# nkkrnkl/category-agnostic-pose-estimation

Measured on AMD Instinct MI355X. Metric: episodes/sec (1-shot, 256x256, 17kpt) training step, higher is better.
Workload: dtype f32 storage/accumulate, GEMMs as bf16x3 split (3 bf16 MFMAs per product); 1 GPU; configs[1]: 1-shot training step (fwd+loss+bwd+clip+AdamW at learning rate 0, dropout on), 256x256, 17 kpt, ResNet-50 + deformable transformer, 16 episodes x 2 queries per GPU; episodes_per_gpu=16, queries_per_episode=2, image_size=256, global_batch_episodes=16, parallelism=dp1, weights=random init (no checkpoint offline)

## Files before the change

### category-agnostic-pose-estimation_amd/csrc/error.hip

```cpp
#include <stdarg.h>
#include "common.h"

static thread_local char g_err[512] = "";

int cape_set_error(const char* fmt, ...) {
  va_list ap;
  va_start(ap, fmt);
  vsnprintf(g_err, sizeof(g_err), fmt, ap);
  va_end(ap);
  return 1;
}

extern "C" const char* cape_last_error(void) { return g_err; }
extern "C" int cape_abi_version(void) { return 11; }

__global__ void rng_advance_kernel(uint64_t* st) { st[1] += 1; }
extern "C" int cape_rng_advance(uint64_t* rng_state, cape_stream_t stream) {
  CAPE_REQUIRE(rng_state != nullptr, "cape_rng_advance: null state");
  hipLaunchKernelGGL(rng_advance_kernel, dim3(1), dim3(1), 0, as_stream(stream), rng_state);
  CAPE_LAUNCH_CHECK("cape_rng_advance");
  return 0;
}

static hipEvent_t g_ev[64];
static int g_ev_next = 0, g_ev_init = 0;
static int order_after(hipStream_t first, hipStream_t then, const char* what) {
  if (!g_ev_init) {
    for (int i = 0; i < 64; ++i) {
      hipError_t e = hipEventCreateWithFlags(&g_ev[i], hipEventDisableTiming);
      if (e != hipSuccess) return cape_set_error("%s: hipEventCreate: %s", what, hipGetErrorString(e));
    }
    g_ev_init = 1;
  }
  hipEvent_t ev = g_ev[g_ev_next];
  g_ev_next = (g_ev_next + 1) & 63;
  hipError_t e = hipEventRecord(ev, first);
  if (e == hipSuccess) e = hipStreamWaitEvent(then, ev, 0);
  if (e != hipSuccess) return cape_set_error("%s: %s", what, hipGetErrorString(e));
  return 0;
}
extern "C" int cape_stream_fork(cape_stream_t main_stream, cape_stream_t side_stream) {
  return order_after(as_stream(main_stream), as_stream(side_stream), "cape_stream_fork");
}
extern "C" int cape_stream_join(cape_stream_t main_stream, cape_stream_t side_stream) {
  return order_after(as_stream(side_stream), as_stream(main_stream), "cape_stream_join");
}
```

### category-agnostic-pose-estimation_amd/csrc/gemm.hip

```cpp
#include "gemm_tile.h"

namespace {

template <int BM, int BN, int AMODE, int BMODE, bool VEC, int PREC, bool KFULL>
__global__ void __launch_bounds__(256) gemm_kernel(const GemmP pin) {
  GemmP p = pin;
  if (gridDim.y > 1) {
    const int b0 = blockIdx.y / p.bdiv, b1 = blockIdx.y - b0 * p.bdiv;
    p.A += b0 * p.sA0 + b1 * p.sA1;
    p.B += b0 * p.sB0 + b1 * p.sB1;
    p.C += b0 * p.sC0 + b1 * p.sC1;
    if (p.bias) p.bias += b0 * p.sBias0 + b1 * p.sBias1;
  }
  gemm_tile_body<BM, BN, AMODE, BMODE, VEC, PREC, KFULL>(p, (int)blockIdx.x);
}

constexpr int SK_COLS = 8, SK_KC = 256;

__global__ void __launch_bounds__(512) gemm_skinny_kernel(const GemmP p) {
  __shared__ __attribute__((aligned(16))) float xs[64 * (SK_KC + 4)];
  __shared__ __attribute__((aligned(16))) float ws[SK_COLS * (SK_KC + 4)];
  const int t = threadIdx.x;
  const int n0 = blockIdx.x * SK_COLS;
  const int col = t & (SK_COLS - 1), row = t >> 3;
// ... 46 lines not shown
      return 0;                                                                            \
    }                                                                                      \
    if (vec && kfull) hipLaunchKernelGGL((gemm_kernel<BM, BN, AM, BM_, true, 0, true>), grid, dim3(256), 0, s, p);   \
    else if (vec) hipLaunchKernelGGL((gemm_kernel<BM, BN, AM, BM_, true, 0, false>), grid, dim3(256), 0, s, p);      \
    else hipLaunchKernelGGL((gemm_kernel<BM, BN, AM, BM_, false, 0, false>), grid, dim3(256), 0, s, p);              \
    return 0;                                                                              \
  }
  CASE(0, 0) CASE(2, 0) CASE(0, 1) CASE(3, 2) CASE(1, 1) CASE(1, 3)
#undef CASE
  return cape_set_error("cape_gemm_f32: unsupported (a_mode=%d, b_mode=%d)", a_mode, b_mode);
}

}

extern "C" int cape_gemm_f32(const cape_gemm_desc* d, cape_stream_t stream) {
  CAPE_REQUIRE(d != nullptr, "cape_gemm_f32: null descriptor");
  CAPE_REQUIRE(d->M >= 0 && d->N >= 0 && d->K >= 0, "cape_gemm_f32: negative size");
  if (d->M == 0 || d->N == 0) return 0;
  CAPE_REQUIRE(d->A && d->B && d->C, "cape_gemm_f32: null operand");
  CAPE_REQUIRE(d->split_k >= 1, "cape_gemm_f32: split_k must be >= 1");
  if (d->split_k > 1)
    CAPE_REQUIRE(!d->scale && !d->residual && !d->relu && d->dropout_p == 0.f,
                 "cape_gemm_f32: split_k > 1 allows no epilogue op besides the bias and accumulation");
  if (d->a_mode == 2 || d->a_mode == 3 || d->b_mode == 2 || d->b_mode == 3) {
    CAPE_REQUIRE(d->cC % 4 == 0 && d->cO % 4 == 0, "cape_gemm_f32: conv channels must be multiples of 4 (C=%d, O=%d)", d->cC, d->cO);
    CAPE_REQUIRE(d->cStride >= 1 && d->cKH >= 1 && d->cKW >= 1, "cape_gemm_f32: bad conv geometry");
    const long long taps = (long long)d->cKH * d->cKW;
    if (d->a_mode == 2) CAPE_REQUIRE(d->K == taps * d->cC && d->M == (long long)d->cN * d->cOH * d->cOW, "cape_gemm_f32: conv-fwd shape mismatch");
    if (d->a_mode == 3) CAPE_REQUIRE(d->K == taps * d->cO && d->M == (long long)d->cN * d->cH * d->cW && d->N == d->cC, "cape_gemm_f32: conv-dgrad shape mismatch");
    if (d->b_mode == 3) CAPE_REQUIRE(d->N == taps * d->cC && d->K == (long long)d->cN * d->cOH * d->cOW && d->M == d->cO, "cape_gemm_f32: conv-wgrad shape mismatch");
    CAPE_REQUIRE((reinterpret_cast<uintptr_t>(d->A) & 15) == 0 && (reinterpret_cast<uintptr_t>(d->B) & 15) == 0,
                 "cape_gemm_f32: conv operands must be 16-byte aligned");
  }
  if (d->dropout_p > 0.f) CAPE_REQUIRE(d->rng_state != nullptr && d->dropout_p < 1.f, "cape_gemm_f32: dropout needs rng_state and p < 1");

  GemmP p;
  p.M = d->M; p.N = d->N; p.K = d->K;
  p.A = d->A; p.lda = d->lda; p.B = d->B; p.ldb = d->ldb; p.C = d->C; p.ldc = d->ldc;
  p.cN = d->cN; p.cH = d->cH; p.cW = d->cW; p.cC = d->cC; p.cKH = d->cKH; p.cKW = d->cKW;
  p.cStride = d->cStride; p.cPad = d->cPad; p.cOH = d->cOH; p.cOW = d->cOW; p.cO = d->cO;
  p.scale = d->scale; p.bias = d->bias; p.residual = d->residual; p.ldr = d->ldr;
  p.relu = d->relu; p.accumulate = d->accumulate; p.split_k = d->split_k;
  p.colsum_out = d->colsum_out;
  if (d->colsum_out) CAPE_REQUIRE(d->a_mode == 1, "cape_gemm_f32: colsum_out needs a_mode 1 (the wgrad product)");
  p.drop_thresh = d->dropout_p > 0.f ? cape_drop_threshold(d->dropout_p) : 0u;
  p.inv_keep = d->dropout_p > 0.f ? 1.f / (1.f - d->dropout_p) : 1.f;
  p.rng_state = d->rng_state; p.rng_stream = d->rng_stream;

  p.Bpack = d->B_packed;
  p.mask_src = d->mask_src; p.ldm = d->ldm; p.mask_scale = d->mask_scale;
  p.bdiv = d->batch_div > 0 ? d->batch_div : 1;
  p.sA0 = d->sA0; p.sA1 = d->sA1; p.sB0 = d->sB0; p.sB1 = d->sB1; p.sC0 = d->sC0; p.sC1 = d->sC1;
  p.res_cols = d->res_cols; p.sBias0 = d->sBias0; p.sBias1 = d->sBias1;
  if (d->cKHp > 0) {
    CAPE_REQUIRE(d->a_mode == 3 && d->b_mode == 2 && d->cStride == 1 && d->cO % 32 == 0 && d->K % 32 == 0 && d->cKWp > 0 &&
                     d->cTapHS >= 1 && d->cTapWS >= 1 && d->cTapH0 >= 0 && d->cTapW0 >= 0 &&
                     d->cTapH0 + (d->cKH - 1) * d->cTapHS < d->cKHp && d->cTapW0 + (d->cKW - 1) * d->cTapWS < d->cKWp,
                 "cape_gemm_f32: tap sub-lattice needs conv-dgrad modes, stride 1, O %% 32 == 0 and taps inside the physical filter");
    p.cPadX = d->cPadX; p.cKHp = d->cKHp; p.cKWp = d->cKWp;
    p.cTapH0 = d->cTapH0; p.cTapHS = d->cTapHS; p.cTapW0 = d->cTapW0; p.cTapWS = d->cTapWS;
  } else {
    p.cPadX = d->cPad; p.cKHp = d->cKH; p.cKWp = d->cKW; p.cTapH0 = 0; p.cTapHS = 1; p.cTapW0 = 0; p.cTapWS = 1;
  }
  CAPE_REQUIRE(d->res_cols >= 0 && d->res_cols % 32 == 0, "cape_gemm_f32: res_cols must be a non-negative multiple of 32");
  if (d->batch > 1)
    CAPE_REQUIRE(d->batch <= 65535 && d->split_k == 1 && !d->scale && !d->residual && !d->mask_src && !d->colsum_out &&
                     d->dropout_p == 0.f && (d->a_mode == 0 || d->a_mode == 1) && (d->b_mode == 0 || d->b_mode == 1),
                 "cape_gemm_f32: batched launches take dense modes, no epilogue vector besides the bias, split_k 1, batch <= 65535");
  if (d->mask_src) CAPE_REQUIRE(d->split_k == 1, "cape_gemm_f32: mask_src needs split_k == 1");
  CAPE_REQUIRE(d->precision >= 0 && d->precision <= 2, "cape_gemm_f32: precision must be 0 (fp32), 1 (bf16x3) or 2 (single bf16)");
  p.single = d->precision == 2;
  const int prec = d->precision == 0 ? 0 : 1;
  if (prec == 1 && d->batch <= 1 && cape_gemm_rs_eligible(p, d->a_mode, d->b_mode)) return cape_gemm_rs_launch(p, d->b_mode, as_stream(stream));

  auto al16 = [](const void* q) { return (reinterpret_cast<uintptr_t>(q) & 15) == 0; };
  bool vec = al16(d->A) && al16(d->B);
  if (d->a_mode == 0) vec = vec && (d->lda % 4 == 0) && (d->K % 4 == 0);
  if (d->a_mode == 1) vec = vec && (d->lda % 4 == 0) && (d->M % 4 == 0) && d->M >= 4;
  if (d->b_mode == 0) vec = vec && (d->ldb % 4 == 0) && (d->K % 4 == 0);
  if (d->b_mode == 1) vec = vec && (d->ldb % 4 == 0) && (d->N % 4 == 0) && d->N >= 4;
  if (d->b_mode == 2 || d->b_mode == 3) vec = vec && (d->N % 4 == 0) && d->N >= 4;
  if (d->batch > 1) vec = vec && ((d->sA0 | d->sA1 | d->sB0 | d->sB1) % 4 == 0);
  if ((d->a_mode >= 2 || d->b_mode >= 2) && !vec) return cape_set_error("cape_gemm_f32: conv modes need the aligned vector path");
  if (d->a_mode == 0 && d->b_mode == 0 && d->M <= 64 && d->batch <= 1 && vec && d->split_k == 1 && d->dropout_p == 0.f && !d->colsum_out &&
      !d->mask_src && (d->N + SK_COLS - 1) / SK_COLS < (1 << 30)) {
    static const bool off = getenv("CAPE_GEMM_NO_SKINNY") != nullptr;
    if (!off) {
      hipLaunchKernelGGL(gemm_skinny_kernel, dim3((d->N + SK_COLS - 1) / SK_COLS), dim3(512), 0, as_stream(stream), p);
      CAPE_LAUNCH_CHECK("cape_gemm_f32(skinny)");
      return 0;
    }
  }

  const long long t128 = (long long)((d->M + 127) / 128) * ((d->N + 127) / 128) * d->split_k;
  bool big = d->K / d->split_k >= 1024 && t128 >= 256 && (long long)d->M * d->N >= 256 * 1024 && prec == 1 && vec;
  {
    static const char* force = getenv("CAPE_GEMM_TILE");
    if (force && force[0] == '1') big = true;
    if (force && force[0] == '6') big = false;
  }
  const int BMv = big ? 128 : 64;
  p.tilesM = (d->M + BMv - 1) / BMv;
  p.tilesN = (d->N + BMv - 1) / BMv;
  const long long ntiles = (long long)p.tilesM * p.tilesN;
  CAPE_REQUIRE(ntiles < (1ll << 31), "cape_gemm_f32: too many tiles");
  CAPE_REQUIRE(ntiles * d->split_k < (1ll << 31), "cape_gemm_f32: grid too large");
// ... 93 lines not shown
```

### category-agnostic-pose-estimation_amd/csrc/gemm_common.h

```cpp
#pragma once
#include "common.h"

typedef float f32x16 __attribute__((ext_vector_type(16)));
typedef __bf16 bf16x8 __attribute__((ext_vector_type(8)));

typedef __bf16 bf16x2 __attribute__((ext_vector_type(2)));
__device__ __forceinline__ unsigned pk_bf16(float lo, float hi) {
  bf16x2 v;
  v[0] = (__bf16)lo;
  v[1] = (__bf16)hi;
  return __builtin_bit_cast(unsigned, v);
}
__device__ __forceinline__ void split2(float& x, float& y, unsigned& hi, unsigned& lo) {
  hi = pk_bf16(x, y);
  const bf16x2 hv = __builtin_bit_cast(bf16x2, hi);
  x = __builtin_amdgcn_fdot2_f32_bf16(hv, __builtin_bit_cast(bf16x2, 0x8000BF80u), x, false);
  y = __builtin_amdgcn_fdot2_f32_bf16(hv, __builtin_bit_cast(bf16x2, 0xBF808000u), y, false);
  lo = pk_bf16(x, y);
}

struct GemmP {
  int M, N, K;
  const float* A; long long lda;
  const float* B; long long ldb;
  float* C; long long ldc;
  int cN, cH, cW, cC, cKH, cKW, cStride, cPad, cOH, cOW, cO;
  const float* scale; const float* bias; const float* residual; long long ldr;
  int relu, accumulate, split_k;
  float* colsum_out;
  uint32_t drop_thresh; float inv_keep;
  const uint64_t* rng_state; uint32_t rng_stream;
  int tilesM, tilesN;
  const unsigned short* Bpack;
  const float* mask_src; long long ldm; float mask_scale;
  int bdiv; long long sA0, sA1, sB0, sB1, sC0, sC1;
  int single;
  int res_cols;
  long long sBias0, sBias1;
  int cPadX, cKHp, cKWp, cTapH0, cTapHS, cTapW0, cTapWS;
};

__device__ __forceinline__ float4 zero4() { return make_float4(0.f, 0.f, 0.f, 0.f); }

template <int W>
__device__ __forceinline__ int tr_off(int k, int chunk) {
  static_assert(W == 64 || W == 128, "tile widths of the family");
  const int mask = (W == 128) ? ((k & 3) << 2) : (((k >> 1) & 1) << 2);
  return k * (W * 2) + ((chunk ^ mask) << 4);
}
typedef short tr_s4 __attribute__((ext_vector_type(4)));
__device__ __forceinline__ bf16x8 tr_read8(const char* p, int rows4) {
#if defined(__HIP_DEVICE_COMPILE__)
  const tr_s4 a = __builtin_amdgcn_ds_read_tr16_b64_v4i16((tr_s4 __attribute__((address_space(3)))*)(p));
  const tr_s4 b = __builtin_amdgcn_ds_read_tr16_b64_v4i16((tr_s4 __attribute__((address_space(3)))*)(p + rows4));
  typedef short s8 __attribute__((ext_vector_type(8)));
  const s8 v = __builtin_shufflevector(a, b, 0, 1, 2, 3, 4, 5, 6, 7);
  return __builtin_bit_cast(bf16x8, v);
#else
  (void)p; (void)rows4;
  return bf16x8{};
#endif
}

constexpr int BK = 32;

bool cape_gemm_rs_eligible(const GemmP& p, int a_mode, int b_mode);
int cape_gemm_rs_launch(const GemmP& p, int b_mode, hipStream_t stream);
```

### category-agnostic-pose-estimation_amd/csrc/gemm_group.hip

```cpp
#include "gemm_tile.h"

namespace {

constexpr int GROUP_MAX = CAPE_GEMM_GROUP_MAX;

struct GroupItem {
  const float* A; const float* B; float* C; float* colsum_out;
  int M, N, K, split_k;
  int lda, ldb, ldc, tilesM;
  int tilesN, cN, cH, cW;
  int cC, cKH, cKW, cStride;
  int cPad, cOH, cOW, cO;
};

struct GroupArgs {
  int n, single;
  int bstart[GROUP_MAX + 1];
  GroupItem it[GROUP_MAX];
};
static_assert(sizeof(GroupArgs) <= 4096, "the item table travels as kernel arguments");

template <int BM, int BN, int BMODE, int PREC, bool KFULL>
__global__ void __launch_bounds__(256) gemm_group_kernel(const GroupArgs g) {
  const int b = blockIdx.x;
  int i = 0;
  while (i + 1 < g.n && b >= g.bstart[i + 1]) ++i;
  const GroupItem& q = g.it[i];
  GemmP p;
  p.M = q.M; p.N = q.N; p.K = q.K;
  p.A = q.A; p.lda = q.lda; p.B = q.B; p.ldb = q.ldb; p.C = q.C; p.ldc = q.ldc;
  p.cN = q.cN; p.cH = q.cH; p.cW = q.cW; p.cC = q.cC; p.cKH = q.cKH; p.cKW = q.cKW;
  p.cStride = q.cStride; p.cPad = q.cPad; p.cOH = q.cOH; p.cOW = q.cOW; p.cO = q.cO;
  p.cPadX = q.cPad; p.cKHp = q.cKH; p.cKWp = q.cKW; p.cTapH0 = 0; p.cTapHS = 1; p.cTapW0 = 0; p.cTapWS = 1;
  p.scale = nullptr; p.bias = nullptr; p.residual = nullptr; p.ldr = 0;
  p.relu = 0; p.accumulate = 1; p.split_k = q.split_k;
  p.colsum_out = q.colsum_out;
  p.drop_thresh = 0; p.inv_keep = 1.f; p.rng_state = nullptr; p.rng_stream = 0;
  p.tilesM = q.tilesM; p.tilesN = q.tilesN;
  p.Bpack = nullptr; p.mask_src = nullptr; p.ldm = 0; p.mask_scale = 1.f;
  p.bdiv = 1; p.sA0 = p.sA1 = p.sB0 = p.sB1 = p.sC0 = p.sC1 = 0;
  p.res_cols = 0; p.sBias0 = p.sBias1 = 0; p.single = g.single;
  gemm_tile_body<BM, BN, 1, BMODE, true, PREC, KFULL>(p, b - g.bstart[i]);
}

template <int BM, int BMODE>
void launch_group(const GroupArgs& g, int prec, bool kfull, hipStream_t s) {
  const dim3 grid((unsigned)g.bstart[g.n]), block(256);
  if (prec == 1) {
    if (kfull) hipLaunchKernelGGL((gemm_group_kernel<BM, BM, BMODE, 1, true>), grid, block, 0, s, g);
    else hipLaunchKernelGGL((gemm_group_kernel<BM, BM, BMODE, 1, false>), grid, block, 0, s, g);
  } else {
    if (kfull) hipLaunchKernelGGL((gemm_group_kernel<BM, BM, BMODE, 0, true>), grid, block, 0, s, g);
    else hipLaunchKernelGGL((gemm_group_kernel<BM, BM, BMODE, 0, false>), grid, block, 0, s, g);
  }
}

}

extern "C" int cape_gemm_group_f32(const cape_gemm_desc* descs, int n, int tile, cape_stream_t stream) {
  CAPE_REQUIRE(descs != nullptr && n >= 1 && n <= GROUP_MAX, "cape_gemm_group_f32: n=%d must be in 1..%d", n, GROUP_MAX);
  CAPE_REQUIRE(tile == 64 || tile == 128, "cape_gemm_group_f32: tile must be 64 or 128");
  const int b_mode = descs[0].b_mode, prec_in = descs[0].precision, prec = prec_in == 0 ? 0 : 1;
  CAPE_REQUIRE(b_mode == 1 || b_mode == 3, "cape_gemm_group_f32: only the weight-gradient modes (a_mode 1, b_mode 1 or 3) are grouped");
  CAPE_REQUIRE(prec_in >= 0 && prec_in <= 2, "cape_gemm_group_f32: precision must be 0 (fp32), 1 (bf16x3) or 2 (single bf16)");
  auto al16 = [](const void* q) { return (reinterpret_cast<uintptr_t>(q) & 15) == 0; };
  GroupArgs g;
  g.n = n;
  g.single = prec_in == 2;
  bool kfull = true;
  long long blocks = 0;
  for (int i = 0; i < n; ++i) {
    const cape_gemm_desc& d = descs[i];
    CAPE_REQUIRE(d.a_mode == 1 && d.b_mode == b_mode && d.precision == prec_in, "cape_gemm_group_f32: item %d: mixed modes / precisions", i);
    CAPE_REQUIRE(d.M > 0 && d.N > 0 && d.K > 0 && d.A && d.B && d.C, "cape_gemm_group_f32: item %d: empty product or null operand", i);
    CAPE_REQUIRE(d.accumulate && !d.scale && !d.bias && !d.residual && !d.relu && d.dropout_p == 0.f && !d.mask_src && d.batch <= 1,
                 "cape_gemm_group_f32: item %d: grouped products accumulate onto C and take no other epilogue operand", i);
    CAPE_REQUIRE(d.split_k >= 1, "cape_gemm_group_f32: item %d: split_k must be >= 1", i);
    CAPE_REQUIRE(al16(d.A) && al16(d.B) && d.lda % 4 == 0 && d.M % 4 == 0 && d.M >= 4 && d.N % 4 == 0 && d.N >= 4 &&
                     (b_mode == 3 || d.ldb % 4 == 0),
                 "cape_gemm_group_f32: item %d: operands must be 16-byte aligned with M, N, lda, ldb multiples of 4", i);
    CAPE_REQUIRE(d.lda < (1ll << 31) && d.ldb < (1ll << 31) && d.ldc < (1ll << 31), "cape_gemm_group_f32: item %d: leading dimension too large", i);
    if (b_mode == 3) {
      const long long taps = (long long)d.cKH * d.cKW;
      CAPE_REQUIRE(d.cC % 4 == 0 && d.cO % 4 == 0 && d.cStride >= 1 && d.cKH >= 1 && d.cKW >= 1, "cape_gemm_group_f32: item %d: bad conv geometry", i);
      CAPE_REQUIRE(d.N == taps * d.cC && d.K == (long long)d.cN * d.cOH * d.cOW && d.M == d.cO, "cape_gemm_group_f32: item %d: conv-wgrad shape mismatch", i);
    }
    GroupItem& q = g.it[i];
    q.A = d.A; q.B = d.B; q.C = d.C; q.colsum_out = d.colsum_out;
    q.M = d.M; q.N = d.N; q.K = d.K; q.split_k = d.split_k;
    q.lda = (int)d.lda; q.ldb = (int)d.ldb; q.ldc = (int)d.ldc;
    q.tilesM = (d.M + tile - 1) / tile; q.tilesN = (d.N + tile - 1) / tile;
    q.cN = d.cN; q.cH = d.cH; q.cW = d.cW; q.cC = d.cC; q.cKH = d.cKH; q.cKW = d.cKW;
    q.cStride = d.cStride; q.cPad = d.cPad; q.cOH = d.cOH; q.cOW = d.cOW; q.cO = d.cO;
    kfull = kfull && (d.K % BK == 0);
// ... 14 lines not shown
```

### category-agnostic-pose-estimation_amd/csrc/gemm_rs.hip

```cpp
#include <stdlib.h>
#include "gemm_common.h"

namespace {

constexpr int RS_UNIT = 64;

#ifdef RS_STAMPS
__device__ long long* g_rs_stamps;
#define RS_STAMP(i) do { if (threadIdx.x == 0 && (i) < 16) g_rs_stamps[blockIdx.x * 16 + (i)] = clock64(); } while (0)
#define RS_FINE(cond, i) do { if ((cond) && threadIdx.x == 0) g_rs_stamps[blockIdx.x * 16 + 8 + (i)] = clock64(); } while (0)
#else
#define RS_STAMP(i) do {} while (0)
#define RS_FINE(cond, i) do {} while (0)
#endif

template <int KS>
struct RsGeom {
  static constexpr int K = 16 * KS;
  static constexpr int LD = K + 8;
  static constexpr int PLANE = RS_UNIT * LD;
  static constexpr int NV = KS / 2;
  static constexpr size_t LDS_BYTES = (size_t)2  * 2  * PLANE * 2;
};

template <int NW, int BMODE, int KS, int EPI>
__global__ void __launch_bounds__(512) gemm_rs_kernel(const GemmP p, int nchunks, int gpc) {
  using G = RsGeom<KS>;
  constexpr int K = G::K, LD = G::LD, NV = G::NV;
  constexpr int CPR = K / 4;
  extern __shared__ __attribute__((aligned(16))) unsigned short lds[];

  const int t = threadIdx.x, lane = t & 63, wave = t >> 6;
  const int r = lane & 31, h = lane >> 5;
  const int wn = wave % NW, wm = wave / NW;

  const int bid = blockIdx.x;
  const int xcd = bid & 7, loc = bid >> 3;
  const int chunk = loc % nchunks;
  const int slot = (loc / nchunks) * 8 + xcd;
  const int n0 = chunk * (32 * NW) + 32 * wn;
  const int nunits = (p.M + RS_UNIT - 1) / RS_UNIT;
  if (slot >= nunits) return;

  const int st_row = t / CPR, st_kc = t % CPR;
  constexpr int RSTEP = 512 / CPR;
  auto load_rows = [&](float4 (&dst)[NV], const float* base, long long ld, int row0, int nrows) {
#pragma unroll
    for (int i = 0; i < NV; ++i) {
      const int row = min(row0 + st_row + RSTEP * i, nrows - 1);
      dst[i] = *reinterpret_cast<const float4*>(base + (long long)row * ld + 4 * st_kc);
    }
  };
  auto store_rows = [&](float4 (&src)[NV], int buf) {
    unsigned short* Ph = lds + buf * 2 * G::PLANE;
    unsigned short* Pl = Ph + G::PLANE;
#pragma unroll
    for (int i = 0; i < NV; ++i) {
      const int o = (st_row + RSTEP * i) * LD + 4 * st_kc;
      unsigned h0, l0, h1, l1;
      split2(src[i].x, src[i].y, h0, l0);
      split2(src[i].z, src[i].w, h1, l1);
      *reinterpret_cast<uint2*>(Ph + o) = make_uint2(h0, h1);
      *reinterpret_cast<uint2*>(Pl + o) = make_uint2(l0, l1);
    }
  };

  const int col = n0 + r;
  const bool col_ok = col < p.N;
  const float sc = p.scale ? p.scale[min(col, p.N - 1)] : 1.f;
  const float bi = p.bias ? p.bias[min(col, p.N - 1)] : 0.f;
  const float floor_v = p.relu ? 0.f : -__builtin_inff();
  uint64_t seed = 0, step = 0;
  if constexpr (EPI == 4) { seed = p.rng_state[0]; step = p.rng_state[1]; }
  const int ldc = (int)p.ldc;
  const unsigned lo_c = (unsigned)(4 * h * ldc + col);
  const int ldx = EPI == 1 ? (int)p.ldr : ldc;
  const unsigned lo_x = (unsigned)(4 * h * ldx + col);
  const bool res_on = EPI != 1 || !p.res_cols || n0 < p.res_cols;

  auto store_piece = [&](float4& v, int i, int buf) {
    unsigned short* Ph = lds + buf * 2 * G::PLANE + (st_row + RSTEP * i) * LD + 4 * st_kc;
    unsigned h0, l0, h1, l1;
    split2(v.x, v.y, h0, l0);
    split2(v.z, v.w, h1, l1);
    *reinterpret_cast<uint2*>(Ph) = make_uint2(h0, h1);
    *reinterpret_cast<uint2*>(Ph + G::PLANE) = make_uint2(l0, l1);
  };

  RS_STAMP(0);
  bf16x8 bhi[KS], blo[KS];
  float4 ra[NV];
  if (p.Bpack) {
    load_rows(ra, p.A, p.lda, slot * RS_UNIT, p.M);
    const int grp = min(n0 >> 5, (p.N + 31) / 32 - 1);
    const uint4* bp = reinterpret_cast<const uint4*>(p.Bpack) + ((long long)grp * KS * 2) * 64 + lane;
#pragma unroll
    for (int s = 0; s < KS; ++s) {
      bhi[s] = __builtin_bit_cast(bf16x8, bp[(2 * s + 0) * 64]);
      blo[s] = __builtin_bit_cast(bf16x8, bp[(2 * s + 1) * 64]);
    }
  } else if constexpr (BMODE == 0) {
    constexpr int NPASS = NW / 2;
    const int nb = chunk * (32 * NW);
    float4 rw[2][NV];
    load_rows(rw[0], p.B, p.ldb, nb, p.N);
    if (NPASS > 1) load_rows(rw[1], p.B, p.ldb, nb + 64, p.N);
    load_rows(ra, p.A, p.lda, slot * RS_UNIT, p.M);
#pragma unroll
    for (int q = 0; q < NPASS; ++q) {
      store_rows(rw[q & 1], q & 1);
      if (q + 2 < NPASS) load_rows(rw[q & 1], p.B, p.ldb, nb + 64 * (q + 2), p.N);
      __syncthreads();
      if ((wn >> 1) == q) {
        const unsigned short* Ph = lds + (q & 1) * 2 * G::PLANE + (32 * (wn & 1) + r) * LD + 8 * h;
#pragma unroll
        for (int s = 0; s < KS; ++s) {
          bhi[s] = *reinterpret_cast<const bf16x8*>(Ph + 16 * s);
          blo[s] = *reinterpret_cast<const bf16x8*>(Ph + G::PLANE + 16 * s);
        }
      }
    }
    __syncthreads();
  } else {
    load_rows(ra, p.A, p.lda, slot * RS_UNIT, p.M);
    const int n = min(n0 + r, p.N - 1);
#pragma unroll
    for (int s = 0; s < KS; ++s) {
      float f[8];
      const int k = 16 * s + 8 * h;
#pragma unroll
      for (int j = 0; j < 8; ++j) f[j] = p.B[(long long)(k + j) * p.ldb + n];
      unsigned hw[4], lw[4];
#pragma unroll
      for (int j = 0; j < 4; ++j) split2(f[2 * j], f[2 * j + 1], hw[j], lw[j]);
      bhi[s] = __builtin_bit_cast(bf16x8, make_uint4(hw[0], hw[1], hw[2], hw[3]));
      blo[s] = __builtin_bit_cast(bf16x8, make_uint4(lw[0], lw[1], lw[2], lw[3]));
    }
  }

  RS_STAMP(1);
  store_rows(ra, 0);
  if (slot + gpc < nunits) load_rows(ra, p.A, p.lda, (slot + gpc) * RS_UNIT, p.M);
  __syncthreads();
  RS_STAMP(2);
  int stamp_i = 3;

  int buf = 0;
  for (int u = slot; u < nunits; u += gpc) {
    const bool has_next = u + gpc < nunits;
    const unsigned short* Ah = lds + buf * 2 * G::PLANE;
    const unsigned short* Al = Ah + G::PLANE;
    const bool full = (u + 1) * RS_UNIT <= p.M;
    constexpr int H1 = (NW == 8) ? 2 : 1;
#pragma unroll
    for (int hh = 0; hh < H1; ++hh) {
      const int half = (NW == 8) ? hh : wm;
      float xv[16];
      if constexpr (EPI >= 1 && EPI <= 3) {
        if (col_ok && res_on) {
          const int rb = u * RS_UNIT + 32 * half;
          const float* xb = EPI == 1 ? p.residual : EPI == 2 ? p.mask_src : p.C;
          const float* x0 = xb + (long long)rb * ldx;
#pragma unroll
          for (int i = 0; i < 16; ++i) {
            const int roff = (i & 3) + 8 * (i >> 2);
            if (full) xv[i] = x0[lo_x + (unsigned)(roff * ldx)];
            else xv[i] = xb[(long long)min(rb + roff + 4 * h, p.M - 1) * ldx + col];
          }
        } else {
#pragma unroll
          for (int i = 0; i < 16; ++i) xv[i] = 0.f;
        }
      }
      f32x16 acc;
#pragma unroll
      for (int i = 0; i < 16; ++i) acc[i] = 0.f;
      RS_FINE(u == slot + gpc, 3 * hh);
      const int ao = (32 * half + r) * LD + 8 * h;
#pragma unroll
      for (int s = 0; s < KS; ++s) {
        const bf16x8 ahi = *reinterpret_cast<const bf16x8*>(Ah + ao + 16 * s);
        const bf16x8 alo = *reinterpret_cast<const bf16x8*>(Al + ao + 16 * s);
        if (!p.single) {
          acc = __builtin_amdgcn_mfma_f32_32x32x16_bf16(alo, bhi[s], acc, 0, 0, 0);
          acc = __builtin_amdgcn_mfma_f32_32x32x16_bf16(ahi, blo[s], acc, 0, 0, 0);
        }
        acc = __builtin_amdgcn_mfma_f32_32x32x16_bf16(ahi, bhi[s], acc, 0, 0, 0);
        if (hh == H1 - 1 && s >= KS - NV && has_next) store_piece(ra[s - (KS - NV)], s - (KS - NV), buf ^ 1);
      }
      RS_FINE(u == slot + gpc, 3 * hh + 1);
      if (!col_ok) continue;
      const int rb = u * RS_UNIT + 32 * half;
      const int rlim = full ? 64 : p.M - rb - 4 * h;
      float* c0 = p.C + (long long)rb * ldc;
      if constexpr (EPI == 0) {
        if (full) {
#pragma unroll
          for (int i = 0; i < 16; ++i) c0[lo_c + (unsigned)(((i & 3) + 8 * (i >> 2)) * ldc)] = fmaxf(fmaf(acc[i], sc, bi), floor_v);
        } else {
#pragma unroll
          for (int i = 0; i < 16; ++i) {
            const int roff = (i & 3) + 8 * (i >> 2);
            if (roff < rlim) c0[lo_c + (unsigned)(roff * ldc)] = fmaxf(fmaf(acc[i], sc, bi), floor_v);
          }
        }
      } else if constexpr (EPI == 4) {
#pragma unroll
        for (int i = 0; i < 16; ++i) {
          const int roff = (i & 3) + 8 * (i >> 2);
          const int row = rb + roff + 4 * h;
          float v = fmaxf(fmaf(acc[i], sc, bi), floor_v);
          v = cape_keep(seed, step, p.rng_stream, (uint64_t)row * (uint64_t)p.N + col, p.drop_thresh) ? v * p.inv_keep : 0.f;
          if (roff < rlim) c0[lo_c + (unsigned)(roff * ldc)] = v;
        }
      } else {
#pragma unroll
        for (int i = 0; i < 16; ++i) {
          const int roff = (i & 3) + 8 * (i >> 2);
          const float x = xv[i];
          float v = fmaf(acc[i], sc, bi);
          if constexpr (EPI == 1) v = fmaxf(v + x, floor_v);
          if constexpr (EPI == 2) v = x != 0.f ? fmaxf(v, floor_v) * p.mask_scale : 0.f;
          if constexpr (EPI == 3) v = fmaxf(v, floor_v) + x;
          if (roff < rlim) c0[lo_c + (unsigned)(roff * ldc)] = v;
        }
      }
    }
    RS_FINE(u == slot + gpc, 6);
    if (u + 2 * gpc < nunits) load_rows(ra, p.A, p.lda, (u + 2 * gpc) * RS_UNIT, p.M);
    __syncthreads();
    RS_FINE(u == slot + gpc, 7);
    RS_STAMP(stamp_i); ++stamp_i;
    buf ^= 1;
  }
}

static int rs_epi(const GemmP& p) {
  const int n = (p.residual != nullptr) + (p.mask_src != nullptr) + (p.accumulate != 0) + (p.drop_thresh != 0);
  if (n == 0) return 0;
  if (n > 1) return -1;
  return p.residual ? 1 : p.mask_src ? 2 : p.accumulate ? 3 : 4;
}

template <int NW, int BMODE, int KS, int EPI>
int rs_launch_epi(const GemmP& p, int nchunks, int gpc, hipStream_t s) {
  static bool attr_set = false;
  auto kfn = gemm_rs_kernel<NW, BMODE, KS, EPI>;
  if (!attr_set) {
    hipError_t e = hipFuncSetAttribute(reinterpret_cast<const void*>(kfn), hipFuncAttributeMaxDynamicSharedMemorySize,
                                       (int)RsGeom<KS>::LDS_BYTES);
    if (e != hipSuccess) return cape_set_error("cape_gemm_f32(rs): hipFuncSetAttribute: %s", hipGetErrorString(e));
    attr_set = true;
  }
  hipLaunchKernelGGL(kfn, dim3((unsigned)(gpc * nchunks)), dim3(512), RsGeom<KS>::LDS_BYTES, s, p, nchunks, gpc);
  return 0;
}

template <int NW, int BMODE, int KS>
int rs_launch(const GemmP& p, int nchunks, int gpc, hipStream_t s) {
  switch (rs_epi(p)) {
    case 0: return rs_launch_epi<NW, BMODE, KS, 0>(p, nchunks, gpc, s);
    case 1: return rs_launch_epi<NW, BMODE, KS, 1>(p, nchunks, gpc, s);
    case 2: return rs_launch_epi<NW, BMODE, KS, 2>(p, nchunks, gpc, s);
    case 3: return rs_launch_epi<NW, BMODE, KS, 3>(p, nchunks, gpc, s);
    case 4: return rs_launch_epi<NW, BMODE, KS, 4>(p, nchunks, gpc, s);
  }
  return cape_set_error("cape_gemm_f32(rs): unsupported epilogue combination");
}

struct PackItem { const float* B; unsigned short* out; long long ldb; int N, K, b_mode, pad; };
static_assert(sizeof(PackItem) == sizeof(cape_pack_item), "cape_pack_item layout");

__global__ void __launch_bounds__(256) pack_weights_kernel(const PackItem* items, int n_items) {
  const int lane = threadIdx.x & 63, wave = threadIdx.x >> 6;
  const int r = lane & 31, h = lane >> 5;
  for (int it = blockIdx.y; it < n_items; it += gridDim.y) {
    const PackItem q = items[it];
    const int KS = q.K >> 4, groups = (q.N + 31) >> 5;
    for (int w = blockIdx.x * 4 + wave; w < groups * KS; w += gridDim.x * 4) {
      const int g = w / KS, s = w - g * KS;
      const int n = 32 * g + r, k = 16 * s + 8 * h;
      float f[8];
#pragma unroll
      for (int j = 0; j < 8; ++j) f[j] = 0.f;
      if (n < q.N) {
        if (q.b_mode == 0) {
#pragma unroll
          for (int j = 0; j < 8; ++j) f[j] = q.B[(long long)n * q.ldb + k + j];
        } else {
#pragma unroll
          for (int j = 0; j < 8; ++j) f[j] = q.B[(long long)(k + j) * q.ldb + n];
        }
      }
      unsigned hw[4], lw[4];
#pragma unroll
      for (int j = 0; j < 4; ++j) split2(f[2 * j], f[2 * j + 1], hw[j], lw[j]);
      uint4* o = reinterpret_cast<uint4*>(q.out) + ((long long)w * 2) * 64 + lane;
      o[0] = make_uint4(hw[0], hw[1], hw[2], hw[3]);
      o[64] = make_uint4(lw[0], lw[1], lw[2], lw[3]);
    }
  }
}

}

extern "C" size_t cape_packed_weight_bytes(int N, int K) {
  if (N <= 0 || K <= 0) return 0;
  return (size_t)((N + 31) / 32) * 32 * (size_t)K * 4;
}

extern "C" int cape_pack_weights(const cape_pack_item* items_dev, int n_items, int max_blocks_per_item, cape_stream_t stream) {
  CAPE_REQUIRE(items_dev != nullptr && n_items >= 0 && max_blocks_per_item >= 1, "cape_pack_weights: bad arguments");
  if (n_items == 0) return 0;
  const unsigned gy = (unsigned)(n_items < 65535 ? n_items : 65535);
  hipLaunchKernelGGL(pack_weights_kernel, dim3((unsigned)max_blocks_per_item, gy), dim3(256), 0, as_stream(stream),
                     reinterpret_cast<const PackItem*>(items_dev), n_items);
  CAPE_LAUNCH_CHECK("cape_pack_weights");
  return 0;
// ... 42 lines not shown
```

### category-agnostic-pose-estimation_amd/csrc/gemm_tile.h

```cpp
#pragma once
#include <stdlib.h>
#include <type_traits>
#include "gemm_common.h"

namespace {

__device__ __forceinline__ float4 ldg4(const float* p, int valid) {
  if (valid >= 4 && ((reinterpret_cast<uintptr_t>(p) & 15) == 0)) return *reinterpret_cast<const float4*>(p);
  float4 r = zero4();
  if (valid > 0) r.x = p[0];
  if (valid > 1) r.y = p[1];
  if (valid > 2) r.z = p[2];
  if (valid > 3) r.w = p[3];
  return r;
}

template <int BM, int BN, int AMODE, int BMODE, bool VEC, int PREC, bool KFULL>
__device__ __forceinline__ void gemm_tile_body(const GemmP& p, const int bid) {
  constexpr bool A_KC = (AMODE == 0 || AMODE == 2 || AMODE == 3);
  constexpr bool B_KC = (BMODE == 0);
  constexpr int A_LD = A_KC ? 36 : (BM + 4);
  constexpr int B_LD = B_KC ? 36 : (BN + 4);
  constexpr int A_SZ = A_KC ? BM * 36 : BK * (BM + 4);
  constexpr int B_SZ = B_KC ? BN * 36 : BK * (BN + 4);
// ... 482 lines not shown
    if (t + 1 + DEPTH < kt_end) load_tiles(t + 1 + DEPTH, NEXT);
  };
  using S0 = std::integral_constant<int, 0>;
  using S1 = std::integral_constant<int, 1 % DEPTH>;
  using S2 = std::integral_constant<int, 2 % DEPTH>;
  load_tiles(kt_begin, S0{});
  if constexpr (DEPTH >= 2)
    if (kt_begin + 1 < kt_end) load_tiles(kt_begin + 1, S1{});
  if constexpr (DEPTH == 3)
    if (kt_begin + 2 < kt_end) load_tiles(kt_begin + 2, S2{});
  if (do_colsum) colsum_tile(S0{});
  store_tiles(0, S0{});
  if (kt_begin + DEPTH < kt_end) load_tiles(kt_begin + DEPTH, S0{});
  __syncthreads();
  int cur = 0;
  for (int kt = kt_begin; kt < kt_end; kt += DEPTH) {
    pipeline_step(kt, cur, S1{});
    cur ^= 1;
    if constexpr (DEPTH >= 2) {
      if (kt + 1 >= kt_end) break;
      pipeline_step(kt + 1, cur, S2{});
      cur ^= 1;
    }
    if constexpr (DEPTH == 3) {
      if (kt + 2 >= kt_end) break;
      pipeline_step(kt + 2, cur, S0{});
      cur ^= 1;
    }
  }

  if constexpr (AMODE == 1) {
    if (do_colsum) {
      float4* red = reinterpret_cast<float4*>(&As[0][0]);
      red[t] = csum;
      __syncthreads();
      if (t < A_CH) {
        float4 r = red[t];
#pragma unroll
        for (int i = 1; i < 256 / A_CH; ++i) { const float4 u = red[t + A_CH * i]; r.x += u.x; r.y += u.y; r.z += u.z; r.w += u.w; }
        const int m = m0 + 4 * t;
        if (m < p.M) atomicAdd(p.colsum_out + m, r.x);
        if (m + 1 < p.M) atomicAdd(p.colsum_out + m + 1, r.y);
        if (m + 2 < p.M) atomicAdd(p.colsum_out + m + 2, r.z);
        if (m + 3 < p.M) atomicAdd(p.colsum_out + m + 3, r.w);
      }
    }
  }

  uint64_t seed = 0, step = 0;
  const bool drop = p.drop_thresh != 0;
  if (drop) { seed = p.rng_state[0]; step = p.rng_state[1]; }
  const bool atomic = p.split_k > 1;
  const bool interior = (m0 + BM <= p.M) && (n0 + BN <= p.N);
  const int n_extra = (p.residual != nullptr) + (p.mask_src != nullptr) + (p.accumulate != 0) + (drop ? 1 : 0);
  const bool same_ld = (!p.residual || p.ldr == p.ldc) && (!p.mask_src || p.ldm == p.ldc);
  if (interior && !drop && n_extra <= 1 && same_ld && (long long)BM * p.ldc < (1ll << 30)) {
    const int wave_s = __builtin_amdgcn_readfirstlane(wave);
    const int wm_s = wave_s >> 1, wn_s = wave_s & 1;
    const int ldc = (int)p.ldc;
    const float floor_v = p.relu ? 0.f : -INFINITY;
    const float* xb = p.residual ? p.residual : p.mask_src ? p.mask_src : (p.accumulate && !atomic) ? p.C : nullptr;
    const int kind = atomic ? 1 : p.residual ? 2 : p.mask_src ? 3 : p.accumulate ? 4 : 0;
#pragma unroll
    for (int i = 0; i < TI; ++i) {
#pragma unroll
      for (int j = 0; j < TJ; ++j) {
        const int colb = n0 + wn_s * WTN + j * 32;
        const long long base = (long long)(m0 + wm_s * WTM + i * 32) * ldc + colb;
        float* c0 = p.C + base;
        const unsigned lo = (unsigned)(4 * lh * ldc + l31);
        const float sc = p.scale ? p.scale[colb + l31] : 1.f;
        const float bi = p.bias ? p.bias[colb + l31] : 0.f;
        const int kind_t = (kind == 2 && p.res_cols && colb >= p.res_cols) ? 0 : kind;
        if (kind == 1) {
          const float b0 = split == 0 ? bi : 0.f;
#pragma unroll
          for (int r = 0; r < 16; ++r) atomicAdd(c0 + (lo + (unsigned)(((r & 3) + 8 * (r >> 2)) * ldc)), acc[i][j][r] + b0);
        } else if (kind_t == 0) {
#pragma unroll
          for (int r = 0; r < 16; ++r) c0[lo + (unsigned)(((r & 3) + 8 * (r >> 2)) * ldc)] = fmaxf(fmaf(acc[i][j][r], sc, bi), floor_v);
        } else {
          const float* x0 = xb + base;
          float xv[16];
#pragma unroll
          for (int r = 0; r < 16; ++r) xv[r] = x0[lo + (unsigned)(((r & 3) + 8 * (r >> 2)) * ldc)];
#pragma unroll
          for (int r = 0; r < 16; ++r) {
            float v = fmaf(acc[i][j][r], sc, bi);
            if (kind == 2) v = fmaxf(v + xv[r], floor_v);
            else if (kind == 3) v = xv[r] != 0.f ? fmaxf(v, floor_v) * p.mask_scale : 0.f;
            else v = fmaxf(v, floor_v) + xv[r];
            c0[lo + (unsigned)(((r & 3) + 8 * (r >> 2)) * ldc)] = v;
          }
        }
      }
    }
    return;
  }
#pragma unroll
  for (int i = 0; i < TI; ++i) {
#pragma unroll
    for (int j = 0; j < TJ; ++j) {
      const int col = n0 + wn * WTN + j * 32 + l31;
      if (!interior && col >= p.N) continue;
      const float sc = p.scale ? p.scale[col] : 1.f;
      const float bi = p.bias ? p.bias[col] : 0.f;
#pragma unroll
      for (int r = 0; r < 16; ++r) {
        const int row = m0 + wm * WTM + i * 32 + (r & 3) + 8 * (r >> 2) + 4 * lh;
        if (!interior && row >= p.M) continue;
        float v = acc[i][j][r];
        float* cp = p.C + (long long)row * p.ldc + col;
        if (atomic) { atomicAdd(cp, split == 0 ? v + bi : v); continue; }
        v = v * sc + bi;
        if (p.residual && (!p.res_cols || col < p.res_cols)) v += p.residual[(long long)row * p.ldr + col];
        if (p.relu) v = fmaxf(v, 0.f);
        if (drop) v = cape_keep(seed, step, p.rng_stream, (uint64_t)row * (uint64_t)p.N + col, p.drop_thresh) ? v * p.inv_keep : 0.f;
        if (p.mask_src) v = p.mask_src[(long long)row * p.ldm + col] != 0.f ? v * p.mask_scale : 0.f;
        if (p.accumulate) v += *cp;
        *cp = v;
      }
    }
  }
}

}
```

### category-agnostic-pose-estimation_amd/csrc/norm.hip

```cpp
#include "common.h"

namespace {

constexpr int LN_MAXV = 4;

__global__ void __launch_bounds__(256) add_ln_fwd_kernel(const float* __restrict__ x, const float* __restrict__ y,
                                                          const float* __restrict__ gamma, const float* __restrict__ beta,
                                                          float* __restrict__ out, float* __restrict__ mean_o,
                                                          float* __restrict__ rstd_o, const float* __restrict__ pos,
                                                          float* __restrict__ out_pos, int rows, int C, uint32_t thresh,
                                                          float inv_keep, const uint64_t* rng_state, uint32_t rng_stream) {
  const int lane = threadIdx.x & 63;
  const int row = blockIdx.x * 4 + (threadIdx.x >> 6);
  if (row >= rows) return;
  const int nv = C >> 8;
  const int rem = (C & 255) >> 2;
  uint64_t seed = 0, step = 0;
  if (thresh) { seed = rng_state[0]; step = rng_state[1]; }
  float4 s[LN_MAXV];
  float sum = 0.f;
  const long long base = (long long)row * C;
#pragma unroll
  for (int i = 0; i < LN_MAXV; ++i) {
    const bool act = (i < nv) || (i == nv && lane < rem);
// ... 55 lines not shown
#endif
constexpr int LN_BWD_ROWS = LN_BWD_ROWS_DEF;

__global__ void __launch_bounds__(256) add_ln_bwd_kernel(const float* __restrict__ d_out, const float* __restrict__ d_out_pos,
                                                          const float* __restrict__ x, const float* __restrict__ y,
                                                          const float* __restrict__ gamma, const float* __restrict__ mean_i,
                                                          const float* __restrict__ rstd_i, float* __restrict__ d_x,
                                                          float* __restrict__ d_y, float* __restrict__ dgamma,
                                                          float* __restrict__ dbeta, int rows, int C, uint32_t thresh,
                                                          float inv_keep, const uint64_t* rng_state, uint32_t rng_stream) {
  __shared__ float red[2][4][1024];
  const int lane = threadIdx.x & 63, w = threadIdx.x >> 6;
  const int nv = C >> 8, rem = (C & 255) >> 2;
  uint64_t seed = 0, step = 0;
  if (thresh) { seed = rng_state[0]; step = rng_state[1]; }
  float4 ag[LN_MAXV], ab[LN_MAXV], gam[LN_MAXV];
#pragma unroll
  for (int i = 0; i < LN_MAXV; ++i) {
    ag[i] = make_float4(0.f, 0.f, 0.f, 0.f);
    ab[i] = make_float4(0.f, 0.f, 0.f, 0.f);
    const bool act = (i < nv) || (i == nv && lane < rem);
    gam[i] = act ? *reinterpret_cast<const float4*>(gamma + (i * 64 + lane) * 4) : make_float4(0.f, 0.f, 0.f, 0.f);
  }
  const int r_begin = blockIdx.x * LN_BWD_ROWS;
  for (int rr = w; rr < LN_BWD_ROWS; rr += 4) {
    const int row = r_begin + rr;
    if (row >= rows) break;
    const long long base = (long long)row * C;
    const float mean = mean_i[row], rstd = rstd_i[row];
    float4 xh[LN_MAXV], g[LN_MAXV];
    uint32_t keepbits = 0;
    float s1 = 0.f, s2 = 0.f;
#pragma unroll
    for (int i = 0; i < LN_MAXV; ++i) {
      const bool act = (i < nv) || (i == nv && lane < rem);
      xh[i] = make_float4(0.f, 0.f, 0.f, 0.f);
      g[i] = make_float4(0.f, 0.f, 0.f, 0.f);
      if (act) {
        const int c = (i * 64 + lane) * 4;
        float4 v = *reinterpret_cast<const float4*>(x + base + c);
        if (y) {
          float4 q = *reinterpret_cast<const float4*>(y + base + c);
          if (thresh) {
            const uint64_t idx = (uint64_t)base + c;
            const bool k0 = cape_keep(seed, step, rng_stream, idx + 0, thresh);
            const bool k1 = cape_keep(seed, step, rng_stream, idx + 1, thresh);
            const bool k2 = cape_keep(seed, step, rng_stream, idx + 2, thresh);
            const bool k3 = cape_keep(seed, step, rng_stream, idx + 3, thresh);
            keepbits |= ((uint32_t)k0 | ((uint32_t)k1 << 1) | ((uint32_t)k2 << 2) | ((uint32_t)k3 << 3)) << (4 * i);
            q.x = k0 ? q.x * inv_keep : 0.f; q.y = k1 ? q.y * inv_keep : 0.f;
            q.z = k2 ? q.z * inv_keep : 0.f; q.w = k3 ? q.w * inv_keep : 0.f;
          }
          v.x += q.x; v.y += q.y; v.z += q.z; v.w += q.w;
        }
        float4 d = *reinterpret_cast<const float4*>(d_out + base + c);
        if (d_out_pos) {
          const float4 e = *reinterpret_cast<const float4*>(d_out_pos + base + c);
          d.x += e.x; d.y += e.y; d.z += e.z; d.w += e.w;
        }
        xh[i].x = (v.x - mean) * rstd; xh[i].y = (v.y - mean) * rstd;
        xh[i].z = (v.z - mean) * rstd; xh[i].w = (v.w - mean) * rstd;
        ag[i].x += d.x * xh[i].x; ag[i].y += d.y * xh[i].y; ag[i].z += d.z * xh[i].z; ag[i].w += d.w * xh[i].w;
        ab[i].x += d.x; ab[i].y += d.y; ab[i].z += d.z; ab[i].w += d.w;
        g[i].x = d.x * gam[i].x; g[i].y = d.y * gam[i].y; g[i].z = d.z * gam[i].z; g[i].w = d.w * gam[i].w;
        s1 += g[i].x + g[i].y + g[i].z + g[i].w;
        s2 += g[i].x * xh[i].x + g[i].y * xh[i].y + g[i].z * xh[i].z + g[i].w * xh[i].w;
      }
    }
    const float m1 = wave_sum(s1) / (float)C, m2 = wave_sum(s2) / (float)C;
#pragma unroll
    for (int i = 0; i < LN_MAXV; ++i) {
      const bool act = (i < nv) || (i == nv && lane < rem);
      if (act) {
        const int c = (i * 64 + lane) * 4;
        float4 ds;
        ds.x = rstd * (g[i].x - m1 - xh[i].x * m2);
        ds.y = rstd * (g[i].y - m1 - xh[i].y * m2);
        ds.z = rstd * (g[i].z - m1 - xh[i].z * m2);
        ds.w = rstd * (g[i].w - m1 - xh[i].w * m2);
        *reinterpret_cast<float4*>(d_x + base + c) = ds;
        if (d_y && d_y != d_x) {
          if (thresh) {
            const uint32_t kb = keepbits >> (4 * i);
            ds.x = (kb & 1) ? ds.x * inv_keep : 0.f; ds.y = (kb & 2) ? ds.y * inv_keep : 0.f;
            ds.z = (kb & 4) ? ds.z * inv_keep : 0.f; ds.w = (kb & 8) ? ds.w * inv_keep : 0.f;
          }
          *reinterpret_cast<float4*>(d_y + base + c) = ds;
        }
      }
    }
  }
#pragma unroll
  for (int i = 0; i < LN_MAXV; ++i) {
    const bool act = (i < nv) || (i == nv && lane < rem);
    if (act) {
      const int c = (i * 64 + lane) * 4;
      *reinterpret_cast<float4*>(&red[0][w][c]) = ag[i];
      *reinterpret_cast<float4*>(&red[1][w][c]) = ab[i];
    }
  }
  __syncthreads();
#ifndef LAB_LN_NO_ATOMIC
  for (int c = threadIdx.x; c < C; c += 256) {
    atomicAdd(&dgamma[c], red[0][0][c] + red[0][1][c] + red[0][2][c] + red[0][3][c]);
    atomicAdd(&dbeta[c], red[1][0][c] + red[1][1][c] + red[1][2][c] + red[1][3][c]);
  }
#endif
}

constexpr int LN256_R = 4;

constexpr int LN256_W = 16;

__global__ void __launch_bounds__(64 * LN256_W) add_ln_bwd256_kernel(const float* __restrict__ d_out, const float* __restrict__ d_out_pos,
                                                             const float* __restrict__ x, const float* __restrict__ y,
                                                             const float* __restrict__ gamma, const float* __restrict__ mean_i,
                                                             const float* __restrict__ rstd_i, float* __restrict__ d_x,
                                                             float* __restrict__ d_y, float* __restrict__ dgamma,
                                                             float* __restrict__ dbeta, int rows, uint32_t thresh, float inv_keep,
                                                             const uint64_t* rng_state, uint32_t rng_stream) {
  __shared__ float red[2][LN256_W][256];
  const int lane = threadIdx.x & 63, w = threadIdx.x >> 6;
  uint64_t seed = 0, step = 0;
  if (thresh) { seed = rng_state[0]; step = rng_state[1]; }
  const float4 gam = *reinterpret_cast<const float4*>(gamma + 4 * lane);
  float4 ag = make_float4(0.f, 0.f, 0.f, 0.f), ab = make_float4(0.f, 0.f, 0.f, 0.f);
  const bool split = d_y && d_y != d_x;
  const int wave_g = blockIdx.x * LN256_W + w, nwaves = gridDim.x * LN256_W;
  for (int r0 = wave_g * LN256_R; r0 < rows; r0 += nwaves * LN256_R) {
    float4 v[LN256_R], d[LN256_R];
    float mean[LN256_R], rstd[LN256_R];
    uint32_t kb[LN256_R];
#pragma unroll
    for (int k = 0; k < LN256_R; ++k) {
      const int row = min(r0 + k, rows - 1);
      const long long base = (long long)row * 256 + 4 * lane;
      v[k] = *reinterpret_cast<const float4*>(x + base);
      d[k] = *reinterpret_cast<const float4*>(d_out + base);
      mean[k] = mean_i[row]; rstd[k] = rstd_i[row];
    }
    if (y) {
#pragma unroll
      for (int k = 0; k < LN256_R; ++k) {
        const int row = min(r0 + k, rows - 1);
        const long long base = (long long)row * 256 + 4 * lane;
        float4 q = *reinterpret_cast<const float4*>(y + base);
        kb[k] = 0xF;
        if (thresh) {
          const uint64_t idx = (uint64_t)base;
          const bool k0 = cape_keep(seed, step, rng_stream, idx + 0, thresh), k1 = cape_keep(seed, step, rng_stream, idx + 1, thresh);
          const bool k2 = cape_keep(seed, step, rng_stream, idx + 2, thresh), k3 = cape_keep(seed, step, rng_stream, idx + 3, thresh);
          kb[k] = (uint32_t)k0 | ((uint32_t)k1 << 1) | ((uint32_t)k2 << 2) | ((uint32_t)k3 << 3);
          q.x = k0 ? q.x * inv_keep : 0.f; q.y = k1 ? q.y * inv_keep : 0.f;
          q.z = k2 ? q.z * inv_keep : 0.f; q.w = k3 ? q.w * inv_keep : 0.f;
        }
        v[k].x += q.x; v[k].y += q.y; v[k].z += q.z; v[k].w += q.w;
      }
    }
    if (d_out_pos) {
#pragma unroll
      for (int k = 0; k < LN256_R; ++k) {
        const int row = min(r0 + k, rows - 1);
        const float4 e = *reinterpret_cast<const float4*>(d_out_pos + (long long)row * 256 + 4 * lane);
        d[k].x += e.x; d[k].y += e.y; d[k].z += e.z; d[k].w += e.w;
      }
    }
#pragma unroll
    for (int k = 0; k < LN256_R; ++k) {
      const bool live = r0 + k < rows;
      float4 xh, g;
      xh.x = (v[k].x - mean[k]) * rstd[k]; xh.y = (v[k].y - mean[k]) * rstd[k];
      xh.z = (v[k].z - mean[k]) * rstd[k]; xh.w = (v[k].w - mean[k]) * rstd[k];
      if (live) {
        ag.x += d[k].x * xh.x; ag.y += d[k].y * xh.y; ag.z += d[k].z * xh.z; ag.w += d[k].w * xh.w;
        ab.x += d[k].x; ab.y += d[k].y; ab.z += d[k].z; ab.w += d[k].w;
      }
      g.x = d[k].x * gam.x; g.y = d[k].y * gam.y; g.z = d[k].z * gam.z; g.w = d[k].w * gam.w;
      const float m1 = wave_sum(g.x + g.y + g.z + g.w) * (1.f / 256.f);
      const float m2 = wave_sum(g.x * xh.x + g.y * xh.y + g.z * xh.z + g.w * xh.w) * (1.f / 256.f);
      float4 ds;
      ds.x = rstd[k] * (g.x - m1 - xh.x * m2); ds.y = rstd[k] * (g.y - m1 - xh.y * m2);
      ds.z = rstd[k] * (g.z - m1 - xh.z * m2); ds.w = rstd[k] * (g.w - m1 - xh.w * m2);
      if (live) {
        const long long base = (long long)(r0 + k) * 256 + 4 * lane;
        *reinterpret_cast<float4*>(d_x + base) = ds;
        if (split) {
          if (thresh) {
            ds.x = (kb[k] & 1) ? ds.x * inv_keep : 0.f; ds.y = (kb[k] & 2) ? ds.y * inv_keep : 0.f;
            ds.z = (kb[k] & 4) ? ds.z * inv_keep : 0.f; ds.w = (kb[k] & 8) ? ds.w * inv_keep : 0.f;
          }
          *reinterpret_cast<float4*>(d_y + base) = ds;
        }
      }
    }
  }
  *reinterpret_cast<float4*>(&red[0][w][4 * lane]) = ag;
  *reinterpret_cast<float4*>(&red[1][w][4 * lane]) = ab;
  __syncthreads();
  if (threadIdx.x < 512) {
    const int which = threadIdx.x >> 8, c = threadIdx.x & 255;
    float a = 0.f;
#pragma unroll
    for (int k = 0; k < LN256_W; ++k) a += red[which][k][c];
    atomicAdd((which ? dbeta : dgamma) + c, a);
  }
}

constexpr int GN_ROWS = 16;

// ... 54 lines not shown
  atomicAdd(w, sd);
  atomicAdd(w + 1, sdx);
}

__global__ void groupnorm_bwd_apply_kernel(const float* __restrict__ d_out, long long d_out_image_stride,
                                           const float* __restrict__ x, const float* __restrict__ gamma,
                                           const float* __restrict__ mean_i, const float* __restrict__ rstd_i,
                                           const float* __restrict__ ws, float* __restrict__ d_x,
                                           float* __restrict__ dgamma, float* __restrict__ dbeta, int HW, int C, int G) {
  const int n = blockIdx.y, c = threadIdx.x;
  const int cpg = C / G;
  const float mean = mean_i[n * G + c / cpg], rstd = rstd_i[n * G + c / cpg];
  const float sd = ws[((long long)n * C + c) * 2], sdx = ws[((long long)n * C + c) * 2 + 1];
  if (blockIdx.x == 0) { atomicAdd(&dgamma[c], sdx); atomicAdd(&dbeta[c], sd); }
  const float g = gamma[c];
  const float cnt = (float)HW * (float)cpg;
  const float A = group_sum(g * sd, cpg) / cnt;
  const float B = group_sum(g * sdx, cpg) / cnt;
  const int r0 = blockIdx.x * GN_ROWS, r1 = min(HW, r0 + GN_ROWS);
  const float* xp = x + (long long)n * HW * C + c;
  const float* dp = d_out + (long long)n * d_out_image_stride + c;
  float* op = d_x + (long long)n * HW * C + c;
  for (int r = r0; r < r1; ++r) {
    const float xh = (xp[(long long)r * C] - mean) * rstd;
    op[(long long)r * C] = rstd * (g * dp[(long long)r * C] - A - xh * B);
  }
}

}

extern "C" int cape_add_layernorm_fwd(const float* x, const float* y, const float* gamma, const float* beta,
                                      float* out, float* mean, float* rstd, const float* pos, float* out_pos,
                                      int rows, int C, float dropout_p, const uint64_t* rng_state,
                                      uint32_t rng_stream, cape_stream_t stream) {
  CAPE_REQUIRE(x && gamma && beta && out && mean && rstd, "cape_add_layernorm_fwd: null pointer");
  CAPE_REQUIRE(C > 0 && C <= 1024 && (C % 4) == 0, "cape_add_layernorm_fwd: C=%d must be a multiple of 4, <= 1024", C);
  CAPE_REQUIRE((pos == nullptr) == (out_pos == nullptr), "cape_add_layernorm_fwd: pos and out_pos go together");
  CAPE_REQUIRE(dropout_p == 0.f || (y && rng_state && dropout_p < 1.f), "cape_add_layernorm_fwd: dropout needs y and rng_state");
  if (rows <= 0) return 0;
  const uint32_t th = dropout_p > 0.f ? cape_drop_threshold(dropout_p) : 0u;
  const float ik = dropout_p > 0.f ? 1.f / (1.f - dropout_p) : 1.f;
  hipLaunchKernelGGL(add_ln_fwd_kernel, dim3((rows + 3) / 4), dim3(256), 0, as_stream(stream), x, y, gamma, beta, out,
                     mean, rstd, pos, out_pos, rows, C, th, ik, rng_state, rng_stream);
  CAPE_LAUNCH_CHECK("cape_add_layernorm_fwd");
  return 0;
}

extern "C" int cape_add_layernorm_bwd(const float* d_out, const float* d_out_pos, const float* x, const float* y,
                                      const float* gamma, const float* mean, const float* rstd, float* d_x,
                                      float* d_y, float* dgamma, float* dbeta, int rows, int C, float dropout_p,
                                      const uint64_t* rng_state, uint32_t rng_stream, cape_stream_t stream) {
  CAPE_REQUIRE(d_out && x && gamma && mean && rstd && d_x && dgamma && dbeta, "cape_add_layernorm_bwd: null pointer");
  CAPE_REQUIRE(C > 0 && C <= 1024 && (C % 4) == 0, "cape_add_layernorm_bwd: C=%d must be a multiple of 4, <= 1024", C);
  CAPE_REQUIRE(dropout_p == 0.f || (y && d_y && d_y != d_x && rng_state && dropout_p < 1.f),
               "cape_add_layernorm_bwd: dropout needs y, a separate d_y and rng_state");
  if (rows <= 0) return 0;
  const uint32_t th = dropout_p > 0.f ? cape_drop_threshold(dropout_p) : 0u;
  const float ik = dropout_p > 0.f ? 1.f / (1.f - dropout_p) : 1.f;
  static const bool general_only = getenv("CAPE_LN_BWD_GENERAL") != nullptr;
  if (C == 256 && !general_only) {
    const int trips = (rows + LN256_W * LN256_R - 1) / (LN256_W * LN256_R);
    const int blocks = trips < 256 ? trips : 256;
    hipLaunchKernelGGL(add_ln_bwd256_kernel, dim3(blocks), dim3(64 * LN256_W), 0, as_stream(stream), d_out, d_out_pos, x, y, gamma, mean, rstd,
                       d_x, d_y, dgamma, dbeta, rows, th, ik, rng_state, rng_stream);
    CAPE_LAUNCH_CHECK("cape_add_layernorm_bwd");
    return 0;
  }
  hipLaunchKernelGGL(add_ln_bwd_kernel, dim3((rows + LN_BWD_ROWS - 1) / LN_BWD_ROWS), dim3(256), 0, as_stream(stream),
                     d_out, d_out_pos, x, y, gamma, mean, rstd, d_x, d_y, dgamma, dbeta, rows, C, th, ik, rng_state,
                     rng_stream);
  CAPE_LAUNCH_CHECK("cape_add_layernorm_bwd");
  return 0;
}

static int gn_check(int N, int HW, int C, int G) {
  if (N <= 0 || HW <= 0) return 0;
  CAPE_REQUIRE(C >= 64 && C <= 1024 && (C % 64) == 0, "cape_groupnorm: C=%d must be a multiple of 64, <= 1024", C);
  CAPE_REQUIRE(G > 0 && (C % G) == 0, "cape_groupnorm: G=%d must divide C=%d", G, C);
  const int cpg = C / G;
  CAPE_REQUIRE(cpg <= 64 && (cpg & (cpg - 1)) == 0, "cape_groupnorm: channels per group (%d) must be a power of two <= 64", cpg);
  return 0;
}

extern "C" size_t cape_groupnorm_workspace_bytes(int N, int C, int G) {
  if (N <= 0 || C <= 0 || G <= 0) return 0;
  const size_t f = (size_t)N * G * 2 * sizeof(double), b = (size_t)N * C * 2 * sizeof(float);
  return f > b ? f : b;
}

extern "C" int cape_groupnorm_fwd(const float* x, const float* gamma, const float* beta, float* out,
                                  long long out_image_stride, float* mean, float* rstd, int N, int HW, int C, int G,
                                  void* workspace, size_t workspace_bytes, cape_stream_t stream) {
  CAPE_REQUIRE(x && gamma && beta && out && mean && rstd, "cape_groupnorm_fwd: null pointer");
  if (gn_check(N, HW, C, G)) return 1;
  if (N <= 0 || HW <= 0) return 0;
  const size_t need = (size_t)N * G * 2 * sizeof(double);
  CAPE_REQUIRE(workspace && workspace_bytes >= need && (reinterpret_cast<uintptr_t>(workspace) & 7) == 0,
               "cape_groupnorm_fwd: workspace of %zu bytes (8-byte aligned) needed, %zu given", need, workspace_bytes);
  CAPE_REQUIRE(N <= 65535, "cape_groupnorm_fwd: N too large");
  hipError_t e = hipMemsetAsync(workspace, 0, need, as_stream(stream));
  if (e != hipSuccess) return cape_set_error("cape_groupnorm_fwd: memset: %s", hipGetErrorString(e));
  const dim3 grid((HW + GN_ROWS - 1) / GN_ROWS, N);
  hipLaunchKernelGGL(groupnorm_stats_kernel, grid, dim3(C), 0, as_stream(stream), x, static_cast<double*>(workspace), HW, C, G);
  hipLaunchKernelGGL(groupnorm_apply_kernel, grid, dim3(C), 0, as_stream(stream), x, gamma, beta, out, out_image_stride,
                     static_cast<const double*>(workspace), mean, rstd, HW, C, G);
  CAPE_LAUNCH_CHECK("cape_groupnorm_fwd");
  return 0;
}
// ... 23 lines not shown
```

### category-agnostic-pose-estimation_amd/hip/functional.py

```python
import contextlib
import ctypes
import os

import torch

from . import lib, ops


class Runtime:
    rng = None
    direct_grad = False
    use_side_stream = os.environ.get("CAPE_SIDE_STREAM", "1") == "1"
    side = None
    on_param_grad = []
    capture_keep = None

    pending = []
    side_dirty = False

    defer_wgrad = os.environ.get("CAPE_DEFER_WGRAD", "1") == "1"
    wgrad_group = int(os.environ.get("CAPE_WGRAD_GROUP", "12"))
    wq = {}
    wq_total = 0
    wq_notify = []
# ... 152 lines not shown
        base = p._base
        if isinstance(base, torch.nn.Parameter) and base.grad is not None and base.requires_grad:
            off = p.storage_offset() - base.storage_offset() + base.grad.storage_offset()
            return torch.as_strided(base.grad, p.shape, p.stride(), off)
        return None

    def side(self, *tensors):
        return _Side(tensors) if self.direct else _NO_SIDE

    def gemm(self, *args, **kw):
        d, keep = ops.gemm_desc(*args, **kw)
        if self.direct and Runtime.defer_wgrad and _groupable(d):
            Runtime.enqueue_wgrad(d, keep)
        else:
            ops.launch_gemm(d)

    def result(self):
        if not self.direct:
            return tuple(self.bufs)
        Runtime.notify(*[r if isinstance(r, torch.nn.Parameter) else r._base for r, n in zip(self.refs, self.needs) if n])
        return (None,) * len(self.refs)


class _Slot:
    __slots__ = ("buf",)

    def __init__(self):
        self.buf = None


_SLOTS = os.environ.get("CAPE_GRAD_SLOTS", "1") == "1"


def _slot_of(x):
    return getattr(x, "_cape_slot", None) if _SLOTS else None


def _grad_target(slot, shape, device):
    if slot is not None and slot.buf is not None:
        b = slot.buf
        if b.is_contiguous() and b.numel() == int(torch.Size(shape).numel()) and b.device == device:
            return b.view(shape), True
    buf = torch.empty(shape, dtype=torch.float32, device=device)
    if slot is not None and slot.buf is None:
        slot.buf = buf
    return buf, False


def _slot_offer(slot, buf):
    if slot is not None and slot.buf is None and buf is not None and buf.is_contiguous():
        slot.buf = buf


class LinearFn(torch.autograd.Function):
    @staticmethod
    def forward(ctx, x, weight, bias, residual, relu, dropout_p, rng_stream):
        K = x.shape[-1]
        N = weight.shape[0]
        assert weight.shape[1] == K and weight.stride(1) == 1
        x2 = _c(x).view(-1, K)
        M = x2.shape[0]
        res2 = _c(residual).view(-1, N) if residual is not None else None
        y = torch.empty(M, N, dtype=torch.float32, device=x.device)
        rng = Runtime.get_rng(x.device) if dropout_p > 0 else None
        ops.gemm(x2, weight, y, M, N, K, ldb=weight.stride(0), bias=bias, residual=res2, relu=relu, dropout_p=dropout_p,
                 rng=rng, rng_stream=rng_stream)
        ctx.save_for_backward(x2, weight, y if (relu or dropout_p > 0) else None)
        ctx.w_ref, ctx.b_ref = weight, bias
        ctx.slot = _slot_of(x)
        ctx.meta = (relu, dropout_p, bias is not None, residual is not None, x.shape, M, N, K)
        return y.view(*x.shape[:-1], N)

    @staticmethod
    def backward(ctx, dy):
        x2, weight, y = ctx.saved_tensors
        relu, p, has_bias, has_res, xshape, M, N, K = ctx.meta
        dy2 = _c(dy).view(M, N)
        dpre = dy2
        if relu or p > 0:
            assert relu, "dropout epilogue is only used together with relu"
            dpre = ops.relu_drop_bwd(dy2, y, 1.0 / (1.0 - p) if p > 0 else 1.0)
        dx = None
        if ctx.needs_input_grad[0]:
            dx, acc = _grad_target(ctx.slot, (M, K), dy.device)
            ops.gemm(dpre, weight, dx, M, K, N, a_mode=0, b_mode=1, ldb=weight.stride(0), accumulate=acc)
            dx = dx.view(xshape)
        pg = _ParamGrads((ctx.w_ref, ctx.b_ref), ctx.needs_input_grad[1:3])
        dw, db = pg.bufs
        with pg.side(dpre, x2):
            if dw is not None:
                pg.gemm(dpre, x2, dw, N, K, M, a_mode=1, b_mode=1, lda=N, ldb=K, ldc=dw.stride(0), accumulate=True,
                        split_k=ops.pick_split_k(N, K, M), colsum_out=db)
            elif db is not None:
                ops.colsum(dpre, M, N, db)
        dres = dy if (has_res and ctx.needs_input_grad[3]) else None
        return (dx,) + pg.result() + (dres, None, None, None)


def linear(x, weight, bias=None, residual=None, relu=False, dropout_p=0.0, rng_stream=0):
    return LinearFn.apply(x, weight, bias, residual, relu, float(dropout_p), int(rng_stream))


class FFNFn(torch.autograd.Function):

    @staticmethod
    def forward(ctx, x, w1, b1, w2, b2, dropout_p, rng_stream):
        K, Hd, N = x.shape[-1], w1.shape[0], w2.shape[0]
        x2 = _c(x).view(-1, K)
        M = x2.shape[0]
        rng = Runtime.get_rng(x.device) if dropout_p > 0 else None
        h = torch.empty(M, Hd, dtype=torch.float32, device=x.device)
        ops.gemm(x2, w1, h, M, Hd, K, ldb=w1.stride(0), bias=b1, relu=True, dropout_p=dropout_p, rng=rng, rng_stream=rng_stream)
        y = torch.empty(M, N, dtype=torch.float32, device=x.device)
        ops.gemm(h, w2, y, M, N, Hd, ldb=w2.stride(0), bias=b2)
        ctx.save_for_backward(x2, w1, w2, h)
        ctx.refs = (w1, b1, w2, b2)
        ctx.slot = _slot_of(x)
        ctx.meta = (dropout_p, x.shape, M, K, Hd, N)
        return y.view(*x.shape[:-1], N)

    @staticmethod
    def backward(ctx, dy):
        x2, w1, w2, h = ctx.saved_tensors
        p, xshape, M, K, Hd, N = ctx.meta
        dy2 = _c(dy).view(M, N)
        dpre = torch.empty(M, Hd, dtype=torch.float32, device=dy.device)
        ops.gemm(dy2, w2, dpre, M, Hd, N, a_mode=0, b_mode=1, ldb=w2.stride(0), mask_src=h, mask_scale=1.0 / (1.0 - p) if p > 0 else 1.0)
        dx = None
        if ctx.needs_input_grad[0]:
            dx, acc = _grad_target(ctx.slot, (M, K), dy.device)
            ops.gemm(dpre, w1, dx, M, K, Hd, a_mode=0, b_mode=1, ldb=w1.stride(0), accumulate=acc)
            dx = dx.view(xshape)
        pg = _ParamGrads(ctx.refs)
        dw1, db1, dw2, db2 = pg.bufs
        with pg.side(dy2, dpre, h, x2):
            pg.gemm(dy2, h, dw2, N, Hd, M, a_mode=1, b_mode=1, lda=N, ldb=Hd, ldc=dw2.stride(0), accumulate=True,
                    split_k=ops.pick_split_k(N, Hd, M), colsum_out=db2)
            pg.gemm(dpre, x2, dw1, Hd, K, M, a_mode=1, b_mode=1, lda=Hd, ldb=K, ldc=dw1.stride(0), accumulate=True,
                    split_k=ops.pick_split_k(Hd, K, M), colsum_out=db1)
        return (dx,) + pg.result() + (None, None)


_NO_FFN_FUSE = os.environ.get("CAPE_NO_FFN_FUSE") is not None
_DETERMINISTIC = os.environ.get("CAPE_DETERMINISTIC", "0") == "1"


def ffn(x, w1, b1, w2, b2, dropout_p=0.0, rng_stream=0):
    if _NO_FFN_FUSE:
        return linear(linear(x, w1, b1, relu=True, dropout_p=dropout_p, rng_stream=rng_stream), w2, b2)
    return FFNFn.apply(x, w1, b1, w2, b2, float(dropout_p), int(rng_stream))


def _adjacent(a, b):
    return (a.is_contiguous() and b.is_contiguous() and a.untyped_storage().data_ptr() == b.untyped_storage().data_ptr()
            and b.data_ptr() == a.data_ptr() + a.numel() * a.element_size())


class LinearCat2Fn(torch.autograd.Function):

    @staticmethod
    def forward(ctx, x, w1, b1, w2, b2):
        K = x.shape[-1]
        N1, N2 = w1.shape[0], w2.shape[0]
        x2 = _c(x).view(-1, K)
        M = x2.shape[0]
        y = torch.empty(M, N1 + N2, dtype=torch.float32, device=x.device)
        adjacent = _adjacent(w1, w2) and _adjacent(b1, b2)
        if adjacent:
            ops.gemm(x2, torch.as_strided(w1, (N1 + N2, K), (K, 1)), y, M, N1 + N2, K, bias=torch.as_strided(b1, (N1 + N2,), (1,)))
        else:
            ops.gemm(x2, w1, y, M, N1, K, bias=b1, ldc=N1 + N2)
            ops.gemm(x2, w2, y[:, N1:], M, N2, K, bias=b2, ldc=N1 + N2)
        ctx.save_for_backward(x2, w1, w2)
        ctx.refs = (w1, b1, w2, b2)
        ctx.meta = (x.shape, M, N1, N2, K, adjacent)
        return y.view(*x.shape[:-1], N1 + N2)

    @staticmethod
    def backward(ctx, dy):
        x2, w1, w2 = ctx.saved_tensors
        xshape, M, N1, N2, K, adjacent = ctx.meta
        NT = N1 + N2
        dy2 = _c(dy).view(M, NT)
        dev = dy.device
        dx = None
        if ctx.needs_input_grad[0]:
            dx = torch.empty(M, K, dtype=torch.float32, device=dev)
            ops.gemm(dy2, w1, dx, M, K, N1, a_mode=0, b_mode=1, lda=NT)
            ops.gemm(dy2[:, N1:], w2, dx, M, K, N2, a_mode=0, b_mode=1, lda=NT, accumulate=True)
            dx = dx.view(xshape)
        pg = _ParamGrads(ctx.refs)
        dw1, db1, dw2, db2 = pg.bufs
        with pg.side(dy2, x2):
            if adjacent and _adjacent(dw1, dw2) and _adjacent(db1, db2):
                pg.gemm(dy2, x2, torch.as_strided(dw1, (NT, K), (K, 1)), NT, K, M, a_mode=1, b_mode=1, lda=NT, accumulate=True,
                        split_k=ops.pick_split_k(NT, K, M), colsum_out=torch.as_strided(db1, (NT,), (1,)))
            else:
                for dw, db, lo, n in ((dw1, db1, 0, N1), (dw2, db2, N1, N2)):
                    pg.gemm(dy2[:, lo:], x2, dw, n, K, M, a_mode=1, b_mode=1, lda=NT, accumulate=True, split_k=ops.pick_split_k(n, K, M),
                            colsum_out=db)
        return (dx,) + pg.result()


# ... 137 lines not shown
    if not relu:
        return dy, (dy if want_res else None)
    d = ops.relu_drop_bwd(dy, y, 1.0)
    return d, (d if want_res else None)


def _mask_only(dy, y, relu):
    return ops.relu_drop_bwd(dy, y, 1.0) if relu else dy


class BottleneckFn(torch.autograd.Function):

    @staticmethod
    def forward(ctx, x, w1, w2, w3, wd, s1, b1, s2, b2, s3, b3, sd, bd, stride, allow_split):
        o1, m1, t1 = _conv_stage_fwd(x, w1, s1, b1, None, 1, 0, True, allow_split)
        o2, m2, t2 = _conv_stage_fwd(o1, w2, s2, b2, None, stride, 1, True, allow_split)
        idt, md, td = x, None, ()
        if wd is not None:
            idt, md, td = _conv_stage_fwd(x, wd, sd, bd, None, stride, 0, False, allow_split)
        y, m3, t3 = _conv_stage_fwd(o2, w3, s3, b3, idt, 1, 0, True, allow_split)
        ctx.save_for_backward(*t1, *t2, *t3, *td)
        ctx.cuts = (len(t1), len(t1) + len(t2), len(t1) + len(t2) + len(t3))
        ctx.metas = (m1, m2, m3, md)
        ctx.w_refs = (w1, w2, w3, wd)
        return y

    @staticmethod
    def backward(ctx, dy):
        t, (a, b, c) = ctx.saved_tensors, ctx.cuts
        t1, t2, t3, td = t[:a], t[a:b], t[b:c], t[c:]
        m1, m2, m3, md = ctx.metas
        w1, w2, w3, wd = ctx.w_refs
        need_x, need_w1, need_w2, need_w3, need_wd = ctx.needs_input_grad[:5]
        d2, dw3, _, dres = _conv_stage_bwd(m3, t3, dy, w3, need_x=True, need_w=need_w3, need_res=need_x or wd is not None)
        d1, dw2, _, _ = _conv_stage_bwd(m2, t2, d2, w2, need_x=True, need_w=need_w2)
        dwd, dshort = None, (dres if need_x else None)
        if wd is not None:
            dshort, dwd, _, _ = _conv_stage_bwd(md, td, dres, wd, need_x=need_x, need_w=need_wd)
        dx, dw1, _, _ = _conv_stage_bwd(m1, t1, d1, w1, need_x=need_x, need_w=need_w1, acc_dx=dshort)
        return (dx, dw1, dw2, dw3, dwd) + (None,) * 10


def bottleneck(x, w1, w2, w3, wd, bn1, bn2, bn3, bnd, stride):
    sd, bd = bnd if bnd is not None else (None, None)
    return BottleneckFn.apply(x, w1, w2, w3, wd, bn1[0], bn1[1], bn2[0], bn2[1], bn3[0], bn3[1], sd, bd, int(stride), torch.is_grad_enabled())


def conv_bn_act(x, weight, scale, shift, stride=1, pad=0, relu=False, residual=None):
    return ConvFn.apply(x, weight, scale, shift, residual, int(stride), int(pad), bool(relu), torch.is_grad_enabled())


class AddLayerNormFn(torch.autograd.Function):
    @staticmethod
    def forward(ctx, x, y, gamma, beta, pos, dropout_p, rng_stream):
        x, y, pos = _c(x), _c(y), _c(pos)
        rng = Runtime.get_rng(x.device) if dropout_p > 0 else None
        out, mean, rstd, out_pos = ops.add_layernorm_fwd(x, y, gamma, beta, pos=pos, dropout_p=dropout_p, rng=rng,
                                                         rng_stream=rng_stream)
        ctx.save_for_backward(x, y, gamma, mean, rstd)
        ctx.refs = (gamma, beta)
        ctx.slot = _slot_of(x)
        ctx.meta = (dropout_p, rng_stream, pos is not None)
        ctx.set_materialize_grads(False)
        if pos is None:
            return out
        return out, out_pos

    @staticmethod
    def backward(ctx, d_out, d_out_pos=None):
        x, y, gamma, mean, rstd = ctx.saved_tensors
        p, stream, has_pos = ctx.meta
        g_pos = d_out_pos
        if d_out is None and d_out_pos is None:
            return None, None, None, None, None, None, None
        if d_out is None:
            d_out, d_out_pos = d_out_pos, None
        d_out, d_out_pos = _c(d_out), _c(d_out_pos)
        pg = _ParamGrads(ctx.refs)
        rng = Runtime.get_rng(x.device) if p > 0 else None
        dx, dy = ops.add_layernorm_bwd(d_out, d_out_pos, x, y, gamma, mean, rstd, *pg.bufs, dropout_p=p, rng=rng,
                                       rng_stream=stream)
        if y is None or dy is not dx:
            _slot_offer(ctx.slot, dx)
        dpos = g_pos if (has_pos and ctx.needs_input_grad[4]) else None
        return (dx, (dy if y is not None else None)) + pg.result() + (dpos, None, None)


def add_layernorm(x, y, gamma, beta, pos=None, dropout_p=0.0, rng_stream=0):
    return AddLayerNormFn.apply(x, y, gamma, beta, pos, float(dropout_p), int(rng_stream))


class AddFn(torch.autograd.Function):
    @staticmethod
    def forward(ctx, a, b):
        return ops.add(_c(a), _c(b))

    @staticmethod
    def backward(ctx, g):
        return g, g


def add(a, b):
    return AddFn.apply(a, b)


class FanOutFn(torch.autograd.Function):

    @staticmethod
    def forward(ctx, x, k, slot):
        ctx.k, ctx.slot = k, slot
        ctx.set_materialize_grads(False)
        return tuple(x.view_as(x) for _ in range(k))

    @staticmethod
    def backward(ctx, *grads):
        ctx.slot.buf = None
        gs, seen = [], set()
        for g in grads:
            if g is not None and (g.data_ptr(), g.numel()) not in seen:
                seen.add((g.data_ptr(), g.numel()))
                gs.append(g)
        if not gs:
            return None, None, None
        if len(gs) > 1 and len(gs) <= 8 and not all(g.is_contiguous() for g in gs) and all(_row_strided(g) for g in gs):
            return ops.add_n_rows(gs), None, None
        gs = [_c(g) for g in gs]
        out = gs[0]
        for i in range(0, len(gs) - 1, 7):
            out = ops.add_n([out] + gs[1 + i:8 + i]) if len(gs) > 1 else out
        return out, None, None


def _row_strided(g):
    if g.dim() < 2 or g.stride(-1) != 1 or g.shape[-1] % 4 or g.data_ptr() % 16 or g.stride(-2) % 4:
        return False
    st, sh = g.stride(), g.shape
    return all(st[i] == st[i + 1] * sh[i + 1] for i in range(len(sh) - 2))


def fanout(x, k):
    if k == 1 or not (torch.is_grad_enabled() and x.requires_grad):
        return (x,) * k
# ... 184 lines not shown
        ctx.N = N
        ctx.le_ref = level_embed
        return out

    @staticmethod
    def backward(ctx, d_pos):
        geo, N = ctx.geo, ctx.N
        d_pos = _c(d_pos)
        C = d_pos.shape[-1]
        pg = _ParamGrads((ctx.le_ref,))
        for l in range(geo.L):
            h, w = geo.shapes[l]
            ops.colsum(d_pos[0, geo.starts[l]:], h * w, C, pg.bufs[0][l], nbatch=N, batch_stride=geo.S * C)
        return (None,) + pg.result() + (None,) * geo.L


def level_pos(geo, level_embed, masks_u8):
    return LevelPosFn.apply(geo, level_embed, *masks_u8)


class MSDAFn(torch.autograd.Function):
    @staticmethod
    def forward(ctx, value, offw, ref, geo, P):
        value, offw, ref = _c(value), _c(offw), _c(ref)
        N, Lq = offw.shape[0], offw.shape[1]
        out = ops.msda_fwd(value, offw, ref, geo, N, Lq, P)
        ctx.save_for_backward(value, offw, ref)
        ctx.meta = (geo, N, Lq, P)
        return out

    @staticmethod
    def backward(ctx, d_out):
        value, offw, ref = ctx.saved_tensors
        geo, N, Lq, P = ctx.meta
        dv, do, dr = ops.msda_bwd(_c(d_out), value, offw, ref, geo, N, Lq, P, need_ref_grad=ctx.needs_input_grad[2])
        return dv, do, dr, None, None


def msda(value, offw, ref, geo, P=4):
    return MSDAFn.apply(value, offw, ref, geo, P)


def _from_row(t, r):
    return t if (t is None or r == 0) else t[r:]


def _col_blocks(groups, bufs, C):
    return [buf[..., j * C:(j + 1) * C] for (_, w, *_), buf in zip(groups, bufs) for j in range(w)]


class MHAFn(torch.autograd.Function):

    @staticmethod
    def forward(ctx, q_in, k_in, v_in, in_w, in_b, out_w, out_b, nheads, mask_mode, kpm_u8, dropout_p, rng_stream):
        ins = q_in, k_in, v_in = _c(q_in), _c(k_in), _c(v_in)
        N, Lq, C = q_in.shape
        Lk = k_in.shape[1]
        dev = q_in.device
        scale = (C // nheads) ** -0.5
        rng = Runtime.get_rng(dev) if dropout_p > 0 else None
        ctx.route = ops.attn_route(N, nheads, Lq, Lk, flash=False)
        if ctx.route != "mm" and k_in is v_in:
            layout = ((0, 3),) if q_in is k_in else ((0, 1), (1, 2))
        else:
            layout = ((0, 1), (1, 1), (2, 1))
        ctx.groups = tuple((r, w, r != 1 and ins[r] is k_in) for r, w in layout)
        bufs = [torch.empty(N, ins[r].shape[1], w * C, dtype=torch.float32, device=dev) for r, w in layout]
        for (r, w), buf in zip(layout, bufs):
            ops.gemm(ins[r].view(-1, C), _from_row(in_w, r * C), buf, N * ins[r].shape[1], w * C, C, bias=_from_row(in_b, r * C))
        q, k, v = _col_blocks(layout, bufs, C)
        O, saved = ops.attn_core_fwd(ctx.route, q, k, v, N, nheads, Lq, Lk, scale, mask_mode=mask_mode, kpm=kpm_u8, dropout_p=dropout_p,
                                     rng=rng, rng_stream=rng_stream)
        out = torch.empty(N, Lq, C, dtype=torch.float32, device=dev)
        ops.gemm(O.view(-1, C), out_w, out, N * Lq, C, C, bias=out_b)
        ctx.save_for_backward(q_in, k_in, v_in, in_w, out_w, q, k, v, O, kpm_u8, *saved)
        ctx.refs = (in_w, in_b, out_w, out_b)
        ctx.slot_q = _slot_of(q_in)
        ctx.meta = (nheads, mask_mode, dropout_p, rng_stream, scale)
        return out

    @staticmethod
    def backward(ctx, d_out):
        q_in, k_in, v_in, in_w, out_w, q, k, v, O, kpm, *saved = ctx.saved_tensors
        nheads, mask_mode, p, stream, scale = ctx.meta
        ins = q_in, k_in, v_in
        N, Lq, C = q_in.shape
        Lk = k_in.shape[1]
        dev = d_out.device
        d_out2 = _c(d_out).view(-1, C)
        Mq = N * Lq
        dO = torch.empty(Mq, C, dtype=torch.float32, device=dev)
        ops.gemm(d_out2, out_w, dO, Mq, C, C, a_mode=0, b_mode=1)
        pg = _ParamGrads(ctx.refs)
        d_in_w, d_in_b, d_out_w, d_out_b = pg.bufs
        with pg.side(d_out2, O):
            pg.gemm(d_out2, O.view(-1, C), d_out_w, C, C, Mq, a_mode=1, b_mode=1, accumulate=True,
                    split_k=ops.pick_split_k(C, C, Mq), colsum_out=d_out_b)
        dbufs = [torch.empty(N, ins[r].shape[1], w * C, dtype=torch.float32, device=dev) for r, w, _ in ctx.groups]
        dq, dk, dv = _col_blocks(ctx.groups, dbufs, C)
        rng = Runtime.get_rng(dev) if p > 0 else None
        ops.attn_core_bwd(ctx.route, saved, dO.view(N, Lq, C), q, k, v, O, dq, dk, dv, N, nheads, Lq, Lk, scale, mask_mode=mask_mode,
                          kpm=kpm, dropout_p=p, rng=rng, rng_stream=stream)
        pairs = list(zip(ctx.groups, dbufs))
        with pg.side(*dbufs, q_in, k_in, v_in):
            for (r, w, _), g in pairs:
                M = N * ins[r].shape[1]
                pg.gemm(g.view(-1, w * C), ins[r].view(-1, C), _from_row(d_in_w, r * C), w * C, C, M, a_mode=1, b_mode=1, lda=w * C,
                        accumulate=True, split_k=ops.pick_split_k(w * C, C, M), colsum_out=_from_row(d_in_b, r * C))
        d_in_w, d_in_b, d_out_w, d_out_b = pg.result()
        d_ins, dk_in = [None, None, None], None
        for (r, w, dup), g in pairs[1:] + pairs[:1]:
            live = [j for j in range(r, r + w) if ctx.needs_input_grad[j]]
            if not live:
                continue
            if dup and dk_in is not None:
                dst, acc = dk_in, True
            else:
                if r == 0 and len(pairs) == 2:
                    dst, acc = _grad_target(ctx.slot_q, ins[r].shape, dev)
                else:
                    dst, acc = torch.empty(ins[r].shape, dtype=torch.float32, device=dev), False
                d_ins[live[0]] = dst
            ops.gemm(g.view(-1, w * C), _from_row(in_w, r * C), dst, N * ins[r].shape[1], C, w * C, a_mode=0, b_mode=1, accumulate=acc)
            if live[0] == 1:
                dk_in = dst
        return (*d_ins, d_in_w, d_in_b, d_out_w, d_out_b, None, None, None, None, None)


class DecSelfAttnFn(torch.autograd.Function):

    @staticmethod
    def forward(ctx, tgt, pos, wq, wk, wv, in_w, in_b, out_w, out_b, nheads, dropout_p, rng_stream):
        N, L, C = tgt.shape
        M = N * L
        dev = tgt.device
        x, pos2 = _c(tgt).view(M, C), _c(pos).view(M, C)
        stacked = _adjacent(wq, wk) and _adjacent(wk, wv)
        qkv1 = torch.empty(M, 3 * C, dtype=torch.float32, device=dev)
        if stacked:
            ops.gemm(x, torch.as_strided(wq, (3 * C, C), (C, 1)), qkv1, M, 3 * C, C, residual=pos2, ldr=C, res_cols=C)
        else:
            ops.gemm(x, wq, qkv1, M, C, C, ldc=3 * C, residual=pos2, ldr=C)
            ops.gemm(x, wk, qkv1[:, C:], M, C, C, ldc=3 * C)
            ops.gemm(x, wv, qkv1[:, 2 * C:], M, C, C, ldc=3 * C)
        qkv2 = torch.empty(N, L, 3 * C, dtype=torch.float32, device=dev)
        ops.gemm(qkv1, in_w, qkv2, M, C, C, lda=3 * C, ldb=C, ldc=3 * C, bias=in_b,
                 batch=(3, 3, 0, C, 0, C * C, 0, C), bias_strides=(0, C))
        q, k, v = qkv2[..., :C], qkv2[..., C:2 * C], qkv2[..., 2 * C:]
        scale = (C // nheads) ** -0.5
        rng = Runtime.get_rng(dev) if dropout_p > 0 else None
        ctx.route = ops.attn_route(N, nheads, L, L, flash=True)
        O, saved = ops.attn_core_fwd(ctx.route, q, k, v, N, nheads, L, L, scale, mask_mode=1, dropout_p=dropout_p, rng=rng,
                                     rng_stream=rng_stream)
        out = torch.empty(N, L, C, dtype=torch.float32, device=dev)
        ops.gemm(O.view(M, C), out_w, out, M, C, C, bias=out_b)
        ctx.save_for_backward(x, wq, wk, wv, in_w, out_w, qkv1, qkv2, O, *saved)
        ctx.refs = (wq, wk, wv, in_w, in_b, out_w, out_b)
        ctx.meta = (nheads, dropout_p, rng_stream, scale, stacked, N, L, C)
        ctx.slot = _slot_of(tgt)
        return out

    @staticmethod
    def backward(ctx, d_out):
        x, wq, wk, wv, in_w, out_w, qkv1, qkv2, O, *saved = ctx.saved_tensors
        nheads, p, stream, scale, stacked, N, L, C = ctx.meta
        M = N * L
        dev = d_out.device
        d_out2 = _c(d_out).view(M, C)
        dO = torch.empty(M, C, dtype=torch.float32, device=dev)
        ops.gemm(d_out2, out_w, dO, M, C, C, a_mode=0, b_mode=1)
        dqkv2 = torch.empty(N, L, 3 * C, dtype=torch.float32, device=dev)
        dq, dk, dv = dqkv2[..., :C], dqkv2[..., C:2 * C], dqkv2[..., 2 * C:]
        q, k, v = qkv2[..., :C], qkv2[..., C:2 * C], qkv2[..., 2 * C:]
        rng = Runtime.get_rng(dev) if p > 0 else None
        ops.attn_core_bwd(ctx.route, saved, dO.view(N, L, C), q, k, v, O, dq, dk, dv, N, nheads, L, L, scale, mask_mode=1, dropout_p=p,
                          rng=rng, rng_stream=stream)
        dqkv1 = torch.empty(M, 3 * C, dtype=torch.float32, device=dev)
        ops.gemm(dqkv2.view(M, 3 * C), in_w, dqkv1, M, C, C, a_mode=0, b_mode=1, lda=3 * C, ldb=C, ldc=3 * C,
                 batch=(3, 3, 0, C, 0, C * C, 0, C))
        need_x, need_pos = ctx.needs_input_grad[0], ctx.needs_input_grad[1]
        dx = None
        if need_x:
            dx, acc = _grad_target(ctx.slot, (N, L, C), dev)
            if stacked:
                ops.gemm(dqkv1, torch.as_strided(wq, (3 * C, C), (C, 1)), dx, M, C, 3 * C, a_mode=0, b_mode=1, accumulate=acc)
            else:
                for i, w in enumerate((wq, wk, wv)):
                    ops.gemm(dqkv1[:, i * C:], w, dx, M, C, C, a_mode=0, b_mode=1, lda=3 * C, accumulate=acc or i > 0)

        pg = _ParamGrads(ctx.refs)
        d_wq, d_wk, d_wv, d_in_w, d_in_b, d_out_w, d_out_b = pg.bufs
        with pg.side(d_out2, O, dqkv2, qkv1, dqkv1, x):
            Mv = dqkv2.view(M, 3 * C)
            pg.gemm(d_out2, O.view(M, C), d_out_w, C, C, M, a_mode=1, b_mode=1, accumulate=True, split_k=ops.pick_split_k(C, C, M),
                    colsum_out=d_out_b)
            for i, dw in enumerate((d_wq, d_wk, d_wv)):
                pg.gemm(Mv[:, i * C:], qkv1[:, i * C:], d_in_w[i * C:], C, C, M, a_mode=1, b_mode=1, lda=3 * C, ldb=3 * C, accumulate=True,
                        split_k=ops.pick_split_k(C, C, M), colsum_out=d_in_b[i * C:])
                pg.gemm(dqkv1[:, i * C:], x, dw, C, C, M, a_mode=1, b_mode=1, lda=3 * C, ldb=C, accumulate=True,
                        split_k=ops.pick_split_k(C, C, M))
        dpos = dqkv1[:, :C].view(N, L, C) if need_pos else None
        return (dx, dpos) + pg.result() + (None, None, None)


def dec_self_attn(tgt, pos, wq, wk, wv, in_w, in_b, out_w, out_b, nheads=8, dropout_p=0.0, rng_stream=0):
    return DecSelfAttnFn.apply(tgt, pos, wq, wk, wv, in_w, in_b, out_w, out_b, nheads, float(dropout_p), int(rng_stream))


def mha(q_in, k_in, v_in, in_w, in_b, out_w, out_b, nheads=8, mask_mode=0, kpm_u8=None, dropout_p=0.0, rng_stream=0):
    return MHAFn.apply(q_in, k_in, v_in, in_w, in_b, out_w, out_b, nheads, mask_mode, kpm_u8, float(dropout_p), int(rng_stream))


class TokenEmbedFn(torch.autograd.Function):
    @staticmethod
    def forward(ctx, table, pad_idx, s11, s21, s12, s22, dx1, dx2, dy1, dy2):
        shape = s11.shape
        seqs = [_c(s).view(-1) for s in (s11, s21, s12, s22)]
        deltas = [_c(d).view(-1) for d in (dx1, dx2, dy1, dy2)]
        out = ops.token_embed_fwd(table, seqs, deltas)
        ctx.save_for_backward(*seqs, *deltas)
        ctx.t_ref = table
        ctx.meta = (table.shape, pad_idx)
        return out.view(*shape, table.shape[1])

    @staticmethod
    def backward(ctx, d_out):
        sv = ctx.saved_tensors
        tshape, pad_idx = ctx.meta
        pg = _ParamGrads((ctx.t_ref,))
        ops.token_embed_bwd(_c(d_out).view(-1, tshape[1]), sv[:4], sv[4:], pg.bufs[0], pad_idx if pad_idx is not None else -1)
        return pg.result() + (None,) * 9


def token_embed(table, pad_idx, s11, s21, s12, s22, dx1, dx2, dy1, dy2):
    return TokenEmbedFn.apply(table, pad_idx, s11, s21, s12, s22, dx1, dx2, dy1, dy2)


class QuerySineFn(torch.autograd.Function):
    @staticmethod
    def forward(ctx, ref):
        ref = _c(ref)
        ctx.save_for_backward(ref)
        return ops.query_sine_fwd(ref).view(*ref.shape[:-1], 256)

    @staticmethod
    def backward(ctx, d_out):
        (ref,) = ctx.saved_tensors
        return ops.query_sine_bwd(_c(d_out).view(-1, 256), ref).view_as(ref)


def query_sine(ref):
    return QuerySineFn.apply(ref)


class RefineFn(torch.autograd.Function):
    @staticmethod
    def forward(ctx, delta, ref):
        delta, ref = _c(delta), _c(ref)
        out = ops.refine_fwd(delta, ref)
        ctx.save_for_backward(out, ref)
        return out

    @staticmethod
# ... 236 lines not shown
```

### category-agnostic-pose-estimation_amd/hip/lib.py

```python
import ctypes
import os

import torch

from ctypes import POINTER, c_char_p, c_float, c_int, c_int32, c_int64, c_longlong, c_size_t, c_uint32, c_uint64, c_uint8, c_void_p

_HERE = os.path.dirname(os.path.abspath(__file__))
LIB_PATH = os.environ.get("CAPE_HIP_LIB", os.path.join(_HERE, "..", "csrc", "libcape_hip.so"))
LIB_PATH = os.path.abspath(LIB_PATH)

if not os.path.exists(LIB_PATH):
    raise ImportError(
        f"libcape_hip.so not found at {LIB_PATH}; build it with `python -c 'import __graft_entry__ as g; g.build()'` "
        "(or `make -C category-agnostic-pose-estimation_amd/csrc`).  There is no CPU fallback.")
try:
    _lib = ctypes.CDLL(LIB_PATH)
except OSError as e:
    raise ImportError(f"cannot load {LIB_PATH}: {e}") from e

_lib.cape_last_error.restype = c_char_p
_lib.cape_abi_version.restype = c_int


class GemmDesc(ctypes.Structure):
    _fields_ = [
        ("M", c_int), ("N", c_int), ("K", c_int), ("a_mode", c_int), ("b_mode", c_int),
        ("A", c_void_p), ("lda", c_longlong), ("B", c_void_p), ("ldb", c_longlong), ("C", c_void_p), ("ldc", c_longlong),
        ("cN", c_int), ("cH", c_int), ("cW", c_int), ("cC", c_int), ("cKH", c_int), ("cKW", c_int),
        ("cStride", c_int), ("cPad", c_int), ("cOH", c_int), ("cOW", c_int), ("cO", c_int),
        ("scale", c_void_p), ("bias", c_void_p), ("residual", c_void_p), ("ldr", c_longlong),
        ("relu", c_int), ("accumulate", c_int), ("split_k", c_int), ("dropout_p", c_float),
        ("rng_state", c_void_p), ("rng_stream", c_uint32), ("colsum_out", c_void_p), ("precision", c_int),
        ("B_packed", c_void_p),
        ("mask_src", c_void_p), ("ldm", c_longlong), ("mask_scale", c_float),
        ("batch", c_int), ("batch_div", c_int), ("sA0", c_longlong), ("sA1", c_longlong), ("sB0", c_longlong), ("sB1", c_longlong),
        ("sC0", c_longlong), ("sC1", c_longlong),
        ("res_cols", c_int), ("sBias0", c_longlong), ("sBias1", c_longlong),
        ("cPadX", c_int), ("cKHp", c_int), ("cKWp", c_int), ("cTapH0", c_int), ("cTapHS", c_int), ("cTapW0", c_int), ("cTapWS", c_int),
    ]


class PackItem(ctypes.Structure):
    _fields_ = [("B", c_void_p), ("out", c_void_p), ("ldb", c_longlong), ("N", c_int), ("K", c_int), ("b_mode", c_int), ("pad", c_int)]


class DecodeLinearDesc(ctypes.Structure):
    _fields_ = [
        ("N", c_int), ("K", c_int), ("Nout", c_int),
        ("X", c_void_p), ("ldx", c_longlong), ("in_gamma", c_void_p), ("in_beta", c_void_p), ("in_add", c_void_p), ("ld_add", c_longlong),
        ("W", c_void_p), ("ldw", c_longlong), ("bias", c_void_p),
        ("X2", c_void_p), ("ldx2", c_longlong), ("K2", c_int), ("W2", c_void_p), ("ldw2", c_longlong), ("n2", c_int),
        ("R", c_void_p), ("ldr", c_longlong), ("res_gamma", c_void_p), ("res_beta", c_void_p),
        ("relu", c_int), ("nseg", c_int), ("seg", c_int), ("out", c_void_p * 3), ("ldo", c_longlong * 3),
    ]


class DecodeTailDesc(ctypes.Structure):
    _fields_ = [
        ("N", c_int), ("L", c_int),
        ("P4", c_void_p), ("ldp", c_longlong), ("g3", c_void_p), ("b3", c_void_p),
        ("W1", c_void_p), ("B1", c_void_p), ("W2", c_void_p), ("B2", c_void_p), ("W3", c_void_p), ("B3", c_void_p),
        ("ref", c_void_p),
        ("Wc", c_void_p), ("Bc", c_void_p), ("ncls", c_int),
        ("Wp", c_void_p), ("Bp", c_void_p), ("gp", c_void_p), ("bp", c_void_p),
        ("dim_t", c_void_p), ("vr", c_void_p),
        ("ref_out", c_void_p), ("ld_ref", c_longlong),
        ("qpos_out", c_void_p), ("refin_out", c_void_p),
        ("cls_out", c_void_p), ("ld_cls", c_longlong),
        ("hs_out", c_void_p), ("ld_hs", c_longlong),
    ]


class AugItem(ctypes.Structure):
    _fields_ = [("src", c_void_p), ("aug", c_void_p), ("out", c_void_p), ("stat", c_void_p), ("h", c_int), ("w", c_int),
                ("M", c_float * 6), ("color_on", c_int), ("order", c_int * 4),
                ("bright", c_float), ("contrast", c_float), ("sat", c_float), ("hue", c_float),
                ("mode", c_int), ("noise_std", c_float), ("seed", c_uint32), ("blur_k", c_int), ("blur_w", c_float * 49)]


DECODE_MAX_LAYERS = 8
GEMM_GROUP_MAX = 32
SUMSQ_PARTS = 256


class DecodeLayerDesc(ctypes.Structure):
    _fields_ = [(n, c_void_p) for n in (
        "w_qkv", "b_qkv", "w_qin", "k_cache", "v_cache", "w_o", "b_o", "ln2_g", "ln2_b",
        "w_sq", "b_sq", "sup_k", "sup_v", "sup_mask", "w_so", "b_so", "lns_g", "lns_b",
        "w_off", "b_off", "value", "w_mo", "b_mo", "ln1_g", "ln1_b",
        "w1", "b1", "w2", "b2", "ln3_g", "ln3_b", "m1w", "m1b", "m2w", "m2b", "m3w", "m3b")]

# ... 36 lines not shown
    "cape_flash_attn_bwd": [P, P, P, P, P, P, P, P, P, P, LL, LL, LL, LL, LL, LL, LL, LL, I, I, I, I, F, I, I, P, F, P, U32, P],
    "cape_attn_softmax_fwd": [P, P, P, I, I, I, I, F, I, I, P, F, P, U32, P],
    "cape_attn_softmax_bwd": [P, P, I, I, I, I, F, F, P, U32, P],
    "cape_add_f32": [P, P, P, LL, P],
    "cape_level_embed_add": [P, P, P, P, I, I, I, I, P],
    "cape_add_n_f32": [POINTER(c_void_p), I, P, LL, P],
    "cape_add_n_rows_f32": [POINTER(c_void_p), POINTER(c_longlong), I, P, LL, LL, I, P],
    "cape_augment_batch": [P, I, I, I, P, P, P],
    "cape_gelu_f32": [P, P, LL, P],
    "cape_support_masks": [P, P, P, I, I, I, P],
    "cape_interleave2x2_f32": [POINTER(c_void_p), P, P, I, I, I, I, P],
    "cape_gelu_bwd_f32": [P, P, P, LL, P],
    "cape_scale_residual_bwd_f32": [P, P, P, P, P, LL, I, P],
    "cape_scale_residual_f32": [P, P, P, P, LL, I, P],
    "cape_nchw_to_nhwc": [P, P, I, I, I, I, I, P],
    "cape_bn_fold": [P, P, P, P, F, P, P, I, P],
    "cape_maxpool3x3s2_nhwc": [P, P, I, I, I, I, P],
    "cape_bn_relu_bwd": [P, P, P, P, P, LL, I, I, P],
    "cape_affine_act_f32": [P, P, P, P, LL, I, I, P],
    "cape_relu_drop_bwd": [P, P, P, LL, F, P],
    "cape_pos_sine_level": [P, P, P, P, LL, I, I, I, I, P],
    "cape_token_embed_fwd": [P, P, P, P, P, P, P, P, P, P, LL, I, I, P],
    "cape_token_embed_bwd": [P, P, P, P, P, P, P, P, P, P, LL, I, I, I, P],
    "cape_query_sine_fwd": [P, P, P, LL, P],
    "cape_query_sine_bwd": [P, P, P, P, I, LL, P],
    "cape_refine_fwd": [P, P, P, LL, P],
    "cape_refine_bwd": [P, P, P, P, P, I, LL, P],
    "cape_sigmoid_fwd": [P, P, LL, P],
    "cape_sigmoid_bwd": [P, P, P, I, LL, P],
    "cape_ref_scale_fwd": [P, P, P, LL, I, I, P],
    "cape_ref_scale_bwd": [P, P, P, I, LL, I, I, P],
    "cape_support_embed_fwd": [P, P, P, P, P, P, P, I, I, I, P],
    "cape_support_embed_bwd": [P, P, P, P, P, I, I, I, P],
    "cape_adjacency": [P, P, P, P, I, I, P],
    "cape_gcn_aggregate_fwd": [P, P, P, I, I, I, P],
    "cape_gcn_aggregate_bwd": [P, P, P, P, I, I, I, P],
    "cape_zero_rows": [P, P, LL, I, P],
    "cape_legacy_coord_embed_fwd": [P, P, P, P, I, I, P],
    "cape_legacy_coord_embed_bwd": [P, P, P, P, P, P, P, I, I, P],
    "cape_support_edge_info_fwd": [P, P, P, P, LL, P, P, P, I, I, I, P],
    "cape_support_edge_info_bwd": [P, LL, P, P, P, I, I, P],
    "cape_pe_dropout_fwd": [P, P, P, I, I, I, F, P, U32, P],
    "cape_pe_dropout_bwd": [P, P, LL, F, P, U32, P],
    "cape_loss_fwd_bwd": [P, P, P, P, P, P, F, F, F, P, P, P, P, I, LL, P],
    "cape_sumsq": [P, LL, P, P],
    "cape_adamw_step": [P, P, P, P, LL, F, F, F, F, F, F, P, I, P, P, P],
    "cape_step_increment": [P, P],
    "cape_decode_next_tokens": [P, P, P, P, P, P, I, I, I, I, I, I, P],
    "cape_decode_advance": [P, LL, P, LL, P, P, P, I, I, I, I, I, I, I, P, I, I, P, P, P],
    "cape_decode_linear": [POINTER(DecodeLinearDesc), P],
    "cape_decode_tail": [POINTER(DecodeTailDesc), P],
    "cape_decode_step": [POINTER(DecodeStepDesc), P],
}
EXPORTS = ["cape_last_error", "cape_abi_version", "cape_groupnorm_workspace_bytes", "cape_packed_weight_bytes"] + list(_SIGS)
_lib.cape_packed_weight_bytes.argtypes = [I, I]
_lib.cape_packed_weight_bytes.restype = c_size_t
_lib.cape_groupnorm_workspace_bytes.argtypes = [I, I, I]
_lib.cape_groupnorm_workspace_bytes.restype = c_size_t

for _name, _args in _SIGS.items():
    _fn = getattr(_lib, _name)
    _fn.argtypes = _args
    _fn.restype = c_int


def last_error() -> str:
    return _lib.cape_last_error().decode()


def abi_version() -> int:
    return _lib.cape_abi_version()


def call(name, *args):
    rc = getattr(_lib, name)(*args)
    if rc != 0:
        raise RuntimeError(f"{name} failed: {last_error()}")


def raw():
    return _lib
```

### category-agnostic-pose-estimation_amd/hip/ops.py

```python
import ctypes
import math
import os
import weakref

import torch

from . import lib

_F32 = torch.float32


_raw_stream = getattr(torch._C, "_cuda_getCurrentRawStream", None)
_raw_device = getattr(torch._C, "_cuda_getDevice", None)


_side = [None]


def raw_current_stream():
    if _raw_stream is not None and _raw_device is not None:
        return _raw_stream(_raw_device())
    return torch.cuda.current_stream().cuda_stream


# ... 143 lines not shown

    @classmethod
    def _pack(cls, es):
        dev = es[0]["buf"].device
        tab = cls._items(es).to(dev)
        lib.call("cape_pack_weights", _p(tab), len(es), 16, _stream())
        es[0].setdefault("_keep", None)
        es[0]["_keep"] = tab

    @classmethod
    def invalidate_and_repack(cls):
        cls.epoch += 1
        if not cls.enabled or not cls.entries:
            return
        dead = [k for k, e in cls.entries.items() if e["base"]() is None]
        if dead and not torch.cuda.is_current_stream_capturing():
            for k in dead:
                del cls.entries[k]
            cls._table = None
        es = list(cls.entries.values())
        if not es:
            return
        if cls._table is None or cls._table[1] != len(es):
            if torch.cuda.is_current_stream_capturing():
                raise RuntimeError("PackedWeights: new weights were registered inside a graph capture")
            cls._table = (cls._items(es).to(es[0]["buf"].device), len(es))
        lib.call("cape_pack_weights", _p(cls._table[0]), len(es), 16, _stream())
        for e in es:
            b = e["base"]()
            e["epoch"], e["version"] = cls.epoch, (b._version if b is not None else -1)

    @classmethod
    def signature(cls):
        return tuple(cls.entries.keys())

    @classmethod
    def mark_repacked(cls):
        cls.epoch += 1
        for e in cls.entries.values():
            b = e["base"]()
            e["epoch"], e["version"] = cls.epoch, (b._version if b is not None else -1)

    @classmethod
    def clear(cls):
        cls.entries, cls._table = {}, None


def gemm(*args, **kw):
    launch_gemm(gemm_desc(*args, **kw)[0])


def gemm_desc(A, B, C, M, N, K, a_mode=0, b_mode=0, lda=None, ldb=None, ldc=None, bias=None, scale=None, residual=None,
              ldr=None, relu=False, accumulate=False, split_k=1, dropout_p=0.0, rng=None, rng_stream=0, conv=None,
              colsum_out=None, packed=None, mask_src=None, mask_scale=1.0, batch=None, res_cols=0, bias_strides=None, conv_sub=None):
    for t, n in ((A, "A"), (B, "B"), (C, "C"), (bias, "bias"), (scale, "scale"), (residual, "residual")):
        _chk(t, "gemm." + n, contiguous=False)
    if (_AUTO_SPLIT_NN and a_mode == 0 and b_mode == 1 and split_k == 1 and K >= 512 and M > 64 and batch is None and conv is None
            and bias is None and scale is None and residual is None and not relu and mask_src is None and dropout_p == 0.0
            and colsum_out is None and (ldc is None or ldc == N) and C.is_contiguous() and ((M + 63) // 64) * ((N + 63) // 64) <= 64):
        sk = pick_split_k(M, N, K)
        if sk >= 4 and _avail(C) >= M * N:
            if not accumulate:
                C.view(-1)[:M * N].zero_()
            split_k, accumulate = sk, True
    d = lib.GemmDesc()
    d.M, d.N, d.K, d.a_mode, d.b_mode = M, N, K, a_mode, b_mode
    d.A, d.B, d.C = A.data_ptr(), B.data_ptr(), C.data_ptr()
    d.lda = lda if lda is not None else (K if a_mode == 0 else M)
    d.ldb = ldb if ldb is not None else (K if b_mode == 0 else N)
    d.ldc = ldc if ldc is not None else N
    if conv is not None:
        (d.cN, d.cH, d.cW, d.cC, d.cKH, d.cKW, d.cStride, d.cPad, d.cOH, d.cOW, d.cO) = conv
        if conv_sub is not None:
            (d.cPadX, d.cKHp, d.cKWp, d.cTapH0, d.cTapHS, d.cTapW0, d.cTapWS) = conv_sub
            assert a_mode == 3 and b_mode == 2 and _avail(B) >= d.cO * d.cKHp * d.cKWp * d.cC
            assert _avail(A) >= d.cN * d.cOH * d.cOW * d.cO and _avail(C) >= d.cN * d.cH * d.cW * d.cC
    d.scale = scale.data_ptr() if scale is not None else None
    d.bias = bias.data_ptr() if bias is not None else None
    d.residual = residual.data_ptr() if residual is not None else None
    d.ldr = ldr if ldr is not None else N
    d.res_cols = int(res_cols)
    d.relu, d.accumulate, d.split_k = int(relu), int(accumulate), int(split_k)
    d.dropout_p = float(dropout_p)
    d.rng_state = rng.t.data_ptr() if (rng is not None and dropout_p > 0) else None
    d.rng_stream = rng_stream
    d.precision = GEMM_PRECISION
    if (packed is None and PackedWeights.enabled and GEMM_PRECISION >= 1 and a_mode == 0 and b_mode in (0, 1) and batch is None
            and split_k == 1 and K in (64, 128, 256) and M > 64 and 32 <= N <= _PACK_MAX_N):
        packed = PackedWeights.lookup(B, N, K, d.ldb, b_mode)
    if packed is not None and GEMM_PRECISION >= 1:
        assert packed.dtype == torch.int16 and packed.is_cuda and packed.numel() * 2 >= lib.raw().cape_packed_weight_bytes(N, K)
        d.B_packed = packed.data_ptr()
    if mask_src is not None:
        _chk(mask_src, "gemm.mask_src")
        assert mask_src.numel() == M * N and split_k == 1
        d.mask_src, d.ldm, d.mask_scale = mask_src.data_ptr(), N, float(mask_scale)
    if colsum_out is not None:
        _chk(colsum_out, "gemm.colsum_out", contiguous=False)
        assert a_mode == 1 and _avail(colsum_out) >= M
        d.colsum_out = colsum_out.data_ptr()
    if batch is not None:
        cnt, div, sA0, sA1, sB0, sB1, sC0, sC1 = batch
        assert cnt >= 1 and div >= 1 and cnt % div == 0
        d.batch, d.batch_div = cnt, div
        d.sA0, d.sA1, d.sB0, d.sB1, d.sC0, d.sC1 = sA0, sA1, sB0, sB1, sC0, sC1
        if bias_strides is not None:
            d.sBias0, d.sBias1 = bias_strides
            assert bias is not None and _avail(bias) >= (cnt // div - 1) * d.sBias0 + (div - 1) * d.sBias1 + N
        last0, last1 = cnt // div - 1, div - 1
        offA, offB, offC = last0 * sA0 + last1 * sA1, last0 * sB0 + last1 * sB1, last0 * sC0 + last1 * sC1
    else:
        offA = offB = offC = 0
    if a_mode == 0 and M > 0:
        assert _avail(A) >= offA + (M - 1) * d.lda + K, "gemm: A too small"
    if a_mode == 1 and K > 0:
        assert _avail(A) >= offA + (K - 1) * d.lda + M, "gemm: A^T too small"
    if b_mode == 0 and N > 0:
        assert _avail(B) >= offB + (N - 1) * d.ldb + K, "gemm: B too small"
    if b_mode == 1 and K > 0:
        assert _avail(B) >= offB + (K - 1) * d.ldb + N, "gemm: B too small"
    if M > 0:
        assert _avail(C) >= offC + (M - 1) * d.ldc + N, "gemm: C too small"
    if residual is not None:
        assert res_cols % 32 == 0 and 0 <= res_cols <= N
        assert _avail(residual) >= (M - 1) * d.ldr + (res_cols or N), "gemm: residual too small"
    if bias is not None:
        assert _avail(bias) >= N
    if scale is not None:
        assert scale.numel() >= N
    return d, (A, B, C, colsum_out)


def launch_gemm(d):
    if GemmProfiler.enabled:
# ... 36 lines not shown

def gemm_group(descs, shapes, tile):
    n = len(descs)
    assert 1 <= n <= lib.GEMM_GROUP_MAX
    arr = (lib.GemmDesc * n)(*descs)
    if GemmProfiler.enabled:
        e0, e1 = torch.cuda.Event(enable_timing=True), torch.cuda.Event(enable_timing=True)
        st = _stream()
        ext = torch.cuda.ExternalStream(st.value) if _side[0] is not None else None
        e0.record(ext)
        lib.call("cape_gemm_group_f32", arr, n, tile, st)
        e1.record(ext)
        fl = sum(2.0 * M * N * K for M, N, K, _, _ in shapes)
        by = sum(GemmProfiler.alg_bytes(M, N, K) for M, N, K, _, _ in shapes)
        GemmProfiler.records.append((e0, e1, fl, ("group", tile, shapes[0][4], n), by, n))
        return
    lib.call("cape_gemm_group_f32", arr, n, tile, _stream())


def colsum(X, M, N, out, ldx=None, accumulate=True, nbatch=1, batch_stride=0):
    _chk(X, "colsum.X", contiguous=False)
    _chk(out, "colsum.out", contiguous=False)
    ldx = N if ldx is None else ldx
    assert M == 0 or _avail(X) >= (nbatch - 1) * batch_stride + (M - 1) * ldx + N
    assert _avail(out) >= N
    lib.call("cape_colsum_f32", _p(X), ldx, nbatch, batch_stride, M, N, _p(out), int(accumulate), _stream())


def add_layernorm_fwd(x, y, gamma, beta, pos=None, dropout_p=0.0, rng=None, rng_stream=0):
    C = x.shape[-1]
    rows = x.numel() // C
    for t, n in ((x, "x"), (y, "y"), (gamma, "gamma"), (beta, "beta"), (pos, "pos")):
        _chk(t, "ln." + n)
    if y is not None:
        assert y.shape == x.shape
    if pos is not None:
        assert pos.numel() == x.numel()
    out = torch.empty_like(x)
    mean = torch.empty(rows, dtype=_F32, device=x.device)
    rstd = torch.empty(rows, dtype=_F32, device=x.device)
    out_pos = torch.empty_like(x) if pos is not None else None
    lib.call("cape_add_layernorm_fwd", _p(x), _p(y), _p(gamma), _p(beta), _p(out), _p(mean), _p(rstd), _p(pos),
             _p(out_pos), rows, C, float(dropout_p), rng.ptr if (rng is not None and dropout_p > 0) else None,
             rng_stream, _stream())
    return out, mean, rstd, out_pos


def add_layernorm_bwd(d_out, d_out_pos, x, y, gamma, mean, rstd, dgamma, dbeta, dropout_p=0.0, rng=None, rng_stream=0):
    C = x.shape[-1]
    rows = x.numel() // C
    for t, n in ((d_out, "d_out"), (d_out_pos, "d_out_pos"), (x, "x"), (y, "y"), (dgamma, "dgamma"), (dbeta, "dbeta")):
        _chk(t, "ln_bwd." + n)
    d_x = torch.empty_like(x)
    d_y = torch.empty_like(x) if (y is not None and dropout_p > 0) else None
    lib.call("cape_add_layernorm_bwd", _p(d_out), _p(d_out_pos), _p(x), _p(y), _p(gamma), _p(mean), _p(rstd), _p(d_x),
             _p(d_y), _p(dgamma), _p(dbeta), rows, C, float(dropout_p),
             rng.ptr if (rng is not None and dropout_p > 0) else None, rng_stream, _stream())
    return d_x, (d_y if d_y is not None else d_x)


def _gn_workspace(N, C, G, device):
    nbytes = lib.raw().cape_groupnorm_workspace_bytes(N, C, G)
    return torch.empty((nbytes + 7) // 8, dtype=torch.float64, device=device), nbytes


def groupnorm_fwd(x, gamma, beta, out, out_image_stride, N, HW, C, G=32):
    for t, n in ((x, "x"), (gamma, "gamma"), (beta, "beta")):
        _chk(t, "gn." + n)
    _chk(out, "gn.out", contiguous=False)
    assert x.numel() == N * HW * C
    mean = torch.empty(N * G, dtype=_F32, device=x.device)
    rstd = torch.empty(N * G, dtype=_F32, device=x.device)
    ws, nbytes = _gn_workspace(N, C, G, x.device)
    lib.call("cape_groupnorm_fwd", _p(x), _p(gamma), _p(beta), _p(out), out_image_stride, _p(mean), _p(rstd), N, HW, C, G,
             _p(ws), nbytes, _stream())
    return mean, rstd


def groupnorm_bwd(d_out, d_out_image_stride, x, gamma, mean, rstd, dgamma, dbeta, N, HW, C, G=32):
    _chk(d_out, "gn_bwd.d_out", contiguous=False)
    d_x = torch.empty_like(x)
    ws, nbytes = _gn_workspace(N, C, G, x.device)
    lib.call("cape_groupnorm_bwd", _p(d_out), d_out_image_stride, _p(x), _p(gamma), _p(mean), _p(rstd), _p(d_x),
             _p(dgamma), _p(dbeta), N, HW, C, G, _p(ws), nbytes, _stream())
    return d_x


class LevelGeometry:

    def __init__(self, shapes):
        self.shapes = [(int(h), int(w)) for h, w in shapes]
        self.L = len(self.shapes)
        starts, s = [], 0
        for h, w in self.shapes:
            starts.append(s)
            s += h * w
        self.S = s
        self.starts = starts
        self._shapes_c = (ctypes.c_int * (2 * self.L))(*[v for hw in self.shapes for v in hw])
        self._starts_c = (ctypes.c_int * self.L)(*starts)


def msda_fwd(value, offw, ref, geo, N, Lq, P=4):
    for t, n in ((value, "value"), (offw, "offw"), (ref, "ref")):
        _chk(t, "msda." + n)
    assert value.numel() == N * geo.S * 256 and offw.numel() == N * Lq * 8 * geo.L * P * 3
    assert ref.numel() == N * Lq * geo.L * 2
# ... 791 lines not shown
```

### category-agnostic-pose-estimation_amd/models/deformable_transformer.py

```python
import copy
import math

import torch
from torch import nn
from torch.nn.init import constant_, xavier_uniform_

from ..hip import functional as HF
from ..hip import ops


def _get_clones(module, N):
    return nn.ModuleList([copy.deepcopy(module) for _ in range(N)])


class MSDeformAttn(nn.Module):

    def __init__(self, d_model=256, n_levels=4, n_heads=8, n_points=4):
        super().__init__()
        if d_model != 256 or n_heads != 8:
            raise ValueError("the MI355X MSDA kernel is specialised to d_model=256, 8 heads x 32 channels")
        if n_levels * n_points > 16 or n_levels > 4:
            raise ValueError("n_levels * n_points must be <= 16 and n_levels <= 4")
        self.im2col_step = 64
        self.d_model, self.n_levels, self.n_heads, self.n_points = d_model, n_levels, n_heads, n_points
        self.sampling_offsets = nn.Linear(d_model, n_heads * n_levels * n_points * 2)
        self.attention_weights = nn.Linear(d_model, n_heads * n_levels * n_points)
        self.value_proj = nn.Linear(d_model, d_model)
        self.output_proj = nn.Linear(d_model, d_model)
        self._reset_parameters()

    def _reset_parameters(self):
        constant_(self.sampling_offsets.weight.data, 0.0)
        thetas = torch.arange(self.n_heads, dtype=torch.float32) * (2.0 * math.pi / self.n_heads)
        grid = torch.stack([thetas.cos(), thetas.sin()], -1)
        grid = (grid / grid.abs().max(-1, keepdim=True)[0]).view(self.n_heads, 1, 1, 2).repeat(1, self.n_levels, self.n_points, 1)
        for i in range(self.n_points):
            grid[:, :, i, :] *= i + 1
        with torch.no_grad():
            self.sampling_offsets.bias.copy_(grid.view(-1))
        constant_(self.attention_weights.weight.data, 0.0)
        constant_(self.attention_weights.bias.data, 0.0)
        xavier_uniform_(self.value_proj.weight.data)
        constant_(self.value_proj.bias.data, 0.0)
        xavier_uniform_(self.output_proj.weight.data)
        constant_(self.output_proj.bias.data, 0.0)

    def project_value(self, input_flatten, padding_rows_u8=None):
        value = HF.linear(input_flatten, self.value_proj.weight, self.value_proj.bias)
        if padding_rows_u8 is not None:
            value = HF.zero_rows(value, padding_rows_u8)
        return value

    def forward(self, query, reference_points, input_flatten, geo, padding_rows_u8=None, value=None):
        if reference_points.shape[-1] != 2:
            raise ValueError("Last dim of reference_points must be 2 (box references are not on the CAPE path)")
        assert geo.S == input_flatten.shape[1]
        if value is None:
            value = self.project_value(input_flatten, padding_rows_u8)
        offw = HF.linear_cat2(query, self.sampling_offsets.weight, self.sampling_offsets.bias,
                              self.attention_weights.weight, self.attention_weights.bias)
        out = HF.msda(value, offw, reference_points, geo, self.n_points)
        return HF.linear(out, self.output_proj.weight, self.output_proj.bias)


class DeformableTransformerEncoderLayer(nn.Module):
    def __init__(self, d_model=256, d_ffn=1024, dropout=0.1, activation="relu", n_levels=4, n_heads=8, n_points=4):
        super().__init__()
        if activation != "relu":
            raise ValueError("only relu is fused in the GEMM epilogue (reference default)")
        self.self_attn = MSDeformAttn(d_model, n_levels, n_heads, n_points)
        self.dropout1 = nn.Dropout(dropout)
        self.norm1 = nn.LayerNorm(d_model)
        self.linear1 = nn.Linear(d_model, d_ffn)
        self.dropout2 = nn.Dropout(dropout)
        self.linear2 = nn.Linear(d_ffn, d_model)
        self.dropout3 = nn.Dropout(dropout)
        self.norm2 = nn.LayerNorm(d_model)
        self._streams = [ops.new_stream_id() for _ in range(3)]

    def forward(self, src, src_pos, pos, reference_points, geo, padding_rows_u8=None):
        p = self.dropout1.p if self.training else 0.0
        src_v, src_r = HF.fanout(src, 2)
        a = self.self_attn(src_pos, reference_points, src_v, geo, padding_rows_u8)
        src = HF.add_layernorm(src_r, a, self.norm1.weight, self.norm1.bias, dropout_p=p, rng_stream=self._streams[0])
        src_f, src_r = HF.fanout(src, 2)
        h = HF.ffn(src_f, self.linear1.weight, self.linear1.bias, self.linear2.weight, self.linear2.bias, dropout_p=p,
                   rng_stream=self._streams[1])
        return HF.add_layernorm(src_r, h, self.norm2.weight, self.norm2.bias, pos=pos, dropout_p=p, rng_stream=self._streams[2])


_REF_POINTS = {}


class DeformableTransformerEncoder(nn.Module):
    def __init__(self, encoder_layer, num_layers):
        super().__init__()
        self.layers = _get_clones(encoder_layer, num_layers)
        for layer in self.layers:
            layer._streams = [ops.new_stream_id() for _ in range(3)]
        self.num_layers = num_layers

    @staticmethod
    def get_reference_points(geo, valid_ratios, device):
        pts = []
        for lvl, (H_, W_) in enumerate(geo.shapes):
            ref_y, ref_x = torch.meshgrid(torch.linspace(0.5, H_ - 0.5, H_, dtype=torch.float32, device=device),
                                          torch.linspace(0.5, W_ - 0.5, W_, dtype=torch.float32, device=device), indexing="ij")
            ref_y = ref_y.reshape(-1)[None] / (valid_ratios[:, None, lvl, 1] * H_)
            ref_x = ref_x.reshape(-1)[None] / (valid_ratios[:, None, lvl, 0] * W_)
            pts.append(torch.stack((ref_x, ref_y), -1))
        ref = torch.cat(pts, 1)
        return (ref[:, :, None] * valid_ratios[:, None]).contiguous()

    def forward(self, src, geo, valid_ratios, pos, padding_rows_u8=None):
        with torch.no_grad():
            if padding_rows_u8 is None:
                key = (tuple(geo.shapes), src.shape[0], str(src.device))
                reference_points = _REF_POINTS.get(key)
                if reference_points is None:
                    reference_points = _REF_POINTS[key] = self.get_reference_points(geo, valid_ratios, src.device)
            else:
                reference_points = self.get_reference_points(geo, valid_ratios, src.device)
        poss = HF.fanout(pos, len(self.layers) + 1)
        output, src0 = HF.fanout(src, 2)
        out_pos = HF.add(src0, poss[0])
        for layer, pos_l in zip(self.layers, poss[1:]):
            output, out_pos = layer(output, out_pos, pos_l, reference_points, geo, padding_rows_u8)
        return output
```

### category-agnostic-pose-estimation_amd/models/deformable_transformer_v2.py

```python
import copy
import math
import os

import numpy as np
import torch
from torch import nn
from torch.nn.init import normal_

from ..hip import functional as HF
from ..hip import ops
from .deformable_transformer import (DeformableTransformerEncoder, DeformableTransformerEncoderLayer, MSDeformAttn)
from ..util.misc import cached_zero_mask
from .kv_cache import KVCache, VCache

_ONES_VR = {}
_FUSED_SELF_ATTN = os.environ.get("CAPE_DEC_SELF_ATTN_NODE", "1") == "1"


def Embedding(num_embeddings, embedding_dim, padding_idx=None, zero_init=False):
    m = nn.Embedding(num_embeddings, embedding_dim, padding_idx=padding_idx)
    nn.init.normal_(m.weight, mean=0, std=embedding_dim ** -0.5)
    if padding_idx is not None:
        nn.init.constant_(m.weight[padding_idx], 0)
    if zero_init:
        nn.init.constant_(m.weight, 0)
    return m


def get_1d_sincos_pos_embed_from_grid(embed_dim, seq_len):
    pos = np.arange(seq_len, dtype=np.float32)
    omega = 1.0 / 10000 ** (np.arange(embed_dim // 2, dtype=np.float64) / (embed_dim / 2.0))
    out = np.einsum("m,d->md", pos.reshape(-1), omega)
    return np.concatenate([np.sin(out), np.cos(out)], axis=1)


class TransformerDecoderLayer(nn.Module):

    def __init__(self, d_model=256, d_ffn=1024, dropout=0.1, activation="relu", n_levels=4, n_heads=8, n_points=4,
                 use_qkv_proj=True):
        super().__init__()
        if activation != "relu" or not use_qkv_proj:
            raise ValueError("CAPE path: relu FFN and dec_qkv_proj=True (reference defaults)")
        self.d_model, self.n_heads = d_model, n_heads
        self.attn_q = nn.Linear(d_model, d_model, bias=False)
        self.attn_k = nn.Linear(d_model, d_model, bias=False)
        self.attn_v = nn.Linear(d_model, d_model, bias=False)
        self.self_attn = nn.MultiheadAttention(d_model, n_heads, dropout=dropout)
        self.dropout2 = nn.Dropout(dropout)
        self.norm2 = nn.LayerNorm(d_model)
        self.support_attn = nn.MultiheadAttention(d_model, n_heads, dropout=dropout, batch_first=True)
        self.dropout_support = nn.Dropout(dropout)
        self.norm_support = nn.LayerNorm(d_model)
        self.cross_attn = MSDeformAttn(d_model, n_levels, n_heads, n_points)
        self.dropout1 = nn.Dropout(dropout)
        self.norm1 = nn.LayerNorm(d_model)
        self.linear1 = nn.Linear(d_model, d_ffn)
        self.dropout3 = nn.Dropout(dropout)
        self.linear2 = nn.Linear(d_ffn, d_model)
        self.dropout4 = nn.Dropout(dropout)
        self.norm3 = nn.LayerNorm(d_model)
        self.kv_cache = None
        self._streams = [ops.new_stream_id() for _ in range(8)]

    def forward(self, tgt, query_pos, reference_points, src, geo, padding_rows_u8=None, support_features=None,
                support_kpm_u8=None):
        p = self.dropout2.p if self.training else 0.0
        st = self._streams
        sa = self.self_attn
        qp_q, qp_s = HF.fanout(query_pos, 2)
        if _FUSED_SELF_ATTN:
            t_a, t_r = HF.fanout(tgt, 2)
            t2 = HF.dec_self_attn(t_a, qp_q, self.attn_q.weight, self.attn_k.weight, self.attn_v.weight, sa.in_proj_weight,
                                  sa.in_proj_bias, sa.out_proj.weight, sa.out_proj.bias, self.n_heads, dropout_p=p, rng_stream=st[0])
        else:
            t_q, t_k, t_v, t_r = HF.fanout(tgt, 4)
            q = HF.linear(t_q, self.attn_q.weight, residual=qp_q)
            k = HF.linear(t_k, self.attn_k.weight)
            v = HF.linear(t_v, self.attn_v.weight)
            t2 = HF.mha(q, k, v, sa.in_proj_weight, sa.in_proj_bias, sa.out_proj.weight, sa.out_proj.bias, self.n_heads,
                        mask_mode=1, dropout_p=p, rng_stream=st[0])
        tgt = HF.add_layernorm(t_r, t2, self.norm2.weight, self.norm2.bias, dropout_p=p, rng_stream=st[1])
        if support_features is not None:
            ca = self.support_attn
            t_q, t_r = HF.fanout(tgt, 2)
            t2 = HF.mha(t_q, support_features, support_features, ca.in_proj_weight, ca.in_proj_bias, ca.out_proj.weight,
                        ca.out_proj.bias, self.n_heads, mask_mode=2 if support_kpm_u8 is not None else 0,
                        kpm_u8=support_kpm_u8, dropout_p=p, rng_stream=st[2])
            tgt, tgt_pos = HF.add_layernorm(t_r, t2, self.norm_support.weight, self.norm_support.bias, pos=qp_s,
                                            dropout_p=p, rng_stream=st[3])
        else:
            tgt, t_r = HF.fanout(tgt, 2)
            tgt_pos = HF.add(t_r, qp_s)
        t2 = self.cross_attn(tgt_pos, reference_points, src, geo, padding_rows_u8)
        tgt = HF.add_layernorm(tgt, t2, self.norm1.weight, self.norm1.bias, dropout_p=p, rng_stream=st[4])
        t_f, t_r = HF.fanout(tgt, 2)
        h = HF.ffn(t_f, self.linear1.weight, self.linear1.bias, self.linear2.weight, self.linear2.bias, dropout_p=p, rng_stream=st[5])
        return HF.add_layernorm(t_r, h, self.norm3.weight, self.norm3.bias, dropout_p=p, rng_stream=st[6])

    @torch.no_grad()
    def decode_step(self, tgt, query_pos, reference_points, geo, step, cache):
        C, H = self.d_model, self.n_heads
        N = tgt.shape[0]
        sa = self.self_attn
        W, B = sa.in_proj_weight, sa.in_proj_bias
        dev = tgt.device
        t2d = tgt.view(N, C)
        tmp = torch.empty(3, N, C, dtype=torch.float32, device=dev)
        ops.gemm(t2d, self.attn_q.weight, tmp[0], N, C, C, residual=query_pos.view(N, C))
        ops.gemm(t2d, self.attn_k.weight, tmp[1], N, C, C)
        ops.gemm(t2d, self.attn_v.weight, tmp[2], N, C, C)
        q = torch.empty(N, 1, C, dtype=torch.float32, device=dev)
        ops.gemm(tmp[0], W, q, N, C, C, bias=B)
        max_len = cache["k"].shape[1]
        ops.gemm(tmp[1], W[C:], cache["k"][:, step], N, C, C, bias=B[C:], ldc=max_len * C)
        ops.gemm(tmp[2], W[2 * C:], cache["v"][:, step], N, C, C, bias=B[2 * C:], ldc=max_len * C)
        Lk = step + 1
        O, _ = ops.attn_fwd(q, cache["k"], cache["v"], N, H, 1, Lk, (C // H) ** -0.5, mask_mode=0)
        t2 = torch.empty(N, 1, C, dtype=torch.float32, device=dev)
        ops.gemm(O.view(N, C), sa.out_proj.weight, t2, N, C, C, bias=sa.out_proj.bias)
        tgt, _, _, _ = ops.add_layernorm_fwd(tgt, t2, self.norm2.weight, self.norm2.bias)
        tgt_pos = None
        if cache.get("sup_k") is not None:
            ca = self.support_attn
            ops.gemm(tgt.view(N, C), ca.in_proj_weight, q, N, C, C, bias=ca.in_proj_bias)
            P = cache["sup_k"].shape[1]
            O, _ = ops.attn_fwd(q, cache["sup_k"], cache["sup_v"], N, H, 1, P, (C // H) ** -0.5,
                                mask_mode=2 if cache["sup_kpm"] is not None else 0, kpm=cache["sup_kpm"])
            ops.gemm(O.view(N, C), ca.out_proj.weight, t2, N, C, C, bias=ca.out_proj.bias)
            tgt, _, _, tgt_pos = ops.add_layernorm_fwd(tgt, t2, self.norm_support.weight, self.norm_support.bias, pos=query_pos)
        else:
            tgt_pos = ops.add(tgt, query_pos)
        m = self.cross_attn
        LP3 = m.n_heads * m.n_levels * m.n_points
        offw = torch.empty(N, 1, 3 * LP3, dtype=torch.float32, device=dev)
        ops.gemm(tgt_pos.view(N, C), m.sampling_offsets.weight, offw, N, 2 * LP3, C, bias=m.sampling_offsets.bias, ldc=3 * LP3)
        ops.gemm(tgt_pos.view(N, C), m.attention_weights.weight, offw.view(N, -1)[:, 2 * LP3:], N, LP3, C,
                 bias=m.attention_weights.bias, ldc=3 * LP3)
        a = ops.msda_fwd(cache["value"], offw, reference_points, geo, N, 1, m.n_points)
        ops.gemm(a.view(N, C), m.output_proj.weight, t2, N, C, C, bias=m.output_proj.bias)
        tgt, _, _, _ = ops.add_layernorm_fwd(tgt, t2, self.norm1.weight, self.norm1.bias)
        F_ = self.linear1.weight.shape[0]
        h = torch.empty(N, F_, dtype=torch.float32, device=dev)
        ops.gemm(tgt.view(N, C), self.linear1.weight, h, N, F_, C, bias=self.linear1.bias, relu=True)
        ops.gemm(h, self.linear2.weight, t2, N, C, F_, bias=self.linear2.bias)
        tgt, _, _, _ = ops.add_layernorm_fwd(tgt, t2, self.norm3.weight, self.norm3.bias)
        return tgt


class TransformerDecoder(nn.Module):
    def __init__(self, decoder_layer, num_layers, poly_refine=True, return_intermediate=False, aux_loss=False,
# ... 180 lines not shown
```

### category-agnostic-pose-estimation_amd/models/geometric_support_encoder.py

```python
from typing import List

import torch
import torch.nn as nn

from ..hip import functional as HF
from ..hip import ops
from .graph_utils import GCNLayer, adj_from_skeleton
from .positional_encoding import PositionalEncoding1D, SinePositionalEncoding2D


class GeometricSupportEncoder(nn.Module):
    def __init__(self, hidden_dim: int = 256, num_encoder_layers: int = 3, nhead: int = 8, dim_feedforward: int = 1024,
                 dropout: float = 0.1, use_gcn_preenc: bool = False, num_gcn_layers: int = 2, activation: str = "relu"):
        super().__init__()
        if activation != "relu" or hidden_dim != 256 or nhead != 8:
            raise ValueError("MI355X kernels: relu, hidden_dim=256, 8 heads (reference defaults)")
        self.hidden_dim = hidden_dim
        self.use_gcn_preenc = use_gcn_preenc
        self.nhead = nhead
        self.coord_mlp = nn.Sequential(nn.Linear(2, hidden_dim), nn.ReLU(), nn.Linear(hidden_dim, hidden_dim))
        self.pos_encoding = SinePositionalEncoding2D(num_feats=hidden_dim // 2, temperature=10000, normalize=True,
                                                     scale=2 * 3.14159265359)
        self.sequence_pos_encoding = PositionalEncoding1D(d_model=hidden_dim, max_len=100, dropout=0.0)
        if use_gcn_preenc:
            self.gcn_layers = nn.ModuleList([GCNLayer(hidden_dim, hidden_dim, kernel_size=2, use_bias=True,
                                                      activation=nn.ReLU(inplace=True), batch_first=True)
                                             for _ in range(num_gcn_layers)])
        else:
            self.gcn_layers = None
        layer = nn.TransformerEncoderLayer(d_model=hidden_dim, nhead=nhead, dim_feedforward=dim_feedforward,
                                           dropout=dropout, activation="relu", batch_first=True)
        self.transformer_encoder = nn.TransformerEncoder(layer, num_layers=num_encoder_layers)
        self.dropout_p = dropout
        self._streams = [[ops.new_stream_id() for _ in range(4)] for _ in range(num_encoder_layers)]

    def forward(self, support_coords: torch.Tensor, support_mask: torch.Tensor, skeleton_edges: List) -> torch.Tensor:
        bs, num_pts, _ = support_coords.shape
        if num_pts > 100:
            raise RuntimeError("more keypoints than PositionalEncoding1D.max_len=100")
        support_mask = support_mask.bool()
        mask_u8 = ops.as_u8(support_mask)
        m0, m2 = self.coord_mlp[0], self.coord_mlp[2]
        h, pe = HF.support_embed(support_coords, m0.weight, m0.bias, self.sequence_pos_encoding.pe[0].contiguous())
        x = HF.linear(h, m2.weight, m2.bias, residual=pe)
        if self.use_gcn_preenc and self.gcn_layers is not None:
            if skeleton_edges is None:
                skeleton_edges = [[] for _ in range(bs)]
            adj = adj_from_skeleton(num_pts, skeleton_edges, mask_u8, support_coords.device)
            for g in self.gcn_layers:
                x = g(x, adj)
        fast = False
        if (not self.training) and (not torch.is_grad_enabled()):
            valid = (~support_mask).to(torch.int8)
            valid[:, 0] |= support_mask.all(dim=1).to(torch.int8)
            fast = bool(((valid[:, 1:] - valid[:, :-1]) <= 0).all())
        kpm, zero_u8 = ops.support_masks(mask_u8, pad_rows=fast)
        p = self.dropout_p if self.training else 0.0
        for li, layer in enumerate(self.transformer_encoder.layers):
            sa, st = layer.self_attn, self._streams[li]
            x_a, x_r = HF.fanout(x, 2)
            a = HF.mha(x_a, x_a, x_a, sa.in_proj_weight, sa.in_proj_bias, sa.out_proj.weight, sa.out_proj.bias, self.nhead,
                       mask_mode=2, kpm_u8=kpm, dropout_p=p, rng_stream=st[0])
            x = HF.add_layernorm(x_r, a, layer.norm1.weight, layer.norm1.bias, dropout_p=p, rng_stream=st[1])
            x_f, x_r = HF.fanout(x, 2)
            hdn = HF.ffn(x_f, layer.linear1.weight, layer.linear1.bias, layer.linear2.weight, layer.linear2.bias, dropout_p=p,
                         rng_stream=st[2])
            x = HF.add_layernorm(x_r, hdn, layer.norm2.weight, layer.norm2.bias, dropout_p=p, rng_stream=st[3])
        x = HF.zero_rows(x, zero_u8.reshape(-1))
        return x

    def __repr__(self):
        gcn = f", use_gcn_preenc=True ({len(self.gcn_layers)} layers)" if self.use_gcn_preenc else ""
        return f"{self.__class__.__name__}(hidden_dim={self.hidden_dim}, spatial_pe=SinePE2D, sequence_pe=SinePE1D{gcn})"
```

### category-agnostic-pose-estimation_amd/models/support_encoder.py

```python
import math

import torch
import torch.nn as nn

from ..hip import functional as HF
from ..hip import ops
from .graph_utils import DeviceSkeleton, _edge_tables


class PositionalEncoding1D(nn.Module):

    def __init__(self, d_model, dropout=0.1, max_len=5000):
        super().__init__()
        self.dropout = nn.Dropout(p=dropout)
        pe = torch.zeros(max_len, d_model)
        position = torch.arange(0, max_len, dtype=torch.float).unsqueeze(1)
        div_term = torch.exp(torch.arange(0, d_model, 2).float() * (-math.log(10000.0) / d_model))
        pe[:, 0::2] = torch.sin(position * div_term)
        pe[:, 1::2] = torch.cos(position * div_term)
        self.register_buffer("pe", pe.unsqueeze(0))
        self._stream = ops.new_stream_id()

    def forward(self, x):
        if x.shape[1] > self.pe.shape[1]:
# ... 17 lines not shown
        layer = nn.TransformerEncoderLayer(d_model=hidden_dim, nhead=nheads, dim_feedforward=dim_feedforward, dropout=dropout,
                                           activation="relu", batch_first=True)
        self.transformer_encoder = nn.TransformerEncoder(layer, num_layers=num_encoder_layers)
        self.norm = nn.LayerNorm(hidden_dim)
        self._reset_parameters()
        self.dropout_p = dropout
        self._streams = [[ops.new_stream_id() for _ in range(4)] for _ in range(num_encoder_layers)]

    def _reset_parameters(self):
        for p in self.parameters():
            if p.dim() > 1:
                nn.init.xavier_uniform_(p)

    def _edge_tables(self, skeleton_edges, dev):
        if isinstance(skeleton_edges, DeviceSkeleton):
            return skeleton_edges.edges.contiguous(), skeleton_edges.start
        flat, start = [], [0]
        for edges in skeleton_edges:
            for e in (edges if edges is not None else []):
                if len(e) == 2:
                    flat.append((int(e[0]), int(e[1])))
            start.append(len(flat))
        return _edge_tables(flat, start, dev)[:2]

    def embed(self, support_coords, skeleton_edges=None):
        B, N, _ = support_coords.shape
        m0, m2 = self.coord_embedding[0], self.coord_embedding[2]
        h = HF.legacy_coord_embed(support_coords, m0.weight, m0.bias)
        if skeleton_edges is not None and len(skeleton_edges) > 0:
            if len(skeleton_edges) != B:
                raise ValueError(f"skeleton_edges holds {len(skeleton_edges)} graphs for a batch of {B}")
            edges, start = self._edge_tables(skeleton_edges, support_coords.device)
            cat = HF.edge_cat(h, m2.weight, m2.bias, self.edge_embedding.weight, edges, start)
            x = HF.linear(cat, self.coord_edge_proj.weight, self.coord_edge_proj.bias)
        else:
            x = HF.linear(h, m2.weight, m2.bias)
        return self.pos_embedding(x)

    def forward(self, support_coords, support_mask=None, skeleton_edges=None):
        B, N, _ = support_coords.shape
        x = self.embed(support_coords, skeleton_edges)
        kpm, mode = None, 0
        if support_mask is not None:
            kpm = ops.as_u8(~support_mask.bool())
            mode = 3
        fast = False
        if kpm is not None and (not self.training) and (not torch.is_grad_enabled()):
            valid = support_mask.bool().to(torch.int8)
            fast = bool(((valid[:, 1:] - valid[:, :-1]) <= 0).all())
        p = self.dropout_p if self.training else 0.0
        for li, layer in enumerate(self.transformer_encoder.layers):
            sa, st = layer.self_attn, self._streams[li]
            x_a, x_r = HF.fanout(x, 2)
            a = HF.mha(x_a, x_a, x_a, sa.in_proj_weight, sa.in_proj_bias, sa.out_proj.weight, sa.out_proj.bias, self.nheads,
                       mask_mode=mode, kpm_u8=kpm, dropout_p=p, rng_stream=st[0])
            x = HF.add_layernorm(x_r, a, layer.norm1.weight, layer.norm1.bias, dropout_p=p, rng_stream=st[1])
            x_f, x_r = HF.fanout(x, 2)
            hdn = HF.ffn(x_f, layer.linear1.weight, layer.linear1.bias, layer.linear2.weight, layer.linear2.bias, dropout_p=p,
                         rng_stream=st[2])
            x = HF.add_layernorm(x_r, hdn, layer.norm2.weight, layer.norm2.bias, dropout_p=p, rng_stream=st[3])
        if fast:
            x = HF.zero_rows(x, kpm.reshape(-1))
        return HF.add_layernorm(x, None, self.norm.weight, self.norm.bias)

    def __repr__(self):
        return f"{self.__class__.__name__}(hidden_dim={self.hidden_dim}, nheads={self.nheads}, edge_info=degree, sequence_pe=SinePE1D)"


def build_support_encoder(args):
    return SupportPoseGraphEncoder(hidden_dim=getattr(args, "hidden_dim", 256), nheads=getattr(args, "nheads", 8),
                                   num_encoder_layers=getattr(args, "support_encoder_layers", 3),
                                   dim_feedforward=getattr(args, "dim_feedforward", 1024), dropout=getattr(args, "dropout", 0.1))
```

### include/cape_hip.h

```cpp
#ifndef CAPE_HIP_H
#define CAPE_HIP_H

#include <stddef.h>
#include <stdint.h>

#ifdef __cplusplus
extern "C" {
#endif

typedef void* cape_stream_t;

const char* cape_last_error(void);
int cape_abi_version(void);

int cape_rng_advance(uint64_t* rng_state, cape_stream_t stream);

int cape_stream_fork(cape_stream_t main_stream, cape_stream_t side_stream);
int cape_stream_join(cape_stream_t main_stream, cape_stream_t side_stream);

typedef struct {
  int M, N, K;
  int a_mode, b_mode;
  const float* A; long long lda;
  const float* B; long long ldb;
  float* C; long long ldc;
  int cN, cH, cW, cC, cKH, cKW, cStride, cPad, cOH, cOW, cO;
  const float* scale;
  const float* bias;
  const float* residual;
  long long ldr;
  int relu;
  int accumulate;
  int split_k;
  float dropout_p;
  const uint64_t* rng_state;
  uint32_t rng_stream;
  float* colsum_out;
  int precision;
  const uint16_t* B_packed;
  const float* mask_src; long long ldm; float mask_scale;
  int batch, batch_div; long long sA0, sA1, sB0, sB1, sC0, sC1;
  int res_cols; long long sBias0, sBias1;
  int cPadX, cKHp, cKWp, cTapH0, cTapHS, cTapW0, cTapWS;
} cape_gemm_desc;

int cape_gemm_f32(const cape_gemm_desc* d, cape_stream_t stream);

#define CAPE_GEMM_GROUP_MAX 32
int cape_gemm_group_f32(const cape_gemm_desc* descs, int n, int tile, cape_stream_t stream);

typedef struct { const float* B; uint16_t* out; long long ldb; int N, K, b_mode, pad; } cape_pack_item;
size_t cape_packed_weight_bytes(int N, int K);
int cape_pack_weights(const cape_pack_item* items_dev, int n_items, int max_blocks_per_item, cape_stream_t stream);

int cape_colsum_f32(const float* X, long long ldx, int nbatch, long long batch_stride, int M, int N, float* out,
                    int accumulate, cape_stream_t stream);

typedef struct {
  int N, K, Nout;
  const float* X; long long ldx; const float* in_gamma; const float* in_beta; const float* in_add; long long ld_add;
  const float* W; long long ldw; const float* bias;
  const float* X2; long long ldx2; int K2; const float* W2; long long ldw2; int n2;
  const float* R; long long ldr; const float* res_gamma; const float* res_beta;
  int relu;
  int nseg, seg; float* out[3]; long long ldo[3];
} cape_decode_linear_desc;
int cape_decode_linear(const cape_decode_linear_desc* d, cape_stream_t stream);

typedef struct {
  int N, L;
  const float* P4; long long ldp; const float* g3; const float* b3;
  const float* W1; const float* B1; const float* W2; const float* B2; const float* W3; const float* B3;
  const float* ref;
  const float* Wc; const float* Bc; int ncls;
  const float* Wp; const float* Bp; const float* gp; const float* bp;
  const float* dim_t; const float* vr;
  float* ref_out; long long ld_ref;
  float* qpos_out; float* refin_out;
  float* cls_out; long long ld_cls;
  float* hs_out; long long ld_hs;
} cape_decode_tail_desc;
int cape_decode_tail(const cape_decode_tail_desc* d, cape_stream_t stream);

#define CAPE_DECODE_MAX_LAYERS 8
typedef struct {
  const float *w_qkv, *b_qkv;
  const float* w_qin;
  float *k_cache, *v_cache;
  const float *w_o, *b_o, *ln2_g, *ln2_b;
  const float *w_sq, *b_sq;
  const float *sup_k, *sup_v;
  const unsigned char* sup_mask;
  const float *w_so, *b_so, *lns_g, *lns_b;
  const float *w_off, *b_off;
  const float* value;
  const float *w_mo, *b_mo, *ln1_g, *ln1_b;
  const float *w1, *b1, *w2, *b2;
  const float *ln3_g, *ln3_b;
  const float *m1w, *m1b, *m2w, *m2b, *m3w, *m3b;
// ... 195 lines not shown
```

Measured before the change: 646.8 episodes/s.

## Fuse residual add and dropout into output-projection GEMM epilogues

Adds a res_post epilogue mode to the tiled and row-split GEMM kernels that applies bias, dropout, and the residual add after the projection. All transformer layers (encoder, decoder, support encoders) now route the out-projection and FFN second GEMM through a PostResidual helper, so the following add_layernorm only normalizes. This removes a separate elementwise read of the residual and the dropout pass in the layernorm kernels. The layernorm backward regenerates dropout keep-bits from the RNG instead of reading y. The cost is more epilogue complexity and tighter coupling of autograd gradient routing between the GEMM and the norm backward.

Result: no change. 646.3 episodes/s (-0.1%).

```diff
diff --git a/category-agnostic-pose-estimation_amd/csrc/error.hip b/category-agnostic-pose-estimation_amd/csrc/error.hip
--- a/category-agnostic-pose-estimation_amd/csrc/error.hip
+++ b/category-agnostic-pose-estimation_amd/csrc/error.hip
@@ -13,6 +13,7 @@
 
 extern "C" const char* cape_last_error(void) { return g_err; }
 extern "C" int cape_abi_version(void) { return 11; }
+extern "C" size_t cape_gemm_desc_bytes(void) { return sizeof(cape_gemm_desc); }
 
 __global__ void rng_advance_kernel(uint64_t* st) { st[1] += 1; }
 extern "C" int cape_rng_advance(uint64_t* rng_state, cape_stream_t stream) {
diff --git a/category-agnostic-pose-estimation_amd/csrc/gemm.hip b/category-agnostic-pose-estimation_amd/csrc/gemm.hip
--- a/category-agnostic-pose-estimation_amd/csrc/gemm.hip
+++ b/category-agnostic-pose-estimation_amd/csrc/gemm.hip
@@ -122,6 +122,11 @@
   p.bdiv = d->batch_div > 0 ? d->batch_div : 1;
   p.sA0 = d->sA0; p.sA1 = d->sA1; p.sB0 = d->sB0; p.sB1 = d->sB1; p.sC0 = d->sC0; p.sC1 = d->sC1;
   p.res_cols = d->res_cols; p.sBias0 = d->sBias0; p.sBias1 = d->sBias1;
+  p.res_post = d->res_post != 0;
+  if (d->res_post)
+    CAPE_REQUIRE(d->residual && !d->relu && !d->res_cols && !d->mask_src && !d->accumulate && d->split_k == 1 && d->batch <= 1 &&
+                     !d->colsum_out,
+                 "cape_gemm_f32: res_post needs a residual and allows only scale, bias and dropout besides it");
   if (d->cKHp > 0) {
     CAPE_REQUIRE(d->a_mode == 3 && d->b_mode == 2 && d->cStride == 1 && d->cO % 32 == 0 && d->K % 32 == 0 && d->cKWp > 0 &&
                      d->cTapHS >= 1 && d->cTapWS >= 1 && d->cTapH0 >= 0 && d->cTapW0 >= 0 &&
diff --git a/category-agnostic-pose-estimation_amd/csrc/gemm_common.h b/category-agnostic-pose-estimation_amd/csrc/gemm_common.h
--- a/category-agnostic-pose-estimation_amd/csrc/gemm_common.h
+++ b/category-agnostic-pose-estimation_amd/csrc/gemm_common.h
@@ -38,6 +38,7 @@
   int res_cols;
   long long sBias0, sBias1;
   int cPadX, cKHp, cKWp, cTapH0, cTapHS, cTapW0, cTapWS;
+  int res_post;
 };
 
 __device__ __forceinline__ float4 zero4() { return make_float4(0.f, 0.f, 0.f, 0.f); }
diff --git a/category-agnostic-pose-estimation_amd/csrc/gemm_group.hip b/category-agnostic-pose-estimation_amd/csrc/gemm_group.hip
--- a/category-agnostic-pose-estimation_amd/csrc/gemm_group.hip
+++ b/category-agnostic-pose-estimation_amd/csrc/gemm_group.hip
@@ -39,7 +39,7 @@
   p.tilesM = q.tilesM; p.tilesN = q.tilesN;
   p.Bpack = nullptr; p.mask_src = nullptr; p.ldm = 0; p.mask_scale = 1.f;
   p.bdiv = 1; p.sA0 = p.sA1 = p.sB0 = p.sB1 = p.sC0 = p.sC1 = 0;
-  p.res_cols = 0; p.sBias0 = p.sBias1 = 0; p.single = g.single;
+  p.res_cols = 0; p.res_post = 0; p.sBias0 = p.sBias1 = 0; p.single = g.single;
   gemm_tile_body<BM, BN, 1, BMODE, true, PREC, KFULL>(p, b - g.bstart[i]);
 }
 
diff --git a/category-agnostic-pose-estimation_amd/csrc/gemm_rs.hip b/category-agnostic-pose-estimation_amd/csrc/gemm_rs.hip
--- a/category-agnostic-pose-estimation_amd/csrc/gemm_rs.hip
+++ b/category-agnostic-pose-estimation_amd/csrc/gemm_rs.hip
@@ -72,9 +72,10 @@
   const float floor_v = p.relu ? 0.f : -__builtin_inff();
   uint64_t seed = 0, step = 0;
   if constexpr (EPI == 4) { seed = p.rng_state[0]; step = p.rng_state[1]; }
+  if constexpr (EPI == 5) { if (p.drop_thresh) { seed = p.rng_state[0]; step = p.rng_state[1]; } }
   const int ldc = (int)p.ldc;
   const unsigned lo_c = (unsigned)(4 * h * ldc + col);
-  const int ldx = EPI == 1 ? (int)p.ldr : ldc;
+  const int ldx = (EPI == 1 || EPI == 5) ? (int)p.ldr : ldc;
   const unsigned lo_x = (unsigned)(4 * h * ldx + col);
   const bool res_on = EPI != 1 || !p.res_cols || n0 < p.res_cols;
 
@@ -156,10 +157,10 @@
     for (int hh = 0; hh < H1; ++hh) {
       const int half = (NW == 8) ? hh : wm;
       float xv[16];
-      if constexpr (EPI >= 1 && EPI <= 3) {
+      if constexpr ((EPI >= 1 && EPI <= 3) || EPI == 5) {
         if (col_ok && res_on) {
           const int rb = u * RS_UNIT + 32 * half;
-          const float* xb = EPI == 1 ? p.residual : EPI == 2 ? p.mask_src : p.C;
+          const float* xb = (EPI == 1 || EPI == 5) ? p.residual : EPI == 2 ? p.mask_src : p.C;
           const float* x0 = xb + (long long)rb * ldx;
 #pragma unroll
           for (int i = 0; i < 16; ++i) {
@@ -212,6 +213,16 @@
           float v = fmaxf(fmaf(acc[i], sc, bi), floor_v);
           v = cape_keep(seed, step, p.rng_stream, (uint64_t)row * (uint64_t)p.N + col, p.drop_thresh) ? v * p.inv_keep : 0.f;
           if (roff < rlim) c0[lo_c + (unsigned)(roff * ldc)] = v;
+        }
+      } else if constexpr (EPI == 5) {
+        const bool drop = p.drop_thresh != 0;
+#pragma unroll
+        for (int i = 0; i < 16; ++i) {
+          const int roff = (i & 3) + 8 * (i >> 2);
+          const int row = rb + roff + 4 * h;
+          float v = fmaf(acc[i], sc, bi);
+          if (drop) v = cape_keep(seed, step, p.rng_stream, (uint64_t)row * (uint64_t)p.N + col, p.drop_thresh) ? __fmul_rn(v, p.inv_keep) : 0.f;
+          if (roff < rlim) c0[lo_c + (unsigned)(roff * ldc)] = xv[i] + v;
         }
       } else {
 #pragma unroll
@@ -236,6 +247,7 @@
 }
 
 static int rs_epi(const GemmP& p) {
+  if (p.res_post) return (p.mask_src || p.accumulate || p.relu || p.res_cols) ? -1 : 5;
   const int n = (p.residual != nullptr) + (p.mask_src != nullptr) + (p.accumulate != 0) + (p.drop_thresh != 0);
   if (n == 0) return 0;
   if (n > 1) return -1;
@@ -264,6 +276,7 @@
     case 2: return rs_launch_epi<NW, BMODE, KS, 2>(p, nchunks, gpc, s);
     case 3: return rs_launch_epi<NW, BMODE, KS, 3>(p, nchunks, gpc, s);
     case 4: return rs_launch_epi<NW, BMODE, KS, 4>(p, nchunks, gpc, s);
+    case 5: return rs_launch_epi<NW, BMODE, KS, 5>(p, nchunks, gpc, s);
   }
   return cape_set_error("cape_gemm_f32(rs): unsupported epilogue combination");
 }
diff --git a/category-agnostic-pose-estimation_amd/csrc/gemm_tile.h b/category-agnostic-pose-estimation_amd/csrc/gemm_tile.h
--- a/category-agnostic-pose-estimation_amd/csrc/gemm_tile.h
+++ b/category-agnostic-pose-estimation_amd/csrc/gemm_tile.h
@@ -558,15 +558,16 @@
   if (drop) { seed = p.rng_state[0]; step = p.rng_state[1]; }
   const bool atomic = p.split_k > 1;
   const bool interior = (m0 + BM <= p.M) && (n0 + BN <= p.N);
-  const int n_extra = (p.residual != nullptr) + (p.mask_src != nullptr) + (p.accumulate != 0) + (drop ? 1 : 0);
+  const bool post = p.res_post != 0;
+  const int n_extra = (p.residual != nullptr) + (p.mask_src != nullptr) + (p.accumulate != 0) + (drop && !post ? 1 : 0);
   const bool same_ld = (!p.residual || p.ldr == p.ldc) && (!p.mask_src || p.ldm == p.ldc);
-  if (interior && !drop && n_extra <= 1 && same_ld && (long long)BM * p.ldc < (1ll << 30)) {
+  if (interior && (!drop || post) && n_extra <= 1 && same_ld && (long long)BM * p.ldc < (1ll << 30)) {
     const int wave_s = __builtin_amdgcn_readfirstlane(wave);
     const int wm_s = wave_s >> 1, wn_s = wave_s & 1;
     const int ldc = (int)p.ldc;
     const float floor_v = p.relu ? 0.f : -INFINITY;
     const float* xb = p.residual ? p.residual : p.mask_src ? p.mask_src : (p.accumulate && !atomic) ? p.C : nullptr;
-    const int kind = atomic ? 1 : p.residual ? 2 : p.mask_src ? 3 : p.accumulate ? 4 : 0;
+    const int kind = atomic ? 1 : p.residual ? (post ? 5 : 2) : p.mask_src ? 3 : p.accumulate ? 4 : 0;
 #pragma unroll
     for (int i = 0; i < TI; ++i) {
 #pragma unroll
@@ -590,6 +591,17 @@
           float xv[16];
 #pragma unroll
           for (int r = 0; r < 16; ++r) xv[r] = x0[lo + (unsigned)(((r & 3) + 8 * (r >> 2)) * ldc)];
+          if (kind == 5) {
+            const int row0 = m0 + wm_s * WTM + i * 32 + 4 * lh;
+#pragma unroll
+            for (int r = 0; r < 16; ++r) {
+              const int roff = (r & 3) + 8 * (r >> 2);
+              float v = fmaf(acc[i][j][r], sc, bi);
+              if (drop) v = cape_keep(seed, step, p.rng_stream, (uint64_t)(row0 + roff) * (uint64_t)p.N + (colb + l31), p.drop_thresh) ? __fmul_rn(v, p.inv_keep) : 0.f;
+              c0[lo + (unsigned)(roff * ldc)] = xv[r] + v;
+            }
+            continue;
+          }
 #pragma unroll
           for (int r = 0; r < 16; ++r) {
             float v = fmaf(acc[i][j][r], sc, bi);
@@ -619,9 +631,10 @@
         float* cp = p.C + (long long)row * p.ldc + col;
         if (atomic) { atomicAdd(cp, split == 0 ? v + bi : v); continue; }
         v = v * sc + bi;
-        if (p.residual && (!p.res_cols || col < p.res_cols)) v += p.residual[(long long)row * p.ldr + col];
+        if (p.residual && !post && (!p.res_cols || col < p.res_cols)) v += p.residual[(long long)row * p.ldr + col];
         if (p.relu) v = fmaxf(v, 0.f);
-        if (drop) v = cape_keep(seed, step, p.rng_stream, (uint64_t)row * (uint64_t)p.N + col, p.drop_thresh) ? v * p.inv_keep : 0.f;
+        if (drop) v = cape_keep(seed, step, p.rng_stream, (uint64_t)row * (uint64_t)p.N + col, p.drop_thresh) ? (post ? __fmul_rn(v, p.inv_keep) : v * p.inv_keep) : 0.f;
+        if (post) v = p.residual[(long long)row * p.ldr + col] + v;
         if (p.mask_src) v = p.mask_src[(long long)row * p.ldm + col] != 0.f ? v * p.mask_scale : 0.f;
         if (p.accumulate) v += *cp;
         *cp = v;
diff --git a/category-agnostic-pose-estimation_amd/csrc/norm.hip b/category-agnostic-pose-estimation_amd/csrc/norm.hip
--- a/category-agnostic-pose-estimation_amd/csrc/norm.hip
+++ b/category-agnostic-pose-estimation_amd/csrc/norm.hip
@@ -131,6 +131,13 @@
             q.z = k2 ? q.z * inv_keep : 0.f; q.w = k3 ? q.w * inv_keep : 0.f;
           }
           v.x += q.x; v.y += q.y; v.z += q.z; v.w += q.w;
+        } else if (thresh) {
+          const uint64_t idx = (uint64_t)base + c;
+          const bool k0 = cape_keep(seed, step, rng_stream, idx + 0, thresh);
+          const bool k1 = cape_keep(seed, step, rng_stream, idx + 1, thresh);
+          const bool k2 = cape_keep(seed, step, rng_stream, idx + 2, thresh);
+          const bool k3 = cape_keep(seed, step, rng_stream, idx + 3, thresh);
+          keepbits |= ((uint32_t)k0 | ((uint32_t)k1 << 1) | ((uint32_t)k2 << 2) | ((uint32_t)k3 << 3)) << (4 * i);
         }
         float4 d = *reinterpret_cast<const float4*>(d_out + base + c);
         if (d_out_pos) {
@@ -234,6 +241,15 @@
           q.z = k2 ? q.z * inv_keep : 0.f; q.w = k3 ? q.w * inv_keep : 0.f;
         }
         v[k].x += q.x; v[k].y += q.y; v[k].z += q.z; v[k].w += q.w;
+      }
+    } else if (thresh) {
+#pragma unroll
+      for (int k = 0; k < LN256_R; ++k) {
+        const int row = min(r0 + k, rows - 1);
+        const uint64_t idx = (uint64_t)((long long)row * 256 + 4 * lane);
+        const bool k0 = cape_keep(seed, step, rng_stream, idx + 0, thresh), k1 = cape_keep(seed, step, rng_stream, idx + 1, thresh);
+        const bool k2 = cape_keep(seed, step, rng_stream, idx + 2, thresh), k3 = cape_keep(seed, step, rng_stream, idx + 3, thresh);
+        kb[k] = (uint32_t)k0 | ((uint32_t)k1 << 1) | ((uint32_t)k2 << 2) | ((uint32_t)k3 << 3);
       }
     }
     if (d_out_pos) {
@@ -394,8 +410,8 @@
                                       const uint64_t* rng_state, uint32_t rng_stream, cape_stream_t stream) {
   CAPE_REQUIRE(d_out && x && gamma && mean && rstd && d_x && dgamma && dbeta, "cape_add_layernorm_bwd: null pointer");
   CAPE_REQUIRE(C > 0 && C <= 1024 && (C % 4) == 0, "cape_add_layernorm_bwd: C=%d must be a multiple of 4, <= 1024", C);
-  CAPE_REQUIRE(dropout_p == 0.f || (y && d_y && d_y != d_x && rng_state && dropout_p < 1.f),
-               "cape_add_layernorm_bwd: dropout needs y, a separate d_y and rng_state");
+  CAPE_REQUIRE(dropout_p == 0.f || (d_y && d_y != d_x && rng_state && dropout_p < 1.f),
+               "cape_add_layernorm_bwd: dropout needs a separate d_y and rng_state");
   if (rows <= 0) return 0;
   const uint32_t th = dropout_p > 0.f ? cape_drop_threshold(dropout_p) : 0u;
   const float ik = dropout_p > 0.f ? 1.f / (1.f - dropout_p) : 1.f;
diff --git a/category-agnostic-pose-estimation_amd/hip/functional.py b/category-agnostic-pose-estimation_amd/hip/functional.py
--- a/category-agnostic-pose-estimation_amd/hip/functional.py
+++ b/category-agnostic-pose-estimation_amd/hip/functional.py
@@ -228,9 +228,29 @@
         slot.buf = buf
 
 
+class PostResidual:
+    __slots__ = ("x", "p", "stream", "dy")
+
+    def __init__(self, x, dropout_p=0.0, rng_stream=0):
+        self.x, self.p, self.stream, self.dy = x, float(dropout_p), int(rng_stream), None
+
+    def gemm(self, A, B, C, M, N, K, **kw):
+        x2 = _c(self.x).view(M, N)
+        rng = Runtime.get_rng(C.device) if self.p > 0 else None
+        ops.gemm(A, B, C, M, N, K, post_residual=x2, dropout_p=self.p, rng=rng, rng_stream=self.stream, **kw)
+
+    def grads(self, d_s, slot):
+        if self.p == 0:
+            return d_s, d_s
+        dy, self.dy = self.dy, None
+        assert dy is not None and dy.shape == d_s.shape, "PostResidual: the norm of this sum has not run its backward"
+        _slot_offer(slot, d_s)
+        return dy, d_s
+
+
 class LinearFn(torch.autograd.Function):
     @staticmethod
-    def forward(ctx, x, weight, bias, residual, relu, dropout_p, rng_stream):
+    def forward(ctx, x, weight, bias, residual, relu, dropout_p, rng_stream, post=None):
         K = x.shape[-1]
         N = weight.shape[0]
         assert weight.shape[1] == K and weight.stride(1) == 1
@@ -239,11 +259,15 @@
         res2 = _c(residual).view(-1, N) if residual is not None else None
         y = torch.empty(M, N, dtype=torch.float32, device=x.device)
         rng = Runtime.get_rng(x.device) if dropout_p > 0 else None
-        ops.gemm(x2, weight, y, M, N, K, ldb=weight.stride(0), bias=bias, residual=res2, relu=relu, dropout_p=dropout_p,
-                 rng=rng, rng_stream=rng_stream)
-        ctx.save_for_backward(x2, weight, y if (relu or dropout_p > 0) else None)
+        if post is not None:
+            post.gemm(x2, weight, y, M, N, K, ldb=weight.stride(0), bias=bias)
+        else:
+            ops.gemm(x2, weight, y, M, N, K, ldb=weight.stride(0), bias=bias, residual=res2, relu=relu, dropout_p=dropout_p,
+                     rng=rng, rng_stream=rng_stream)
+        ctx.save_for_backward(x2, weight, y if ((relu or dropout_p > 0) and post is None) else None)
         ctx.w_ref, ctx.b_ref = weight, bias
         ctx.slot = _slot_of(x)
+        ctx.post, ctx.slot_res = post, (_slot_of(residual) if post is not None else None)
         ctx.meta = (relu, dropout_p, bias is not None, residual is not None, x.shape, M, N, K)
         return y.view(*x.shape[:-1], N)
 
@@ -253,7 +277,10 @@
         relu, p, has_bias, has_res, xshape, M, N, K = ctx.meta
         dy2 = _c(dy).view(M, N)
         dpre = dy2
-        if relu or p > 0:
+        if ctx.post is not None:
+            dpre, dy = ctx.post.grads(dy, ctx.slot_res)
+            dpre = _c(dpre).view(M, N)
+        elif relu or p > 0:
             assert relu, "dropout epilogue is only used together with relu"
             dpre = ops.relu_drop_bwd(dy2, y, 1.0 / (1.0 - p) if p > 0 else 1.0)
         dx = None
@@ -270,17 +297,20 @@
             elif db is not None:
                 ops.colsum(dpre, M, N, db)
         dres = dy if (has_res and ctx.needs_input_grad[3]) else None
-        return (dx,) + pg.result() + (dres, None, None, None)
-
-
-def linear(x, weight, bias=None, residual=None, relu=False, dropout_p=0.0, rng_stream=0):
-    return LinearFn.apply(x, weight, bias, residual, relu, float(dropout_p), int(rng_stream))
+        return (dx,) + pg.result() + (dres, None, None, None, None)
+
+
+def linear(x, weight, bias=None, residual=None, relu=False, dropout_p=0.0, rng_stream=0, post=None):
+    if post is not None:
+        assert residual is None and not relu and dropout_p == 0.0
+        return LinearFn.apply(x, weight, bias, post.x, False, post.p, post.stream, post)
+    return LinearFn.apply(x, weight, bias, residual, relu, float(dropout_p), int(rng_stream), None)
 
 
 class FFNFn(torch.autograd.Function):
 
     @staticmethod
-    def forward(ctx, x, w1, b1, w2, b2, dropout_p, rng_stream):
+    def forward(ctx, x, w1, b1, w2, b2, dropout_p, rng_stream, res=None, post=None):
         K, Hd, N = x.shape[-1], w1.shape[0], w2.shape[0]
         x2 = _c(x).view(-1, K)
         M = x2.shape[0]
@@ -288,10 +318,14 @@
         h = torch.empty(M, Hd, dtype=torch.float32, device=x.device)
         ops.gemm(x2, w1, h, M, Hd, K, ldb=w1.stride(0), bias=b1, relu=True, dropout_p=dropout_p, rng=rng, rng_stream=rng_stream)
         y = torch.empty(M, N, dtype=torch.float32, device=x.device)
-        ops.gemm(h, w2, y, M, N, Hd, ldb=w2.stride(0), bias=b2)
+        if post is not None:
+            post.gemm(h, w2, y, M, N, Hd, ldb=w2.stride(0), bias=b2)
+        else:
+            ops.gemm(h, w2, y, M, N, Hd, ldb=w2.stride(0), bias=b2)
         ctx.save_for_backward(x2, w1, w2, h)
         ctx.refs = (w1, b1, w2, b2)
         ctx.slot = _slot_of(x)
+        ctx.post, ctx.slot_res = post, (_slot_of(res) if post is not None else None)
         ctx.meta = (dropout_p, x.shape, M, K, Hd, N)
         return y.view(*x.shape[:-1], N)
 
@@ -299,6 +333,9 @@
     def backward(ctx, dy):
         x2, w1, w2, h = ctx.saved_tensors
         p, xshape, M, K, Hd, N = ctx.meta
+        dres = None
+        if ctx.post is not None:
+            dy, dres = ctx.post.grads(dy, ctx.slot_res)
         dy2 = _c(dy).view(M, N)
         dpre = torch.empty(M, Hd, dtype=torch.float32, device=dy.device)
         ops.gemm(dy2, w2, dpre, M, Hd, N, a_mode=0, b_mode=1, ldb=w2.stride(0), mask_src=h, mask_scale=1.0 / (1.0 - p) if p > 0 else 1.0)
@@ -314,17 +351,17 @@
                     split_k=ops.pick_split_k(N, Hd, M), colsum_out=db2)
             pg.gemm(dpre, x2, dw1, Hd, K, M, a_mode=1, b_mode=1, lda=Hd, ldb=K, ldc=dw1.stride(0), accumulate=True,
                     split_k=ops.pick_split_k(Hd, K, M), colsum_out=db1)
-        return (dx,) + pg.result() + (None, None)
+        return (dx,) + pg.result() + (None, None, dres if ctx.needs_input_grad[7] else None, None)
 
 
 _NO_FFN_FUSE = os.environ.get("CAPE_NO_FFN_FUSE") is not None
 _DETERMINISTIC = os.environ.get("CAPE_DETERMINISTIC", "0") == "1"
 
 
-def ffn(x, w1, b1, w2, b2, dropout_p=0.0, rng_stream=0):
+def ffn(x, w1, b1, w2, b2, dropout_p=0.0, rng_stream=0, post=None):
     if _NO_FFN_FUSE:
-        return linear(linear(x, w1, b1, relu=True, dropout_p=dropout_p, rng_stream=rng_stream), w2, b2)
-    return FFNFn.apply(x, w1, b1, w2, b2, float(dropout_p), int(rng_stream))
+        return linear(linear(x, w1, b1, relu=True, dropout_p=dropout_p, rng_stream=rng_stream), w2, b2, post=post)
+    return FFNFn.apply(x, w1, b1, w2, b2, float(dropout_p), int(rng_stream), post.x if post is not None else None, post)
 
 
 def _adjacent(a, b):
@@ -568,14 +605,20 @@
 
 class AddLayerNormFn(torch.autograd.Function):
     @staticmethod
-    def forward(ctx, x, y, gamma, beta, pos, dropout_p, rng_stream):
+    def forward(ctx, x, y, gamma, beta, pos, dropout_p, rng_stream, post=None):
         x, y, pos = _c(x), _c(y), _c(pos)
         rng = Runtime.get_rng(x.device) if dropout_p > 0 else None
-        out, mean, rstd, out_pos = ops.add_layernorm_fwd(x, y, gamma, beta, pos=pos, dropout_p=dropout_p, rng=rng,
-                                                         rng_stream=rng_stream)
+        if post is not None:
+            assert y is None
+            dropout_p, rng_stream = post.p, post.stream
+            out, mean, rstd, out_pos = ops.add_layernorm_fwd(x, None, gamma, beta, pos=pos)
+        else:
+            out, mean, rstd, out_pos = ops.add_layernorm_fwd(x, y, gamma, beta, pos=pos, dropout_p=dropout_p, rng=rng,
+                                                             rng_stream=rng_stream)
         ctx.save_for_backward(x, y, gamma, mean, rstd)
         ctx.refs = (gamma, beta)
         ctx.slot = _slot_of(x)
+        ctx.post = post
         ctx.meta = (dropout_p, rng_stream, pos is not None)
         ctx.set_materialize_grads(False)
         if pos is None:
@@ -588,7 +631,7 @@
         p, stream, has_pos = ctx.meta
         g_pos = d_out_pos
         if d_out is None and d_out_pos is None:
-            return None, None, None, None, None, None, None
+            return None, None, None, None, None, None, None, None
         if d_out is None:
             d_out, d_out_pos = d_out_pos, None
         d_out, d_out_pos = _c(d_out), _c(d_out_pos)
@@ -596,14 +639,19 @@
         rng = Runtime.get_rng(x.device) if p > 0 else None
         dx, dy = ops.add_layernorm_bwd(d_out, d_out_pos, x, y, gamma, mean, rstd, *pg.bufs, dropout_p=p, rng=rng,
                                        rng_stream=stream)
-        if y is None or dy is not dx:
+        if ctx.post is not None:
+            ctx.post.dy = dy if p > 0 else None
+        elif y is None or dy is not dx:
             _slot_offer(ctx.slot, dx)
         dpos = g_pos if (has_pos and ctx.needs_input_grad[4]) else None
-        return (dx, (dy if y is not None else None)) + pg.result() + (dpos, None, None)
-
-
-def add_layernorm(x, y, gamma, beta, pos=None, dropout_p=0.0, rng_stream=0):
-    return AddLayerNormFn.apply(x, y, gamma, beta, pos, float(dropout_p), int(rng_stream))
+        return (dx, (dy if y is not None else None)) + pg.result() + (dpos, None, None, None)
+
+
+def add_layernorm(x, y, gamma, beta, pos=None, dropout_p=0.0, rng_stream=0, post=None):
+    if post is not None:
+        assert y is None and dropout_p == 0.0
+        return AddLayerNormFn.apply(x, None, gamma, beta, pos, 0.0, 0, post)
+    return AddLayerNormFn.apply(x, y, gamma, beta, pos, float(dropout_p), int(rng_stream), None)
 
 
 class AddFn(torch.autograd.Function):
@@ -894,7 +942,7 @@
 class MHAFn(torch.autograd.Function):
 
     @staticmethod
-    def forward(ctx, q_in, k_in, v_in, in_w, in_b, out_w, out_b, nheads, mask_mode, kpm_u8, dropout_p, rng_stream):
+    def forward(ctx, q_in, k_in, v_in, in_w, in_b, out_w, out_b, nheads, mask_mode, kpm_u8, dropout_p, rng_stream, res=None, post=None):
         ins = q_in, k_in, v_in = _c(q_in), _c(k_in), _c(v_in)
         N, Lq, C = q_in.shape
         Lk = k_in.shape[1]
@@ -914,7 +962,11 @@
         O, saved = ops.attn_core_fwd(ctx.route, q, k, v, N, nheads, Lq, Lk, scale, mask_mode=mask_mode, kpm=kpm_u8, dropout_p=dropout_p,
                                      rng=rng, rng_stream=rng_stream)
         out = torch.empty(N, Lq, C, dtype=torch.float32, device=dev)
-        ops.gemm(O.view(-1, C), out_w, out, N * Lq, C, C, bias=out_b)
+        if post is not None:
+            post.gemm(O.view(-1, C), out_w, out, N * Lq, C, C, bias=out_b)
+        else:
+            ops.gemm(O.view(-1, C), out_w, out, N * Lq, C, C, bias=out_b)
+        ctx.post, ctx.slot_res = post, (_slot_of(res) if post is not None else None)
         ctx.save_for_backward(q_in, k_in, v_in, in_w, out_w, q, k, v, O, kpm_u8, *saved)
         ctx.refs = (in_w, in_b, out_w, out_b)
         ctx.slot_q = _slot_of(q_in)
@@ -929,6 +981,9 @@
         N, Lq, C = q_in.shape
         Lk = k_in.shape[1]
         dev = d_out.device
+        d_res = None
+        if ctx.post is not None:
+            d_out, d_res = ctx.post.grads(d_out, ctx.slot_res)
         d_out2 = _c(d_out).view(-1, C)
         Mq = N * Lq
         dO = torch.empty(Mq, C, dtype=torch.float32, device=dev)
@@ -966,13 +1021,13 @@
             ops.gemm(g.view(-1, w * C), _from_row(in_w, r * C), dst, N * ins[r].shape[1], C, w * C, a_mode=0, b_mode=1, accumulate=acc)
             if live[0] == 1:
                 dk_in = dst
-        return (*d_ins, d_in_w, d_in_b, d_out_w, d_out_b, None, None, None, None, None)
+        return (*d_ins, d_in_w, d_in_b, d_out_w, d_out_b, None, None, None, None, None, d_res if ctx.needs_input_grad[12] else None, None)
 
 
 class DecSelfAttnFn(torch.autograd.Function):
 
     @staticmethod
-    def forward(ctx, tgt, pos, wq, wk, wv, in_w, in_b, out_w, out_b, nheads, dropout_p, rng_stream):
+    def forward(ctx, tgt, pos, wq, wk, wv, in_w, in_b, out_w, out_b, nheads, dropout_p, rng_stream, res=None, post=None):
         N, L, C = tgt.shape
         M = N * L
         dev = tgt.device
@@ -995,7 +1050,11 @@
         O, saved = ops.attn_core_fwd(ctx.route, q, k, v, N, nheads, L, L, scale, mask_mode=1, dropout_p=dropout_p, rng=rng,
                                      rng_stream=rng_stream)
         out = torch.empty(N, L, C, dtype=torch.float32, device=dev)
-        ops.gemm(O.view(M, C), out_w, out, M, C, C, bias=out_b)
+        if post is not None:
+            post.gemm(O.view(M, C), out_w, out, M, C, C, bias=out_b)
+        else:
+            ops.gemm(O.view(M, C), out_w, out, M, C, C, bias=out_b)
+        ctx.post, ctx.slot_res = post, (_slot_of(res) if post is not None else None)
         ctx.save_for_backward(x, wq, wk, wv, in_w, out_w, qkv1, qkv2, O, *saved)
         ctx.refs = (wq, wk, wv, in_w, in_b, out_w, out_b)
         ctx.meta = (nheads, dropout_p, rng_stream, scale, stacked, N, L, C)
@@ -1008,6 +1067,9 @@
         nheads, p, stream, scale, stacked, N, L, C = ctx.meta
         M = N * L
         dev = d_out.device
+        d_res = None
+        if ctx.post is not None:
+            d_out, d_res = ctx.post.grads(d_out, ctx.slot_res)
         d_out2 = _c(d_out).view(M, C)
         dO = torch.empty(M, C, dtype=torch.float32, device=dev)
         ops.gemm(d_out2, out_w, dO, M, C, C, a_mode=0, b_mode=1)
@@ -1042,15 +1104,17 @@
                 pg.gemm(dqkv1[:, i * C:], x, dw, C, C, M, a_mode=1, b_mode=1, lda=3 * C, ldb=C, accumulate=True,
                         split_k=ops.pick_split_k(C, C, M))
         dpos = dqkv1[:, :C].view(N, L, C) if need_pos else None
-        return (dx, dpos) + pg.result() + (None, None, None)
-
-
-def dec_self_attn(tgt, pos, wq, wk, wv, in_w, in_b, out_w, out_b, nheads=8, dropout_p=0.0, rng_stream=0):
-    return DecSelfAttnFn.apply(tgt, pos, wq, wk, wv, in_w, in_b, out_w, out_b, nheads, float(dropout_p), int(rng_stream))
-
-
-def mha(q_in, k_in, v_in, in_w, in_b, out_w, out_b, nheads=8, mask_mode=0, kpm_u8=None, dropout_p=0.0, rng_stream=0):
-    return MHAFn.apply(q_in, k_in, v_in, in_w, in_b, out_w, out_b, nheads, mask_mode, kpm_u8, float(dropout_p), int(rng_stream))
+        return (dx, dpos) + pg.result() + (None, None, None, d_res if ctx.needs_input_grad[12] else None, None)
+
+
+def dec_self_attn(tgt, pos, wq, wk, wv, in_w, in_b, out_w, out_b, nheads=8, dropout_p=0.0, rng_stream=0, post=None):
+    return DecSelfAttnFn.apply(tgt, pos, wq, wk, wv, in_w, in_b, out_w, out_b, nheads, float(dropout_p), int(rng_stream),
+                               post.x if post is not None else None, post)
+
+
+def mha(q_in, k_in, v_in, in_w, in_b, out_w, out_b, nheads=8, mask_mode=0, kpm_u8=None, dropout_p=0.0, rng_stream=0, post=None):
+    return MHAFn.apply(q_in, k_in, v_in, in_w, in_b, out_w, out_b, nheads, mask_mode, kpm_u8, float(dropout_p), int(rng_stream),
+                       post.x if post is not None else None, post)
 
 
 class TokenEmbedFn(torch.autograd.Function):
diff --git a/category-agnostic-pose-estimation_amd/hip/lib.py b/category-agnostic-pose-estimation_amd/hip/lib.py
--- a/category-agnostic-pose-estimation_amd/hip/lib.py
+++ b/category-agnostic-pose-estimation_amd/hip/lib.py
@@ -37,6 +37,7 @@
         ("sC0", c_longlong), ("sC1", c_longlong),
         ("res_cols", c_int), ("sBias0", c_longlong), ("sBias1", c_longlong),
         ("cPadX", c_int), ("cKHp", c_int), ("cKWp", c_int), ("cTapH0", c_int), ("cTapHS", c_int), ("cTapW0", c_int), ("cTapWS", c_int),
+        ("res_post", c_int),
     ]
 
 
@@ -179,11 +180,19 @@
     "cape_decode_tail": [POINTER(DecodeTailDesc), P],
     "cape_decode_step": [POINTER(DecodeStepDesc), P],
 }
-EXPORTS = ["cape_last_error", "cape_abi_version", "cape_groupnorm_workspace_bytes", "cape_packed_weight_bytes"] + list(_SIGS)
+EXPORTS = ["cape_last_error", "cape_abi_version", "cape_gemm_desc_bytes", "cape_groupnorm_workspace_bytes", "cape_packed_weight_bytes"] + list(_SIGS)
 _lib.cape_packed_weight_bytes.argtypes = [I, I]
 _lib.cape_packed_weight_bytes.restype = c_size_t
 _lib.cape_groupnorm_workspace_bytes.argtypes = [I, I, I]
 _lib.cape_groupnorm_workspace_bytes.restype = c_size_t
+try:
+    _lib.cape_gemm_desc_bytes.restype = c_size_t
+    _desc_bytes = _lib.cape_gemm_desc_bytes()
+except AttributeError:
+    _desc_bytes = -1
+if _desc_bytes != ctypes.sizeof(GemmDesc):
+    raise ImportError(f"{LIB_PATH} is stale: its cape_gemm_desc has {_desc_bytes} bytes, this binding {ctypes.sizeof(GemmDesc)}; "
+                      "rebuild it (make -C category-agnostic-pose-estimation_amd/csrc)")
 
 for _name, _args in _SIGS.items():
     _fn = getattr(_lib, _name)
diff --git a/category-agnostic-pose-estimation_amd/hip/ops.py b/category-agnostic-pose-estimation_amd/hip/ops.py
--- a/category-agnostic-pose-estimation_amd/hip/ops.py
+++ b/category-agnostic-pose-estimation_amd/hip/ops.py
@@ -219,7 +219,11 @@
 
 def gemm_desc(A, B, C, M, N, K, a_mode=0, b_mode=0, lda=None, ldb=None, ldc=None, bias=None, scale=None, residual=None,
               ldr=None, relu=False, accumulate=False, split_k=1, dropout_p=0.0, rng=None, rng_stream=0, conv=None,
-              colsum_out=None, packed=None, mask_src=None, mask_scale=1.0, batch=None, res_cols=0, bias_strides=None, conv_sub=None):
+              colsum_out=None, packed=None, mask_src=None, mask_scale=1.0, batch=None, res_cols=0, bias_strides=None, conv_sub=None,
+              post_residual=None):
+    if post_residual is not None:
+        assert residual is None and not relu and not accumulate and split_k == 1 and mask_src is None and batch is None and res_cols == 0
+        residual = post_residual
     for t, n in ((A, "A"), (B, "B"), (C, "C"), (bias, "bias"), (scale, "scale"), (residual, "residual")):
         _chk(t, "gemm." + n, contiguous=False)
     if (_AUTO_SPLIT_NN and a_mode == 0 and b_mode == 1 and split_k == 1 and K >= 512 and M > 64 and batch is None and conv is None
@@ -247,6 +251,7 @@
     d.residual = residual.data_ptr() if residual is not None else None
     d.ldr = ldr if ldr is not None else N
     d.res_cols = int(res_cols)
+    d.res_post = int(post_residual is not None)
     d.relu, d.accumulate, d.split_k = int(relu), int(accumulate), int(split_k)
     d.dropout_p = float(dropout_p)
     d.rng_state = rng.t.data_ptr() if (rng is not None and dropout_p > 0) else None
@@ -389,7 +394,7 @@
     for t, n in ((d_out, "d_out"), (d_out_pos, "d_out_pos"), (x, "x"), (y, "y"), (dgamma, "dgamma"), (dbeta, "dbeta")):
         _chk(t, "ln_bwd." + n)
     d_x = torch.empty_like(x)
-    d_y = torch.empty_like(x) if (y is not None and dropout_p > 0) else None
+    d_y = torch.empty_like(x) if dropout_p > 0 else None
     lib.call("cape_add_layernorm_bwd", _p(d_out), _p(d_out_pos), _p(x), _p(y), _p(gamma), _p(mean), _p(rstd), _p(d_x),
              _p(d_y), _p(dgamma), _p(dbeta), rows, C, float(dropout_p),
              rng.ptr if (rng is not None and dropout_p > 0) else None, rng_stream, _stream())
diff --git a/category-agnostic-pose-estimation_amd/models/deformable_transformer.py b/category-agnostic-pose-estimation_amd/models/deformable_transformer.py
--- a/category-agnostic-pose-estimation_amd/models/deformable_transformer.py
+++ b/category-agnostic-pose-estimation_amd/models/deformable_transformer.py
@@ -51,7 +51,7 @@
             value = HF.zero_rows(value, padding_rows_u8)
         return value
 
-    def forward(self, query, reference_points, input_flatten, geo, padding_rows_u8=None, value=None):
+    def forward(self, query, reference_points, input_flatten, geo, padding_rows_u8=None, value=None, post=None):
         if reference_points.shape[-1] != 2:
             raise ValueError("Last dim of reference_points must be 2 (box references are not on the CAPE path)")
         assert geo.S == input_flatten.shape[1]
@@ -60,7 +60,7 @@
         offw = HF.linear_cat2(query, self.sampling_offsets.weight, self.sampling_offsets.bias,
                               self.attention_weights.weight, self.attention_weights.bias)
         out = HF.msda(value, offw, reference_points, geo, self.n_points)
-        return HF.linear(out, self.output_proj.weight, self.output_proj.bias)
+        return HF.linear(out, self.output_proj.weight, self.output_proj.bias, post=post)
 
 
 class DeformableTransformerEncoderLayer(nn.Module):
@@ -81,12 +81,14 @@
     def forward(self, src, src_pos, pos, reference_points, geo, padding_rows_u8=None):
         p = self.dropout1.p if self.training else 0.0
         src_v, src_r = HF.fanout(src, 2)
-        a = self.self_attn(src_pos, reference_points, src_v, geo, padding_rows_u8)
-        src = HF.add_layernorm(src_r, a, self.norm1.weight, self.norm1.bias, dropout_p=p, rng_stream=self._streams[0])
+        post = HF.PostResidual(src_r, p, self._streams[0])
+        s = self.self_attn(src_pos, reference_points, src_v, geo, padding_rows_u8, post=post)
+        src = HF.add_layernorm(s, None, self.norm1.weight, self.norm1.bias, post=post)
         src_f, src_r = HF.fanout(src, 2)
-        h = HF.ffn(src_f, self.linear1.weight, self.linear1.bias, self.linear2.weight, self.linear2.bias, dropout_p=p,
-                   rng_stream=self._streams[1])
-        return HF.add_layernorm(src_r, h, self.norm2.weight, self.norm2.bias, pos=pos, dropout_p=p, rng_stream=self._streams[2])
+        post = HF.PostResidual(src_r, p, self._streams[2])
+        s = HF.ffn(src_f, self.linear1.weight, self.linear1.bias, self.linear2.weight, self.linear2.bias, dropout_p=p,
+                   rng_stream=self._streams[1], post=post)
+        return HF.add_layernorm(s, None, self.norm2.weight, self.norm2.bias, pos=pos, post=post)
 
 
 _REF_POINTS = {}
diff --git a/category-agnostic-pose-estimation_amd/models/deformable_transformer_v2.py b/category-agnostic-pose-estimation_amd/models/deformable_transformer_v2.py
--- a/category-agnostic-pose-estimation_amd/models/deformable_transformer_v2.py
+++ b/category-agnostic-pose-estimation_amd/models/deformable_transformer_v2.py
@@ -70,32 +70,38 @@
         qp_q, qp_s = HF.fanout(query_pos, 2)
         if _FUSED_SELF_ATTN:
             t_a, t_r = HF.fanout(tgt, 2)
+            post = HF.PostResidual(t_r, p, st[1])
             t2 = HF.dec_self_attn(t_a, qp_q, self.attn_q.weight, self.attn_k.weight, self.attn_v.weight, sa.in_proj_weight,
-                                  sa.in_proj_bias, sa.out_proj.weight, sa.out_proj.bias, self.n_heads, dropout_p=p, rng_stream=st[0])
+                                  sa.in_proj_bias, sa.out_proj.weight, sa.out_proj.bias, self.n_heads, dropout_p=p, rng_stream=st[0],
+                                  post=post)
         else:
             t_q, t_k, t_v, t_r = HF.fanout(tgt, 4)
             q = HF.linear(t_q, self.attn_q.weight, residual=qp_q)
             k = HF.linear(t_k, self.attn_k.weight)
             v = HF.linear(t_v, self.attn_v.weight)
+            post = HF.PostResidual(t_r, p, st[1])
             t2 = HF.mha(q, k, v, sa.in_proj_weight, sa.in_proj_bias, sa.out_proj.weight, sa.out_proj.bias, self.n_heads,
-                        mask_mode=1, dropout_p=p, rng_stream=st[0])
-        tgt = HF.add_layernorm(t_r, t2, self.norm2.weight, self.norm2.bias, dropout_p=p, rng_stream=st[1])
+                        mask_mode=1, dropout_p=p, rng_stream=st[0], post=post)
+        tgt = HF.add_layernorm(t2, None, self.norm2.weight, self.norm2.bias, post=post)
         if support_features is not None:
             ca = self.support_attn
             t_q, t_r = HF.fanout(tgt, 2)
+            post = HF.PostResidual(t_r, p, st[3])
             t2 = HF.mha(t_q, support_features, support_features, ca.in_proj_weight, ca.in_proj_bias, ca.out_proj.weight,
                         ca.out_proj.bias, self.n_heads, mask_mode=2 if support_kpm_u8 is not None else 0,
-                        kpm_u8=support_kpm_u8, dropout_p=p, rng_stream=st[2])
-            tgt, tgt_pos = HF.add_layernorm(t_r, t2, self.norm_support.weight, self.norm_support.bias, pos=qp_s,
-                                            dropout_p=p, rng_stream=st[3])
+                        kpm_u8=support_kpm_u8, dropout_p=p, rng_stream=st[2], post=post)
+            tgt, tgt_pos = HF.add_layernorm(t2, None, self.norm_support.weight, self.norm_support.bias, pos=qp_s, post=post)
         else:
             tgt, t_r = HF.fanout(tgt, 2)
             tgt_pos = HF.add(t_r, qp_s)
-        t2 = self.cross_attn(tgt_pos, reference_points, src, geo, padding_rows_u8)
-        tgt = HF.add_layernorm(tgt, t2, self.norm1.weight, self.norm1.bias, dropout_p=p, rng_stream=st[4])
+        post = HF.PostResidual(tgt, p, st[4])
+        t2 = self.cross_attn(tgt_pos, reference_points, src, geo, padding_rows_u8, post=post)
+        tgt = HF.add_layernorm(t2, None, self.norm1.weight, self.norm1.bias, post=post)
         t_f, t_r = HF.fanout(tgt, 2)
-        h = HF.ffn(t_f, self.linear1.weight, self.linear1.bias, self.linear2.weight, self.linear2.bias, dropout_p=p, rng_stream=st[5])
-        return HF.add_layernorm(t_r, h, self.norm3.weight, self.norm3.bias, dropout_p=p, rng_stream=st[6])
+        post = HF.PostResidual(t_r, p, st[6])
+        h = HF.ffn(t_f, self.linear1.weight, self.linear1.bias, self.linear2.weight, self.linear2.bias, dropout_p=p, rng_stream=st[5],
+                   post=post)
+        return HF.add_layernorm(h, None, self.norm3.weight, self.norm3.bias, post=post)
 
     @torch.no_grad()
     def decode_step(self, tgt, query_pos, reference_points, geo, step, cache):
diff --git a/category-agnostic-pose-estimation_amd/models/geometric_support_encoder.py b/category-agnostic-pose-estimation_amd/models/geometric_support_encoder.py
--- a/category-agnostic-pose-estimation_amd/models/geometric_support_encoder.py
+++ b/category-agnostic-pose-estimation_amd/models/geometric_support_encoder.py
@@ -59,13 +59,15 @@
         for li, layer in enumerate(self.transformer_encoder.layers):
             sa, st = layer.self_attn, self._streams[li]
             x_a, x_r = HF.fanout(x, 2)
+            post = HF.PostResidual(x_r, p, st[1])
             a = HF.mha(x_a, x_a, x_a, sa.in_proj_weight, sa.in_proj_bias, sa.out_proj.weight, sa.out_proj.bias, self.nhead,
-                       mask_mode=2, kpm_u8=kpm, dropout_p=p, rng_stream=st[0])
-            x = HF.add_layernorm(x_r, a, layer.norm1.weight, layer.norm1.bias, dropout_p=p, rng_stream=st[1])
+                       mask_mode=2, kpm_u8=kpm, dropout_p=p, rng_stream=st[0], post=post)
+            x = HF.add_layernorm(a, None, layer.norm1.weight, layer.norm1.bias, post=post)
             x_f, x_r = HF.fanout(x, 2)
+            post = HF.PostResidual(x_r, p, st[3])
             hdn = HF.ffn(x_f, layer.linear1.weight, layer.linear1.bias, layer.linear2.weight, layer.linear2.bias, dropout_p=p,
-                         rng_stream=st[2])
-            x = HF.add_layernorm(x_r, hdn, layer.norm2.weight, layer.norm2.bias, dropout_p=p, rng_stream=st[3])
+                         rng_stream=st[2], post=post)
+            x = HF.add_layernorm(hdn, None, layer.norm2.weight, layer.norm2.bias, post=post)
         x = HF.zero_rows(x, zero_u8.reshape(-1))
         return x
 
diff --git a/category-agnostic-pose-estimation_amd/models/support_encoder.py b/category-agnostic-pose-estimation_amd/models/support_encoder.py
--- a/category-agnostic-pose-estimation_amd/models/support_encoder.py
+++ b/category-agnostic-pose-estimation_amd/models/support_encoder.py
@@ -93,13 +93,15 @@
         for li, layer in enumerate(self.transformer_encoder.layers):
             sa, st = layer.self_attn, self._streams[li]
             x_a, x_r = HF.fanout(x, 2)
+            post = HF.PostResidual(x_r, p, st[1])
             a = HF.mha(x_a, x_a, x_a, sa.in_proj_weight, sa.in_proj_bias, sa.out_proj.weight, sa.out_proj.bias, self.nheads,
-                       mask_mode=mode, kpm_u8=kpm, dropout_p=p, rng_stream=st[0])
-            x = HF.add_layernorm(x_r, a, layer.norm1.weight, layer.norm1.bias, dropout_p=p, rng_stream=st[1])
+                       mask_mode=mode, kpm_u8=kpm, dropout_p=p, rng_stream=st[0], post=post)
+            x = HF.add_layernorm(a, None, layer.norm1.weight, layer.norm1.bias, post=post)
             x_f, x_r = HF.fanout(x, 2)
+            post = HF.PostResidual(x_r, p, st[3])
             hdn = HF.ffn(x_f, layer.linear1.weight, layer.linear1.bias, layer.linear2.weight, layer.linear2.bias, dropout_p=p,
-                         rng_stream=st[2])
-            x = HF.add_layernorm(x_r, hdn, layer.norm2.weight, layer.norm2.bias, dropout_p=p, rng_stream=st[3])
+                         rng_stream=st[2], post=post)
+            x = HF.add_layernorm(hdn, None, layer.norm2.weight, layer.norm2.bias, post=post)
         if fast:
             x = HF.zero_rows(x, kpm.reshape(-1))
         return HF.add_layernorm(x, None, self.norm.weight, self.norm.bias)
diff --git a/include/cape_hip.h b/include/cape_hip.h
--- a/include/cape_hip.h
+++ b/include/cape_hip.h
@@ -42,9 +42,11 @@
   int batch, batch_div; long long sA0, sA1, sB0, sB1, sC0, sC1;
   int res_cols; long long sBias0, sBias1;
   int cPadX, cKHp, cKWp, cTapH0, cTapHS, cTapW0, cTapWS;
+  int res_post;
 } cape_gemm_desc;
 
 int cape_gemm_f32(const cape_gemm_desc* d, cape_stream_t stream);
+size_t cape_gemm_desc_bytes(void);
 
 #define CAPE_GEMM_GROUP_MAX 32
 int cape_gemm_group_f32(const cape_gemm_desc* descs, int n, int tile, cape_stream_t stream);
```
